# tgm-team/tgm

Measured on AMD Instinct MI355X. Metric: sampled-edges/sec (TGAT 2-hop k=20 recency sampler, tgbl-wiki synthetic), higher is better.
Workload: dtype int32/int64 indices + f32 feature rows (copied, no arithmetic)

## Files before the change

include/tgm_amd.h:

```cpp
#ifndef TGM_AMD_H
#define TGM_AMD_H

#include <stddef.h>
#include <stdint.h>

#ifdef __cplusplus
extern "C" {
#endif

#define TGMX_ABI_VERSION 7

#define TGMX_OK 0
#define TGMX_E_INVALID (-1)
#define TGMX_E_LAUNCH (-2)
#define TGMX_E_UNSUPPORTED (-3)

#define TGMX_ST_SEED_RANGE 1
#define TGMX_ST_SEED_TIME 2
#define TGMX_ST_EDGE_RANGE 4
#define TGMX_ST_SCRATCH 8
#define TGMX_ST_TS_BOUND 16

typedef void* tgmx_stream_t;
typedef void* tgmx_event_t;
// ... 40 lines not shown
                     int32_t* status, tgmx_stream_t stream,
                     tgmx_event_t ev_start, tgmx_event_t ev_stop);

size_t tgmx_ring_update_scratch_bytes(int64_t n, int32_t directed);
int tgmx_ring_update(tgmx_adj_t* ring, int32_t* write_pos, float* ring_x, int32_t D, int32_t B,
                     int32_t num_nodes, const int32_t* src, const int32_t* dst, const int64_t* ts,
                     const float* edge_x, int64_t n, int64_t eid0, int32_t directed, int32_t key_wrap32,
                     int32_t* scratch, int32_t* status, tgmx_stream_t stream);

#define TGMX_MAX_SEED_GROUPS 8
#define TGMX_MAX_HOPS 8
typedef struct tgmx_recency_step {
  tgmx_adj_t* ring;
  int32_t* write_pos;
  float* ring_x;
  const int64_t* indptr;
  int64_t ev_lo, ev_hi;
  int32_t D, B, num_nodes;
  int32_t n_groups;
  const int32_t* grp_nid[TGMX_MAX_SEED_GROUPS];
  const int64_t* grp_ts[TGMX_MAX_SEED_GROUPS];
  int64_t grp_n[TGMX_MAX_SEED_GROUPS];
  int32_t* seed_nid0;
  int64_t* seed_ts0;
  int64_t S0;
  int32_t n_hops;
  int32_t k[TGMX_MAX_HOPS];
  int32_t* out_nid[TGMX_MAX_HOPS];
  int64_t* out_ts[TGMX_MAX_HOPS];
  float* out_x[TGMX_MAX_HOPS];
  const int32_t* src;
  const int32_t* dst;
  const int64_t* ts;
  const float* edge_x;
  int64_t n, eid0;
  int32_t directed, key_wrap32;
  int32_t* scratch;
  int32_t* status;
  int32_t timed_hop;
  tgmx_event_t ev_start, ev_stop;
  int64_t ts_bound;
  int32_t neg_group, neg_low, neg_high;
  uint64_t neg_seed, neg_call;
  int32_t* neg_out;
  int64_t* neg_time_out;
  int32_t guard_seed_errors;
  int32_t sorted_ts;
  int32_t* out_valid[TGMX_MAX_HOPS];
  int32_t* out_valid_prev[TGMX_MAX_HOPS];
  int64_t neg_index0;
  int64_t* csr_cursor;
  int32_t csr_x_by_pos;
  int32_t* out_eid[TGMX_MAX_HOPS];
} tgmx_recency_step_t;

int tgmx_recency_step(const tgmx_recency_step_t* step, tgmx_stream_t stream);
int tgmx_recency_step_plan(const tgmx_recency_step_t* step);

#define TGMX_SEED_SRC 0
#define TGMX_SEED_DST 1
#define TGMX_SEED_NEG 2
typedef struct tgmx_pipeline {
  const int32_t* src;
  const int32_t* dst;
  const int64_t* ts;
  const float* edge_x;
  int64_t num_edges;
  int32_t rank, world;
  int32_t n_roles;
  int32_t seed_role[TGMX_MAX_SEED_GROUPS];
  int32_t neg_low, neg_high;
  uint64_t neg_seed;
  int32_t update;
  int32_t reserved0;
  tgmx_recency_step_t step;
} tgmx_pipeline_t;

typedef struct tgmx_pipeline_out {
  int32_t* neg;
  int64_t* neg_time;
  int32_t* seed_nid0;
  int64_t* seed_ts0;
  int32_t* out_nid[TGMX_MAX_HOPS];
  int64_t* out_ts[TGMX_MAX_HOPS];
  float* out_x[TGMX_MAX_HOPS];
  int32_t timed_hop;
  tgmx_event_t ev_start, ev_stop;
  int32_t* out_valid[TGMX_MAX_HOPS];
  int32_t* out_valid_prev[TGMX_MAX_HOPS];
  int32_t* out_eid[TGMX_MAX_HOPS];
} tgmx_pipeline_out_t;

typedef struct tgmx_pipeline_post {
  int32_t dedup;
  int32_t dedup_neg, dedup_nbr;
  int32_t num_nodes;
  void* dedup_ws;
  int32_t* uniq_out;
  int32_t edge_hop;
  int64_t edge_cap;
  int64_t* row_off;
  int64_t* edge_index;
  int64_t* edge_t;
  float* edge_x;
  int64_t* dev_sizes;
  int64_t* host_sizes;
  tgmx_event_t sizes_ready;
} tgmx_pipeline_post_t;

typedef void* tgmx_worker_t;
// ... 374 lines not shown
```

tgm_amd/_native.py:

```python
from __future__ import annotations

import ctypes
import os
from ctypes import c_char_p, c_int32, c_int64, c_size_t, c_void_p
from typing import Optional

import torch

from .exceptions import NativeLibraryError

_HERE = os.path.dirname(os.path.abspath(__file__))
LIB_PATH = os.path.join(_HERE, 'csrc', 'libtgm_amd.so')

_P = c_void_p
SIGNATURES = {
    'tgmx_version': (c_int32, []),
    'tgmx_abi_sizeof': (c_size_t, [c_int32]),
    'tgmx_last_error': (c_char_p, []),
    'tgmx_event_create': (c_int32, [ctypes.POINTER(c_void_p)]),
    'tgmx_event_destroy': (c_int32, [_P]),
    'tgmx_event_elapsed_ms': (c_int32, [_P, _P, ctypes.POINTER(ctypes.c_float)]),
    'tgmx_recency_lookup_csr': (
        c_int32,
        [_P, _P, _P, c_int32, _P, _P, c_int64, c_int32, c_int32, c_int64, c_int64, c_int32, c_int32, _P, _P, _P, _P, _P, _P, _P],
# ... 91 lines not shown
class TgatLayerGrads(ctypes.Structure):
    _fields_ = [(n, c_void_p) for n in ('W_Q', 'W_KV', 'W_O', 'b_O', 'ln_g', 'ln_b', 'fc1_w', 'fc1_b', 'fc2_w', 'fc2_b')]


class TgatGrads(ctypes.Structure):
    _fields_ = [('tw', c_void_p), ('tb', c_void_p), ('layers', TgatLayerGrads * TGAT_MAX_LAYERS)]


PACK_MAX_JOBS = 32


class PackJob(ctypes.Structure):
    _fields_ = [('src', c_void_p), ('dst', c_void_p), ('src_ld', c_int64), ('dst_ld', c_int64), ('rows', c_int32), ('cols', c_int32),
                ('dst_rows', c_int32), ('dst_cols', c_int32), ('transpose', c_int32), ('reserved_', c_int32)]


class TgatLayerLayout(ctypes.Structure):
    _fields_ = [(n, c_int64) for n in ('R', 'rres', 'oattn', 'y', 'Q', 'qf', 'zbar', 'cat', 'h1', 'probs', 'out')] + [
        (n, c_int32) for n in ('Op', 'dhp', 'Cp', 'Kc', 'Ep')
    ]


class TgatLayout(ctypes.Structure):
    _fields_ = [('total_bytes', c_int64), ('z0', c_int64), ('level_rows', c_int64 * (TGAT_MAX_LAYERS + 1)),
                ('level_off', c_int64 * (TGAT_MAX_LAYERS + 2)), ('layers', TgatLayerLayout * TGAT_MAX_LAYERS),
                ('compact', c_int64 * (TGAT_MAX_LAYERS + 1))]


MAX_SEED_GROUPS = 8
MAX_HOPS = 8


class RecencyStep(ctypes.Structure):

    _fields_ = [
        ('ring', c_void_p), ('write_pos', c_void_p), ('ring_x', c_void_p),
        ('indptr', c_void_p), ('ev_lo', c_int64), ('ev_hi', c_int64),
        ('D', c_int32), ('B', c_int32), ('num_nodes', c_int32),
        ('n_groups', c_int32),
        ('grp_nid', c_void_p * MAX_SEED_GROUPS), ('grp_ts', c_void_p * MAX_SEED_GROUPS), ('grp_n', c_int64 * MAX_SEED_GROUPS),
        ('seed_nid0', c_void_p), ('seed_ts0', c_void_p), ('S0', c_int64),
        ('n_hops', c_int32), ('k', c_int32 * MAX_HOPS),
        ('out_nid', c_void_p * MAX_HOPS), ('out_ts', c_void_p * MAX_HOPS), ('out_x', c_void_p * MAX_HOPS),
        ('src', c_void_p), ('dst', c_void_p), ('ts', c_void_p), ('edge_x', c_void_p),
        ('n', c_int64), ('eid0', c_int64), ('directed', c_int32), ('key_wrap32', c_int32),
        ('scratch', c_void_p), ('status', c_void_p),
        ('timed_hop', c_int32), ('ev_start', c_void_p), ('ev_stop', c_void_p),
        ('ts_bound', c_int64),
        ('neg_group', c_int32), ('neg_low', c_int32), ('neg_high', c_int32),
        ('neg_seed', ctypes.c_uint64), ('neg_call', ctypes.c_uint64), ('neg_out', c_void_p), ('neg_time_out', c_void_p),
        ('guard_seed_errors', c_int32), ('sorted_ts', c_int32),
        ('out_valid', c_void_p * MAX_HOPS), ('out_valid_prev', c_void_p * MAX_HOPS),
        ('neg_index0', c_int64), ('csr_cursor', c_void_p), ('csr_x_by_pos', c_int32), ('out_eid', c_void_p * MAX_HOPS),
    ]


class PipelinePost(ctypes.Structure):

    _fields_ = [
        ('dedup', c_int32), ('dedup_neg', c_int32), ('dedup_nbr', c_int32), ('num_nodes', c_int32), ('dedup_ws', c_void_p), ('uniq_out', c_void_p),
        ('edge_hop', c_int32), ('edge_cap', c_int64), ('row_off', c_void_p), ('edge_index', c_void_p), ('edge_t', c_void_p), ('edge_x', c_void_p),
        ('dev_sizes', c_void_p), ('host_sizes', c_void_p), ('sizes_ready', c_void_p),
    ]


class TgnMemoryFwd(ctypes.Structure):

    _fields_ = [
        ('nodes', c_void_p), ('R', c_int64), ('memory', c_void_p), ('last_update', c_void_p), ('M', c_int32), ('num_nodes', c_int32),
        ('st_lo_s', c_void_p), ('st_cnt_s', c_void_p), ('st_lo_d', c_void_p), ('st_cnt_d', c_void_p),
        ('log_other', c_void_p), ('log_t', c_void_p), ('log_raw', c_void_p), ('D', c_int32),
        ('tw', c_void_p), ('tb', c_void_p), ('T', c_int32), ('mean', c_int32),
        ('W_ih', c_void_p), ('b_ih', c_void_p), ('W_hh', c_void_p), ('b_hh', c_void_p),
        ('ws_aggr', c_void_p), ('ws_h', c_void_p), ('ws_gi', c_void_p), ('ws_gh', c_void_p),
        ('out_mem', c_void_p), ('out_lu', c_void_p), ('assoc', c_void_p), ('stamp', c_int64),
    ]


class TgnStep(ctypes.Structure):

    _fields_ = [
        ('mem', c_void_p), ('conv', c_void_p),
        ('src', c_void_p), ('dst', c_void_p), ('t', c_void_p), ('raw', c_void_p), ('n', c_int32),
        ('memory', c_void_p), ('last_update', c_void_p), ('reuse_status', c_void_p),
        ('log_base', c_int64), ('log_other', c_void_p), ('log_t', c_void_p), ('log_raw', c_void_p),
        ('st_lo_s', c_void_p), ('st_cnt_s', c_void_p), ('st_lo_d', c_void_p), ('st_cnt_d', c_void_p),
    ]


class TgcnFwd(ctypes.Structure):

    _fields_ = [
        ('x', c_void_p), ('N', c_int64), ('in_ch', c_int32), ('C', c_int32),
        ('src', c_void_p), ('dst', c_void_p), ('edge_w', c_void_p), ('E', c_int64), ('fill', ctypes.c_float), ('add_self_loops', c_int32),
        ('W3', c_void_p), ('b3', c_void_p),
        ('lin_w', c_void_p * 3), ('lin_b', c_void_p * 3),
        ('H', c_void_p),
        ('A', c_void_p), ('ldA', c_int64), ('norm_ws', c_void_p), ('xwt', c_void_p), ('G', c_void_p), ('cat', c_void_p), ('pre', c_void_p * 3),
        ('out', c_void_p), ('idx32', c_int32),
    ]


MIXER_MAX_LAYERS = 8


class MixerLayer(ctypes.Structure):
# ... 8 lines not shown
        ('nbr_edge_x', c_void_p), ('seed_t', c_void_p), ('nbr_t', c_void_p), ('nbr_nids', c_void_p),
        ('seeds', c_void_p * 3), ('n_seeds', c_int64 * 3),
        ('tg_nbr', c_void_p), ('tg_lo', c_void_p), ('tg_cnt', c_void_p),
        ('node_x', c_void_p), ('num_nodes', c_int64), ('F', c_int32),
        ('S', c_int64), ('K', c_int32), ('D', c_int32), ('T', c_int32), ('E', c_int32), ('num_layers', c_int32), ('eps', ctypes.c_float),
        ('tw', c_void_p), ('tb', c_void_p), ('proj_w', c_void_p), ('proj_b', c_void_p), ('out_w', c_void_p), ('out_b', c_void_p),
        ('layers', MixerLayer * MIXER_MAX_LAYERS),
        ('x0', c_void_p), ('z', c_void_p), ('z1', c_void_p), ('y', c_void_p), ('h', c_void_p), ('cat', c_void_p),
        ('ldx0', c_int64), ('ldz', c_int64), ('ldh', c_int64), ('ldcat', c_int64),
        ('out', c_void_p),
    ]


class TconvFwd(ctypes.Structure):

    _fields_ = [
        ('x', c_void_p), ('U', c_int64), ('in_ch', c_int32), ('last_update_local', c_void_p),
        ('src', c_void_p), ('tgt', c_void_p), ('t', c_void_p), ('msg', c_void_p), ('E', c_int64), ('D', c_int32), ('T', c_int32),
        ('tw', c_void_p), ('tb', c_void_p), ('W4', c_void_p), ('b4', c_void_p), ('W_edge', c_void_p), ('H', c_int32), ('C', c_int32),
        ('edge_attr', c_void_p), ('qkvs', c_void_p), ('eproj', c_void_p), ('order', c_void_p), ('seg_lo', c_void_p), ('seg_hi', c_void_p),
        ('sort_ws', c_void_p), ('sort_ws_bytes', c_size_t), ('status', c_void_p),
        ('tgt_count', c_void_p), ('cursor', c_void_p), ('order_big', c_void_p),
    ]


SEED_SRC, SEED_DST, SEED_NEG = 0, 1, 2


class Pipeline(ctypes.Structure):

    _fields_ = [
        ('src', c_void_p), ('dst', c_void_p), ('ts', c_void_p), ('edge_x', c_void_p), ('num_edges', c_int64),
        ('rank', c_int32), ('world', c_int32), ('n_roles', c_int32), ('seed_role', c_int32 * MAX_SEED_GROUPS),
        ('neg_low', c_int32), ('neg_high', c_int32), ('neg_seed', ctypes.c_uint64),
        ('update', c_int32), ('reserved0', c_int32), ('step', RecencyStep),
    ]


class PipelineOut(ctypes.Structure):

    _fields_ = [
        ('neg', c_void_p), ('neg_time', c_void_p), ('seed_nid0', c_void_p), ('seed_ts0', c_void_p),
        ('out_nid', c_void_p * MAX_HOPS), ('out_ts', c_void_p * MAX_HOPS), ('out_x', c_void_p * MAX_HOPS),
        ('timed_hop', c_int32), ('ev_start', c_void_p), ('ev_stop', c_void_p),
        ('out_valid', c_void_p * MAX_HOPS), ('out_valid_prev', c_void_p * MAX_HOPS), ('out_eid', c_void_p * MAX_HOPS),
    ]


ACCOUNTING_PARTIALS = 1024
SIGNATURES['tgmx_lookup_accounting'] = (c_int32, [_P, c_int64, _P, _P, c_int64, _P, _P])
SIGNATURES['tgmx_uniform_lookup_csr'] = (c_int32, [_P, _P, _P, c_int32, _P, c_int64, c_int32, c_int64, c_int32, c_int32, ctypes.c_uint64, ctypes.c_uint64,
                                                   _P, _P, _P, _P, _P])
SIGNATURES['tgmx_ring_update_scratch_bytes'] = (c_size_t, [c_int64, c_int32])
SIGNATURES['tgmx_tgn_gru_gate_backward'] = (c_int32, [_P, _P, _P, _P, c_int32, c_int64, _P, _P, _P])
SIGNATURES['tgmx_tgn_aggregate_backward'] = (c_int32, [c_int64, _P, _P, _P, _P, _P, _P, c_int32, c_int32, _P, _P, c_int32, c_int32, _P, _P, _P])
SIGNATURES['tgmx_tconv_edge_attr_backward'] = (c_int32, [_P, _P, _P, _P, _P, _P, c_int32, c_int32, c_int64, _P, _P])
SIGNATURES['tgmx_tconv_attend_backward'] = (c_int32, [_P, _P, _P, _P, _P, _P, _P, _P, c_int64, c_int32, c_int32, ctypes.c_float, _P, _P, _P, _P, _P, _P, _P])
SIGNATURES['tgmx_group_ids'] = (c_int32, [_P, c_int32, _P, _P, _P, _P, _P, _P])
SIGNATURES['tgmx_group_ids_workspace_bytes'] = (c_size_t, [c_int64])
SIGNATURES['tgmx_group_ids_large'] = (c_int32, [_P, c_int64, _P, _P, _P, _P, _P, _P, c_size_t, _P])
SIGNATURES['tgmx_random_negatives'] = (c_int32, [c_int32, c_int32, c_int64, ctypes.c_uint64, ctypes.c_uint64, _P, _P, c_int64, _P, _P])
SIGNATURES['tgmx_random_negatives_at'] = (c_int32, [c_int32, c_int32, c_int64, ctypes.c_uint64, ctypes.c_uint64, c_int64, _P, _P, c_int64, _P, _P])
SIGNATURES['tgmx_unique_ids_workspace_bytes'] = (c_size_t, [c_int32])
SIGNATURES['tgmx_unique_ids'] = (c_int32, [_P, _P, c_int32, c_int32, _P, _P, _P, _P, _P])
SIGNATURES['tgmx_csr_build_workspace_bytes'] = (c_size_t, [c_int64, c_int32, c_int32])
SIGNATURES['tgmx_csr_build'] = (c_int32, [_P, _P, _P, c_int64, c_int32, _P, c_int64, c_int32, _P, _P, _P, c_size_t, _P, _P])
SIGNATURES['tgmx_recency_step'] = (c_int32, [ctypes.POINTER(RecencyStep), _P])
SIGNATURES['tgmx_recency_step_plan'] = (c_int32, [ctypes.POINTER(RecencyStep)])
SIGNATURES['tgmx_pipeline_step'] = (c_int32, [ctypes.POINTER(Pipeline), c_int64, c_int64, ctypes.c_uint64, ctypes.POINTER(PipelineOut), ctypes.POINTER(PipelinePost), _P])
SIGNATURES['tgmx_event_synchronize'] = (c_int32, [_P])
SIGNATURES['tgmx_event_create_sync'] = (c_int32, [ctypes.POINTER(c_void_p)])
SIGNATURES['tgmx_event_record'] = (c_int32, [_P, _P])
SIGNATURES['tgmx_stream_wait_event'] = (c_int32, [_P, _P])
SIGNATURES['tgmx_stream_handoff'] = (c_int32, [_P, _P, _P])
SIGNATURES['tgmx_worker_create'] = (c_int32, [ctypes.POINTER(c_void_p)])
SIGNATURES['tgmx_worker_destroy'] = (c_int32, [_P])
SIGNATURES['tgmx_worker_pipeline_step'] = (c_int32, [_P, ctypes.POINTER(Pipeline), c_int64, c_int64, ctypes.c_uint64, ctypes.POINTER(PipelineOut),
                                                     ctypes.POINTER(PipelinePost), _P, _P, _P, ctypes.POINTER(ctypes.c_uint64)])
SIGNATURES['tgmx_worker_wait'] = (c_int32, [_P, ctypes.c_uint64])
SIGNATURES['tgmx_slice'] = (c_int32, [_P, c_int64, c_int32, c_int64, c_int32, c_int64, c_int64, c_int64, ctypes.POINTER(c_int64), ctypes.POINTER(c_int64)])
SIGNATURES['tgmx_discretize_workspace_bytes'] = (c_size_t, [c_int64])
SIGNATURES['tgmx_discretize_keep'] = (c_int32, [_P, _P, _P, c_int64, ctypes.c_double, _P, _P, _P, _P, c_size_t, _P])
SIGNATURES['tgmx_tgn_memory_forward'] = (c_int32, [ctypes.POINTER(TgnMemoryFwd), _P])
SIGNATURES['tgmx_tconv_forward'] = (c_int32, [ctypes.POINTER(TconvFwd), _P])
SIGNATURES['tgmx_tgn_step'] = (c_int32, [ctypes.POINTER(TgnStep), _P])
SIGNATURES['tgmx_segment_sort_workspace_bytes'] = (c_size_t, [c_int64])
SIGNATURES['tgmx_segment_sort'] = (c_int32, [_P, c_int64, c_int32, _P, _P, _P, _P, c_size_t, _P, _P])
SIGNATURES['tgmx_tgat_tile16_floats'] = (c_size_t, [c_int32, c_int32])
SIGNATURES['tgmx_tgat_tile16'] = (c_int32, [_P, c_int64, c_int32, c_int32, _P, _P])
SIGNATURES['tgmx_pack2d'] = (c_int32, [ctypes.POINTER(PackJob), c_int32, _P])

SIGNATURES['tgmx_pair_dedup_workspace_bytes'] = (c_size_t, [c_int64])
SIGNATURES['tgmx_pair_dedup'] = (c_int32, [_P, _P, c_int64, _P, _P, _P, _P, _P, c_size_t, _P])
SIGNATURES['tgmx_tgat_layout'] = (c_int32, [ctypes.POINTER(TgatModel), c_int64, ctypes.POINTER(TgatHop), c_int32, ctypes.POINTER(TgatLayout)])
SIGNATURES['tgmx_tgat_workspace_bytes'] = (c_size_t, [ctypes.POINTER(TgatModel), c_int64, ctypes.POINTER(TgatHop)])
SIGNATURES['tgmx_tgat_backward_workspace_bytes'] = (c_size_t, [ctypes.POINTER(TgatModel), ctypes.POINTER(TgatLayout), ctypes.POINTER(TgatHop)])
SIGNATURES['tgmx_tgat_backward'] = (c_int32, [ctypes.POINTER(TgatModel), ctypes.POINTER(TgatLayout), ctypes.POINTER(TgatHop), _P, _P, c_int64,
                                              ctypes.POINTER(Dropout), ctypes.POINTER(TgatGrads), _P, c_size_t, _P])
SIGNATURES['tgmx_tgat_forward'] = (
    c_int32,
    [ctypes.POINTER(TgatModel), _P, c_int64, _P, c_int64, ctypes.POINTER(TgatHop), _P, c_size_t, c_int32, _P, _P],
)

SIGNATURES['tgmx_sgemm_nt_ep'] = (c_int32, [_P, c_int64, _P, c_int64, _P, c_int64, c_int64, c_int32, c_int32, _P, c_int32, _P, c_int64, _P])
SIGNATURES['tgmx_time_gap_workspace_bytes'] = (c_size_t, [c_int64])
SIGNATURES['tgmx_time_gap_group'] = (c_int32, [_P, _P, c_int64, c_int64, _P, c_int64, _P, c_int64, _P, c_int64, _P, c_size_t, _P, _P, _P, _P])
# ... 90 lines not shown
```

tgm_amd/csrc/pipeline.hip:

```cpp
#include <algorithm>

#include "common.h"

using namespace tgmx;

__global__ __launch_bounds__(64) void sizes_to_host_kernel(const int64_t* __restrict__ dev, int64_t* __restrict__ host) {
  if (threadIdx.x < 3) __hip_atomic_store(&host[threadIdx.x], dev[threadIdx.x], __ATOMIC_RELAXED, __HIP_MEMORY_SCOPE_SYSTEM);
}

static int pipeline_post(const tgmx_pipeline_t* p, const tgmx_recency_step_t& s, int64_t edge_lo, int64_t n_edges, long long share,
                         const tgmx_pipeline_out_t* out, const tgmx_pipeline_post_t* post, tgmx_stream_t stream) {
  TGMX_REQUIRE(post->dev_sizes && post->host_sizes && post->sizes_ready, "pipeline_step: post block needs dev_sizes / host_sizes / sizes_ready");
  long long rows[TGMX_MAX_HOPS + 1];
  rows[0] = share * p->n_roles;
  for (int h = 0; h < s.n_hops; ++h) rows[h + 1] = rows[h] * s.k[h];
  bool scan_rides = false;
  if (post->dedup) {
    TGMX_REQUIRE(post->dedup_ws && post->uniq_out, "pipeline_step: null dedup buffer");
    const int32_t* parts[16];
    int64_t sizes[16];
    int np = 0;
    parts[np] = p->src + edge_lo; sizes[np++] = n_edges;
    parts[np] = p->dst + edge_lo; sizes[np++] = n_edges;
    if (post->dedup_neg && s.neg_out) { parts[np] = s.neg_out; sizes[np++] = share; }
// ... 39 lines not shown
                                  const tgmx_pipeline_out_t* out, const tgmx_pipeline_post_t* post, tgmx_stream_t stream) {
  TGMX_REQUIRE(p && out, "pipeline_step: null argument block");
  TGMX_REQUIRE(p->src && p->dst && p->ts && p->num_edges >= 0, "pipeline_step: null stream pointer");
  TGMX_REQUIRE(edge_lo >= 0 && n_edges >= 0 && edge_lo + n_edges <= p->num_edges, "pipeline_step: edges [%lld, +%lld) outside the store (%lld)",
               (long long)edge_lo, (long long)n_edges, (long long)p->num_edges);
  TGMX_REQUIRE(p->world >= 1 && p->rank >= 0 && p->rank < p->world, "pipeline_step: rank %d of %d", p->rank, p->world);
  TGMX_REQUIRE(p->n_roles >= 1 && p->n_roles <= TGMX_MAX_SEED_GROUPS, "pipeline_step: %d seed roles", p->n_roles);
  tgmx_recency_step_t s = p->step;
  const long long lo = n_edges * p->rank / p->world, hi = n_edges * (p->rank + 1) / p->world;
  const long long share = hi - lo;
  s.n_groups = p->n_roles;
  s.neg_out = nullptr;
  s.neg_group = -1;
  for (int g = 0; g < p->n_roles; ++g) {
    s.grp_ts[g] = p->ts + edge_lo + lo;
    s.grp_n[g] = share;
    switch (p->seed_role[g]) {
      case TGMX_SEED_SRC: s.grp_nid[g] = p->src + edge_lo + lo; break;
      case TGMX_SEED_DST: s.grp_nid[g] = p->dst + edge_lo + lo; break;
      case TGMX_SEED_NEG:
        TGMX_REQUIRE(s.neg_group < 0, "pipeline_step: more than one negatives role");
        TGMX_REQUIRE(share == 0 || (out->neg && out->neg_time), "pipeline_step: null negatives output");
        s.grp_nid[g] = nullptr;
        s.neg_group = g; s.neg_low = p->neg_low; s.neg_high = p->neg_high; s.neg_seed = p->neg_seed; s.neg_call = neg_call;
        s.neg_index0 = lo;
        s.neg_out = out->neg; s.neg_time_out = out->neg_time;
        break;
      default: TGMX_REQUIRE(false, "pipeline_step: seed role %d", p->seed_role[g]);
    }
  }
  s.seed_nid0 = out->seed_nid0;
  s.seed_ts0 = out->seed_ts0;
  for (int h = 0; h < s.n_hops && h < TGMX_MAX_HOPS; ++h) {
    s.out_nid[h] = out->out_nid[h];
    s.out_ts[h] = out->out_ts[h];
    s.out_x[h] = out->out_x[h];
    s.out_valid[h] = out->out_valid[h];
    s.out_valid_prev[h] = out->out_valid_prev[h];
    s.out_eid[h] = out->out_eid[h];
  }
  s.timed_hop = out->timed_hop;
  s.ev_start = out->ev_start;
  s.ev_stop = out->ev_stop;
  if (s.indptr) {
    s.ev_hi = edge_lo;
    s.n = 0;
  } else if (p->update && n_edges > 0) {
    s.src = p->src + edge_lo;
    s.dst = p->dst + edge_lo;
    s.ts = p->ts + edge_lo;
    s.edge_x = (p->edge_x && s.D > 0) ? p->edge_x + edge_lo * (long long)s.D : nullptr;
    s.n = n_edges;
    s.eid0 = edge_lo;
  } else {
    s.n = 0;
  }
  if (share == 0) {
    return TGMX_OK;
  }
  const int rc = tgmx_recency_step(&s, stream);
  if (rc || !post) return rc;
  return pipeline_post(p, s, edge_lo, n_edges, share, out, post, stream);
}

extern "C" int tgmx_slice(const int64_t* t, int64_t n, int32_t has_start_time, int64_t start_time, int32_t has_end_time,
                          int64_t end_time, int64_t start_idx, int64_t end_idx, int64_t* lb, int64_t* ub) {
  TGMX_REQUIRE((t || n == 0) && n >= 0 && lb && ub, "slice: bad arguments");
  long long l = has_start_time ? std::lower_bound(t, t + n, start_time) - t : 0;
  long long u = has_end_time ? std::upper_bound(t, t + n, end_time) - t : n;
  const long long lo_c = start_idx > 0 ? start_idx : 0, hi_c = end_idx >= 0 ? end_idx : n;
  l = std::max(lo_c, std::min(hi_c, l));
  u = std::max(lo_c, std::min(hi_c, u));
  *lb = l;
  *ub = u;
  return TGMX_OK;
}

namespace {
__global__ __launch_bounds__(256) void lookup_accounting_kernel(const int32_t* __restrict__ ids, long long slots, const int32_t* __restrict__ sp,
                                                                const int32_t* __restrict__ sc, long long rows, unsigned long long* __restrict__ counts) {
  unsigned long long v = 0, m = 0, c = 0;
  const long long step = (long long)gridDim.x * blockDim.x;
  for (long long i = (long long)blockIdx.x * blockDim.x + threadIdx.x; i < slots; i += step) v += ids[i] != -1;
  if (sp && sc)
    for (long long i = (long long)blockIdx.x * blockDim.x + threadIdx.x; i < rows; i += step) {
      const int a = sp[i], b = sc[i];
      m += (unsigned long long)(a > b ? a : b);
      c += (unsigned long long)b;
    }
  for (int o = 32; o > 0; o >>= 1) {
    v += __shfl_xor(v, o);
    m += __shfl_xor(m, o);
    c += __shfl_xor(c, o);
  }
  if ((threadIdx.x & 63) == 0) {
    unsigned long long* o = counts + ((long long)blockIdx.x * (blockDim.x >> 6) + (threadIdx.x >> 6)) * 3;
    o[0] = v; o[1] = m; o[2] = c;
  }
}
}

extern "C" int tgmx_lookup_accounting(const int32_t* ids, int64_t slots, const int32_t* span_prev, const int32_t* span_cur, int64_t rows,
                                      int64_t* counts, tgmx_stream_t stream) {
  TGMX_REQUIRE(ids && counts && slots >= 0 && rows >= 0, "lookup_accounting: bad arguments");
  hipStream_t st = (hipStream_t)stream;
  hipLaunchKernelGGL(lookup_accounting_kernel, dim3(TGMX_ACCOUNTING_PARTIALS / 4), dim3(256), 0, st, ids, (long long)slots, span_prev, span_cur, (long long)rows,
// ... 5 lines not shown
```

tgm_amd/csrc/recency.hip:

```cpp
#include <atomic>
#include <cstdlib>
#include <cstring>

#include <hip/hip_ext.h>
#include <rocprim/block/block_radix_sort.hpp>
#include <rocprim/block/block_scan.hpp>
#include <rocprim/device/device_radix_sort.hpp>
#include <rocprim/device/device_scan.hpp>
#include <rocprim/iterator/counting_iterator.hpp>
#include <rocprim/iterator/transform_iterator.hpp>

#include "common.h"

namespace tgmx {

struct __align__(16) Rec {
  int nbr;
  int eid;
  long long ts;
};
static_assert(sizeof(Rec) == sizeof(tgmx_adj_t), "record layout");

struct SeedGroups {
  const int32_t* nid[TGMX_MAX_SEED_GROUPS];
  const int64_t* ts[TGMX_MAX_SEED_GROUPS];
  long long end[TGMX_MAX_SEED_GROUPS];
  int32_t* out_nid;
  int64_t* out_ts;
  int groups;
  int gen;
  int gen_low;
  unsigned gen_range;
  unsigned long long gen_seed, gen_call, gen_index0;
  int32_t* gen_out;
  int64_t* gen_out_ts;
};

struct LookupArgs {
  SeedGroups grp;
  const int64_t* indptr;
  const Rec* recs;
  const int32_t* write_pos;
  const float* edge_x;
  const int32_t* seeds;
  const int64_t* qtimes;
  int32_t* out_nid;
  int64_t* out_ts;
  float* out_x;
  int32_t* status;
  long long S;
  long long ev_lo, ev_hi;
  int D, k, B, N, allow_pad;
  int row_vecs;
  FastDiv dv;
  FastDiv dv_seed;
  int32_t* out_eid;
  int32_t* out_eid1;
  int x_by_pos;
  long long* cursor;
  int leave_room;
  unsigned side_blocks;
  int side_stage;
  unsigned tail_blocks;
  int k1;
  int32_t* out_nid1;
  int64_t* out_ts1;
  float* out_x1;
  int32_t* out_valid;
  int32_t* out_valid1;
  int32_t* out_valid_prev;
  int32_t* out_valid_prev1;
};

template <int VEC>
struct VecOf;
template <>
struct VecOf<4> { using type = float4; };
template <>
struct VecOf<2> { using type = float2; };
template <>
struct VecOf<1> { using type = float; };

template <typename T>
__device__ __forceinline__ T zero_vec();
template <>
__device__ __forceinline__ float4 zero_vec<float4>() { return make_float4(0.f, 0.f, 0.f, 0.f); }
template <>
__device__ __forceinline__ float2 zero_vec<float2>() { return make_float2(0.f, 0.f); }
template <>
__device__ __forceinline__ float zero_vec<float>() { return 0.f; }

__device__ __forceinline__ long long wave_prefix_count(const Rec* recs, long long a, long long z,
                                                       long long bound, int lane) {
  long long lo = a, hi = z;
  while (hi - lo > kWave) {
    const long long len = hi - lo;
    const long long stride = (len + kWave - 1) / kWave;
    long long idx = lo + (long long)(lane + 1) * stride - 1;
    if (idx > hi - 1) idx = hi - 1;
    const bool less = (long long)recs[idx].eid < bound;
    const int c = __popcll(__ballot(less));
    long long nlo = lo, nhi = hi;
    if (c > 0) {
      long long p = lo + (long long)c * stride - 1;
      if (p > hi - 1) p = hi - 1;
      nlo = p + 1;
    }
    if (c < kWave) {
      long long p = lo + (long long)(c + 1) * stride - 1;
      if (p > hi - 1) p = hi - 1;
      nhi = p;
    }
    lo = nlo;
    hi = nhi < nlo ? nlo : nhi;
  }
  const long long idx = lo + lane;
  const bool less = idx < hi && (long long)recs[idx].eid < bound;
  return lo + __popcll(__ballot(less)) - a;
}

struct UpdateArgs {
  Rec* ring;
  int32_t* write_pos;
  float* ring_x;
  const float* edge_x;
  const int32_t* src;
  const int32_t* dst;
  const int64_t* ts;
  int32_t* sorted_j;
  int32_t* sorted_node;
  int32_t* target;
  int32_t* winner;
  Rec* sorted_rec;
  long long* key;
  int32_t* node;
  long long* span;
  unsigned long long* keys_in;
  unsigned int* vals_in;
  int32_t* hash_key;
  int32_t* hash_maxp;
  int32_t* run_start;
  int32_t* run_len;
  int hash_bits;
  long long ts_bound;
  int sorted_ts;
  int sort_bits;
  int32_t* barrier;
  int32_t* status;
  int guard_mask;
  long long n, m, eid0;
  int B, N, D, key_wrap32;
};

__device__ __forceinline__ long long update_key(int node, long long t, long long span, int wrap32) {
  if (wrap32) {
    const unsigned int prod = (unsigned int)node * (unsigned int)(int)span;
    return (long long)(int)prod + t;
  }
  return (long long)node * span + t;
}

__device__ __forceinline__ void update_entry(const UpdateArgs& a, long long j, int& node, int& nbr, long long& t,
                                             long long& i) {
  const bool rev = j >= a.n;
  i = rev ? j - a.n : j;
  const int s = a.src[i], d = a.dst[i];
  node = rev ? d : s;
  nbr = rev ? s : d;
  t = a.ts[i];
}

constexpr int kBlockMaxM = 4096;
constexpr int kChunk = 256;

__device__ __forceinline__ long long strided_max_ts(const int64_t* __restrict__ ts, long long n, int tid, int nthr) {
  long long mx = -0x7fffffffffffffffLL;
  for (long long base = tid; base < n; base += 8ll * nthr) {
    long long v[8];
#pragma unroll
    for (int u = 0; u < 8; ++u) {
      const long long x = base + (long long)u * nthr;
      v[u] = x < n ? ts[x] : mx;
    }
#pragma unroll
    for (int u = 0; u < 8; ++u) mx = v[u] > mx ? v[u] : mx;
  }
  return mx;
}

__device__ __forceinline__ long long strided_min_ts(const int64_t* __restrict__ ts, long long n, int tid, int nthr) {
  long long mn = 0x7fffffffffffffffLL;
  for (long long base = tid; base < n; base += 8ll * nthr) {
    long long v[8];
#pragma unroll
    for (int u = 0; u < 8; ++u) {
      const long long x = base + (long long)u * nthr;
      v[u] = x < n ? ts[x] : mn;
    }
#pragma unroll
    for (int u = 0; u < 8; ++u) mn = v[u] < mn ? v[u] : mn;
  }
  return mn;
}

constexpr int kBlockThreads = 1024;


__device__ __forceinline__ void bitonic_select(long long& key, int& pay, long long pk, int pp, int e, int jj, int k) {
  const bool low = (e & jj) == 0, asc = (e & k) == 0;
  const bool mine_after = pair_after(key, pay, pk, pp);
  if ((low == asc) == mine_after) {
    key = pk;
    pay = pp;
  }
}

__device__ __forceinline__ bool update_blocked(const UpdateArgs& a) {
  return a.guard_mask != 0 && (__hip_atomic_load(a.status, __ATOMIC_RELAXED, __HIP_MEMORY_SCOPE_AGENT) & a.guard_mask) != 0;
}

__device__ __forceinline__ void commit_write_pos(int32_t* wp, int kept, int B) {
  const int old = atomicAdd(wp, kept);
  constexpr int kFold = 1 << 30;
  if (old < kFold && old + kept >= kFold) atomicSub(wp, kFold / B * B);
}

template <int MAXM>
struct PlaceLds {
  int sn[MAXM];
  int len[MAXM];
  int h_key[2 * MAXM], h_maxp[2 * MAXM];
  long long red[kBlockThreads / kWave], red2[kBlockThreads / kWave];
  int wave_tot[kBlockThreads / kWave];
};
template <int MAXM>
struct SortLds {
  long long key[MAXM];
  int pay[MAXM];
};

template <typename T>
__device__ __forceinline__ void st_agent(T* p, T v) {
  __hip_atomic_store(p, v, __ATOMIC_RELAXED, __HIP_MEMORY_SCOPE_AGENT);
}
template <typename T>
__device__ __forceinline__ T ld_agent(const T* p) {
  return __hip_atomic_load(p, __ATOMIC_RELAXED, __HIP_MEMORY_SCOPE_AGENT);
}

template <int E, int MAXM, bool PRESORTED, bool DEFER, bool COH = false>
__device__ __forceinline__ void update_block_body(const UpdateArgs& a, PlaceLds<MAXM>& L, SortLds<PRESORTED ? 1 : MAXM>& S,
                                                  int part = 0, int parts = 1) {
  constexpr int H = 2 * MAXM;
  constexpr int HBITS = MAXM == 512 ? 10 : (MAXM == 1024 ? 11 : (MAXM == 2048 ? 12 : 13));
  static_assert((1 << HBITS) == H, "hash size");
  long long* s_key = S.key;
  int* s_pay = S.pay;
  int* s_sn = L.sn;
  int* s_len = L.len;
  int* h_key = L.h_key;
  int* h_maxp = L.h_maxp;
  long long* red = L.red;
  long long* red2 = L.red2;
  int* wave_tot = L.wave_tot;
  const int m = (int)a.m;
  const int tid = threadIdx.x, lane = tid & 63, wave = tid >> 6;
  const int nthr = blockDim.x, nwaves = nthr >> 6;
  const int P = nthr * E;
  const bool blocked = DEFER ? false : update_blocked(a);

  for (int x = tid; x < H; x += nthr) {
    h_key[x] = -1;
    h_maxp[x] = -1;
  }
  int pay[E], node[E], w[E];
  if constexpr (PRESORTED) {
#pragma unroll
// ... 80 lines not shown
    }
    if (lane == kWave - 1) wave_tot[wave] = incl;
    int before = __shfl_up(incl, 1);
    if (lane == 0) before = 0;
    __syncthreads();
    for (int wv = 0; wv < wave; ++wv) before = wave_tot[wv] > before ? wave_tot[wv] : before;
#pragma unroll
    for (int r = 0; r < E; ++r) st[r] = st[r] > before ? st[r] : before;
  }
#pragma unroll
  for (int r = 0; r < E; ++r) {
    const int p = tid * E + r;
    if (p < m && (p == m - 1 || s_sn[p + 1] != node[r])) s_len[st[r]] = p - st[r] + 1;
  }
  __syncthreads();

  int tgt[E], hs[E], cnt[E];
#pragma unroll
  for (int r = 0; r < E; ++r) {
    const int p = tid * E + r;
    tgt[r] = -1;
    hs[r] = 0;
    cnt[r] = 0;
    if (p < m && node[r] >= 0 && (parts == 1 || node[r] % parts == part)) {
      cnt[r] = s_len[st[r]];
      const int pos = p - st[r];
      const int drop = cnt[r] > a.B ? cnt[r] - a.B : 0;
      if (pos >= drop) {
        const int t = node[r] * a.B + (w[r] + pos - drop) % a.B;
        unsigned h = ((unsigned)t * 2654435761u) >> (32 - HBITS);
        for (;;) {
          const int old = atomicCAS(&h_key[h], -1, t);
          if (old == -1 || old == t) break;
          h = (h + 1) & (H - 1);
        }
        atomicMax(&h_maxp[h], p);
        tgt[r] = t;
        hs[r] = (int)h;
      }
    }
  }
  __syncthreads();

#pragma unroll
  for (int r = 0; r < E; ++r) {
    const int p = tid * E + r;
    if (p >= m) continue;
    if (parts > 1 && (node[r] >= 0 ? node[r] % parts : 0) != part) continue;
    int win = -1, kept = 0;
    if (tgt[r] >= 0) {
      if (h_maxp[hs[r]] == p) {
        Rec rec;
        if constexpr (DEFER) {
        } else if constexpr (PRESORTED) {
          rec = a.sorted_rec[p];
        } else {
          int nd, nbr;
          long long t, i;
          update_entry(a, pay[r], nd, nbr, t, i);
          rec.nbr = nbr;
          rec.eid = a.eid0 >= 0 ? (int)(a.eid0 + i) : -1;
          rec.ts = t;
        }
        if constexpr (!DEFER) {
          if (!blocked) a.ring[tgt[r]] = rec;
        }
        win = blocked ? -1 : tgt[r];
      }
      if (p == st[r] + cnt[r] - 1) {
        kept = cnt[r] > a.B ? a.B : cnt[r];
        if constexpr (!DEFER) {
          if (!blocked) commit_write_pos(&a.write_pos[node[r]], kept, a.B);
        }
      }
    }
    a.winner[p] = win;
    if constexpr (DEFER) a.target[p] = kept;
    if constexpr (!PRESORTED) a.sorted_j[p] = pay[r];
  }
}

template <int E, int MAXM, bool PRESORTED>
__global__ __launch_bounds__(kBlockThreads) void ring_update_block_kernel(const UpdateArgs a) {
  __shared__ PlaceLds<MAXM> L;
  __shared__ SortLds<PRESORTED ? 1 : MAXM> S;
  update_block_body<E, MAXM, PRESORTED, false>(a, L, S, (int)blockIdx.x, (int)gridDim.x);
}

template <int E, int MAXM>
__global__ __launch_bounds__(kBlockThreads) void ring_update_decide_kernel(const UpdateArgs a) {
  __shared__ PlaceLds<MAXM> L;
  __shared__ SortLds<1> S;
  update_block_body<E, MAXM, true, true>(a, L, S, (int)blockIdx.x, (int)gridDim.x);
}


struct ChunkSortLds {
  long long key[kChunk];
  int pay[kChunk];
  long long red[kChunk / kWave], red2[kChunk / kWave];
};

template <bool AGENT = false>
__device__ __forceinline__ void update_chunk_sort(const UpdateArgs& a, int chunk, ChunkSortLds& W) {
  long long* s_key = W.key;
  int* s_pay = W.pay;
  long long* red = W.red;
  long long* red2 = W.red2;
  const int tid = threadIdx.x, lane = tid & 63, wave = tid >> 6;
  long long mx = strided_max_ts(a.ts, a.n, tid, kChunk), mn = strided_min_ts(a.ts, a.n, tid, kChunk);
  for (int off = 32; off > 0; off >>= 1) {
    const long long o = __shfl_xor(mx, off), o2 = __shfl_xor(mn, off);
    mx = o > mx ? o : mx;
    mn = o2 < mn ? o2 : mn;
  }
  if (lane == 0) {
    red[wave] = mx;
    red2[wave] = mn;
  }
  __syncthreads();
  mx = red[0];
  mn = red2[0];
  for (int w = 1; w < kChunk / kWave; ++w) {
    mx = red[w] > mx ? red[w] : mx;
    mn = red2[w] < mn ? red2[w] : mn;
// ... 104 lines not shown
  __syncthreads();

  int pos[NE][NC];
#pragma unroll
  for (int q = 0; q < NE; ++q) {
#pragma unroll
    for (int o = 0; o < NC; ++o) {
      int cnt = 0;
      if (act[q] && o < chunks && o != c0 + q) {
        const long long* sk = W.key + o * kSamplesPerChunk;
        const int* sp = W.pay + o * kSamplesPerChunk;
        if (pair_after(key[q], pay[q], sk[kSamplesPerChunk - 1], sp[kSamplesPerChunk - 1])) {
          cnt = kSamplesPerChunk;
        } else {
#pragma unroll
          for (int st = kSamplesPerChunk / 2; st > 0; st >>= 1)
            if (pair_after(key[q], pay[q], sk[cnt + st - 1], sp[cnt + st - 1])) cnt += st;
        }
      }
      pos[q][o] = cnt > 0 ? (cnt - 1) * kSampleEvery + 1 : -1;
    }
  }
#pragma unroll
  for (int st = kSampleEvery / 2; st > 0; st >>= 1) {
    long long k2[NE][NC];
#pragma unroll
    for (int q = 0; q < NE; ++q)
#pragma unroll
      for (int o = 0; o < NC; ++o) k2[q][o] = pos[q][o] >= 0 ? ld_agent(&gk[o * kChunk + pos[q][o] + st - 1]) : 0;
#pragma unroll
    for (int q = 0; q < NE; ++q) {
#pragma unroll
      for (int o = 0; o < NC; ++o) {
        if (pos[q][o] < 0) continue;
        bool after = key[q] > k2[q][o];
        if (key[q] == k2[q][o]) after = pay[q] > ld_agent(&gp[o * kChunk + pos[q][o] + st - 1]);
        if (after) pos[q][o] += st;
      }
    }
  }
  int node[NE], nbr[NE];
  long long t[NE], i[NE];
#pragma unroll
  for (int q = 0; q < NE; ++q) {
    node[q] = nbr[q] = -1;
    t[q] = i[q] = 0;
    if (act[q]) update_entry(a, pay[q], node[q], nbr[q], t[q], i[q]);
  }
  int w[NE];
  bool valid[NE];
#pragma unroll
  for (int q = 0; q < NE; ++q) {
    valid[q] = act[q] && node[q] >= 0 && node[q] < a.N && nbr[q] >= 0 && nbr[q] < a.N;
    w[q] = valid[q] ? a.write_pos[node[q]] : 0;
  }
#pragma unroll
  for (int q = 0; q < NE; ++q) {
    if (!act[q]) continue;
    int rank = tid;
#pragma unroll
    for (int o = 0; o < NC; ++o) rank += pos[q][o] >= 0 ? pos[q][o] : 0;
    if (!valid[q]) atomicOr(a.status, TGMX_ST_EDGE_RANGE);
    Rec rec;
    rec.nbr = nbr[q];
    rec.eid = a.eid0 >= 0 ? (int)(a.eid0 + i[q]) : -1;
    rec.ts = t[q];
    if constexpr (COH) {
      st_agent(&a.sorted_j[rank], pay[q]);
      st_agent(&a.sorted_node[rank], valid[q] ? node[q] : -1);
      st_agent(&a.target[rank], w[q] % a.B);
    } else {
      a.sorted_j[rank] = pay[q];
      a.sorted_node[rank] = valid[q] ? node[q] : -1;
      a.target[rank] = w[q] % a.B;
    }
    a.sorted_rec[rank] = rec;
  }
}

constexpr int kSideSort = 1, kSideMerge = 2, kSidePlace = 3, kSideAll = 4, kSideSortMerge = 5, kSidePlaceOnly = 6, kSideSortMergePlace = 7, kSideMergePlace = 8;

__device__ __forceinline__ bool rider_barrier(int32_t* bar, int parts) {
  __syncthreads();
  bool ok = true;
  if (threadIdx.x == 0) {
    const int gen = __hip_atomic_load(&bar[1], __ATOMIC_RELAXED, __HIP_MEMORY_SCOPE_AGENT);
    const int prev = __hip_atomic_fetch_add(&bar[0], 1, __ATOMIC_RELAXED, __HIP_MEMORY_SCOPE_AGENT);
    if (prev == parts - 1) {
      __hip_atomic_store(&bar[0], 0, __ATOMIC_RELAXED, __HIP_MEMORY_SCOPE_AGENT);
      __builtin_amdgcn_s_waitcnt(0);
      __hip_atomic_fetch_add(&bar[1], 1, __ATOMIC_RELAXED, __HIP_MEMORY_SCOPE_AGENT);
    } else {
      int spins = 0;
      while (__hip_atomic_load(&bar[1], __ATOMIC_RELAXED, __HIP_MEMORY_SCOPE_AGENT) == gen) {
        __builtin_amdgcn_s_sleep(8);
        if (++spins > (1 << 19)) {
          ok = false;
          break;
        }
      }
    }
  }
  __syncthreads();
  return ok;
}
constexpr int kRidePlaceMaxM = 1024;

constexpr int kTailGroups = 32;
__device__ __forceinline__ void tail_signal(int32_t* bar, bool publish, unsigned bid, unsigned nblk) {
  __syncthreads();
  if (threadIdx.x == 0) {
    if (publish) {
      __threadfence();
      __hip_atomic_store(&bar[4], 1, __ATOMIC_RELAXED, __HIP_MEMORY_SCOPE_AGENT);
      __hip_atomic_fetch_add(&bar[2], 1, __ATOMIC_RELAXED, __HIP_MEMORY_SCOPE_AGENT);
    } else {
      const unsigned g = bid % kTailGroups;
      const unsigned size = (nblk - g + kTailGroups - 1) / kTailGroups;
      int32_t* cnt = &bar[16 + 16 * g];
      const int prev = __hip_atomic_fetch_add(cnt, 1, __ATOMIC_RELAXED, __HIP_MEMORY_SCOPE_AGENT);
      if (prev == (int)size - 1) {
        __hip_atomic_store(cnt, 0, __ATOMIC_RELAXED, __HIP_MEMORY_SCOPE_AGENT);
        __hip_atomic_fetch_add(&bar[2], (int)size, __ATOMIC_RELAXED, __HIP_MEMORY_SCOPE_AGENT);
      }
    }
  }
}

__device__ __forceinline__ bool tail_wait(const int32_t* word, unsigned need) {
  int spins = 0;
  while ((unsigned)__hip_atomic_load(word, __ATOMIC_RELAXED, __HIP_MEMORY_SCOPE_AGENT) < need) {
    __builtin_amdgcn_s_sleep(8);
    if (++spins > (1 << 22)) return false;
  }
  return true;
}

__device__ __forceinline__ void tail_commit(const UpdateArgs& a, unsigned tb, unsigned tail_blocks, unsigned need) {
  __shared__ int ok_s;
  const int lane = lane_id();
  const long long p = (long long)tb * (blockDim.x >> 6) + (threadIdx.x >> 6);
  if (threadIdx.x == 0) ok_s = tail_wait(&a.barrier[4], 1u) ? 1 : 0;
  __syncthreads();
  bool ok = ok_s != 0;
  int row = -1, kept = 0, node = 0;
  long long rec_lo = 0, rec_hi = 0;
  constexpr int kMaxCols = 8;
  float xv[kMaxCols];
  const float* x = nullptr;
  const bool wide = a.D > kMaxCols * kWave;
  if (ok && p < a.m) {
    row = ld_agent(&a.winner[p]);
    kept = ld_agent(&a.target[p]);
    if (row >= 0) {
      const long long* src = reinterpret_cast<const long long*>(&a.sorted_rec[p]);
      rec_lo = ld_agent(&src[0]);
      rec_hi = ld_agent(&src[1]);
    }
    if (kept > 0) node = ld_agent(&a.sorted_node[p]);
    if (row >= 0 && a.D > 0 && a.edge_x) {
      const long long j = ld_agent(&a.sorted_j[p]);
      x = a.edge_x + (j >= a.n ? j - a.n : j) * a.D;
      if (!wide) {
#pragma unroll
        for (int u = 0; u < kMaxCols; ++u) {
          const int c = lane + u * kWave;
          xv[u] = c < a.D ? x[c] : 0.f;
        }
      }
    }
  }
  if (threadIdx.x == 0) ok_s = (ok && tail_wait(&a.barrier[2], need)) ? 1 : 0;
  __syncthreads();
  ok = ok_s != 0;
  if (!ok) {
    if (threadIdx.x == 0) atomicOr(a.status, TGMX_ST_SCRATCH);
  } else if (p < a.m && !update_blocked(a)) {
    if (lane == 0) {
      if (row >= 0) {
        long long* dst = reinterpret_cast<long long*>(&a.ring[row]);
        dst[0] = rec_lo;
        dst[1] = rec_hi;
      }
      if (kept > 0) commit_write_pos(&a.write_pos[node], kept, a.B);
    }
    if (row >= 0 && a.D > 0) {
      float* __restrict__ o = a.ring_x + (long long)row * a.D;
      if (!x) {
        for (int c = lane; c < a.D; c += kWave) o[c] = 0.f;
      } else if (wide) {
        for (int c = lane; c < a.D; c += kWave) o[c] = x[c];
      } else {
#pragma unroll
        for (int u = 0; u < kMaxCols; ++u) {
          const int c = lane + u * kWave;
          if (c < a.D) o[c] = xv[u];
        }
      }
    }
  }
  __syncthreads();
  if (threadIdx.x == 0) {
    const int prev = __hip_atomic_fetch_add(&a.barrier[3], 1, __ATOMIC_RELAXED, __HIP_MEMORY_SCOPE_AGENT);
    if (prev == (int)tail_blocks - 1) {
      __hip_atomic_store(&a.barrier[2], 0, __ATOMIC_RELAXED, __HIP_MEMORY_SCOPE_AGENT);
      __hip_atomic_store(&a.barrier[3], 0, __ATOMIC_RELAXED, __HIP_MEMORY_SCOPE_AGENT);
      __hip_atomic_store(&a.barrier[4], 0, __ATOMIC_RELAXED, __HIP_MEMORY_SCOPE_AGENT);
    }
  }
}

template <int PCAP>
union RiderLds {
  ChunkSortLds sort;
  SampleLds smp;
  PlaceLds<PCAP> place;
};
template <>
union RiderLds<0> {
  ChunkSortLds sort;
  SampleLds smp;
};

template <int PCAP = kRidePlaceMaxM>
__device__ __forceinline__ void update_side_work(const UpdateArgs& u, int stage, int block) {
  __shared__ RiderLds<PCAP> W;
  if (stage == kSideSort) {
    update_chunk_sort(u, block, W.sort);
  } else if (stage == kSideMerge) {
    update_merge_riding<1, kBlockMaxM / kChunk>(u, block, W.smp);
  } else if (stage == kSideSortMerge) {
    update_chunk_sort<true>(u, block, W.sort);
    if (!rider_barrier(u.barrier, (int)((u.m + kChunk - 1) / kChunk)) && threadIdx.x == 0) atomicOr(u.status, TGMX_ST_SCRATCH);
    update_merge_riding<1, kBlockMaxM / kChunk>(u, block, W.smp);
  } else if constexpr (PCAP > 0) {
    constexpr int NCH = PCAP / kChunk;
    if (stage == kSideSortMergePlace) {
      const int chunks = (int)((u.m + kChunk - 1) / kChunk);
      __shared__ int last_out;
      update_chunk_sort<true>(u, block, W.sort);
      if (!rider_barrier(u.barrier, chunks) && threadIdx.x == 0) atomicOr(u.status, TGMX_ST_SCRATCH);
      update_merge_riding<1, NCH, true>(u, block, W.smp);
      __syncthreads();
      if (threadIdx.x == 0) {
        const int prev = __hip_atomic_fetch_add(&u.barrier[5], 1, __ATOMIC_RELAXED, __HIP_MEMORY_SCOPE_AGENT);
        last_out = prev == chunks - 1;
        if (last_out) __hip_atomic_store(&u.barrier[5], 0, __ATOMIC_RELAXED, __HIP_MEMORY_SCOPE_AGENT);
      }
      __syncthreads();
      if (!last_out) return;
      SortLds<1> none;
      update_block_body<NCH, PCAP, true, true, true>(u, W.place, none);
      return;
    }
    if (stage == kSideMergePlace) {
      const int chunks = (int)((u.m + kChunk - 1) / kChunk);
      __shared__ int last_mp;
      update_merge_riding<1, NCH, true>(u, block, W.smp);
      __syncthreads();
      if (threadIdx.x == 0) {
        const int prev = __hip_atomic_fetch_add(&u.barrier[5], 1, __ATOMIC_RELAXED, __HIP_MEMORY_SCOPE_AGENT);
        last_mp = prev == chunks - 1;
// ... 61 lines not shown
    const int32_t* pn = a.grp.nid[0];
    const int64_t* pt = a.grp.ts[0];
    long long base = 0;
    int sel = 0;
#pragma unroll
    for (int g = 1; g < TGMX_MAX_SEED_GROUPS; ++g) {
      if (g < a.grp.groups && s >= a.grp.end[g - 1]) {
        pn = a.grp.nid[g];
        pt = a.grp.ts[g];
        base = a.grp.end[g - 1];
        sel = g;
      }
    }
    const bool gen = sel == a.grp.gen;
    n = gen ? negative_draw(a.grp.gen_seed, a.grp.gen_call, a.grp.gen_index0 + (unsigned long long)(s - base), a.grp.gen_low, a.grp.gen_range) : pn[s - base];
    q = pt[s - base];
    if (publish && lane == 0) {
      a.grp.out_nid[s] = n;
      a.grp.out_ts[s] = q;
      if (gen) {
        a.grp.gen_out[s - base] = n;
        a.grp.gen_out_ts[s - base] = q;
      }
    }
  } else {
    n = a.seeds[s];
    q = a.qtimes[s];
  }
}

__device__ __forceinline__ void check_seed(const LookupArgs& a, int n, long long q, int allow_pad, int lane) {
  if (lane == 0) {
    int st = 0;
    if (n >= a.N || n < -1 || (n == -1 && !allow_pad)) st |= TGMX_ST_SEED_RANGE;
    if (q < 0 && !allow_pad) st |= TGMX_ST_SEED_TIME;
    if (st) atomicOr(a.status, st);
  }
}

struct Window {
  long long w0;
  int wlen, wrot;
};

template <bool RING>
__device__ __forceinline__ Window find_window(const LookupArgs& a, int n, bool live, int lane) {
  Window w;
  w.w0 = 0;
  w.wlen = 0;
  w.wrot = 0;
  if (live) {
    if (RING) {
      w.w0 = (long long)n * a.B;
      w.wrot = a.write_pos[n] % a.B;
      w.wlen = a.B;
    } else {
      const long long ra = a.indptr[n], rz = a.indptr[n + 1];
      const long long p_hi = ra + wave_prefix_count(a.recs, ra, rz, a.ev_hi, lane);
      const long long p_lo = a.ev_lo <= 0 ? ra : ra + wave_prefix_count(a.recs, ra, rz, a.ev_lo, lane);
      w.w0 = p_hi - a.B > p_lo ? p_hi - a.B : p_lo;
      w.wlen = (int)(p_hi - w.w0);
    }
  }
  return w;
}

template <bool RING>
__device__ __forceinline__ long long slot_of(const Window& w, int B, int i) {
  if (RING) {
    int sl = w.wrot + i;
    if (sl >= B) sl -= B;
    return w.w0 + sl;
  }
  return w.w0 + i;
}

struct SmallPick {
  bool has;
  int nbr, src, eid;
  long long ts;
};

template <bool RING>
__device__ __forceinline__ SmallPick small_pick(const LookupArgs& a, int n, long long q, int k, bool live, int lane) {
  const int B = a.B;
  const Window w = find_window<RING>(a, n, live, lane);
  Rec r;
  r.nbr = -1; r.eid = 0; r.ts = 0;
  if (RING) {
    if (live && lane < B) r = a.recs[(long long)n * B + lane];
    int from_slot = w.wrot + lane;
    if (from_slot >= B) from_slot -= B;
    if (lane >= B) from_slot = lane;
    r.nbr = __shfl(r.nbr, from_slot);
    r.ts = __shfl(r.ts, from_slot);
    if (a.out_eid || a.out_eid1) r.eid = __shfl(r.eid, from_slot);
  } else if (lane < w.wlen) {
    r = a.recs[slot_of<RING>(w, B, lane)];
  }
  const bool ok = lane < w.wlen && r.nbr >= 0 && r.ts < q;
  const unsigned long long m = __ballot(ok);
  const int cnt = m ? 64 - __clzll((long long)m) : 0;
  const int i = cnt - k + lane;
  const int from = i > 0 ? i : 0;
  const int g_nbr = __shfl(r.nbr, from);
  const int g_eid = __shfl(r.eid, from);
  const long long g_ts = __shfl(r.ts, from);
  SmallPick o;
  o.has = i >= 0 && g_nbr >= 0;
  o.nbr = o.has ? g_nbr : -1;
  o.ts = o.has ? g_ts : 0;
  o.src = o.has ? ((RING || a.x_by_pos) ? (int)slot_of<RING>(w, B, from) : g_eid) : -1;
  o.eid = o.has ? g_eid : -1;
  return o;
}

template <int VEC>
__device__ __forceinline__ void gather_rows(const LookupArgs& a, long long s, int k, int lane, const int* lds_eid, float* out_x, int first_slot) {
  using V = typename VecOf<VEC>::type;
  const V* __restrict__ X = reinterpret_cast<const V*>(a.edge_x);
  V* __restrict__ O = reinterpret_cast<V*>(out_x + s * (long long)k * a.D);
  const int total = k * a.row_vecs;
  constexpr int U = 8;
  for (int f0 = first_slot * a.row_vecs + lane; f0 < total; f0 += kWave * U) {
    long long idx[U];
    bool has[U];
#pragma unroll
    for (int u = 0; u < U; ++u) {
      const int f = f0 + u * kWave;
      const int fc = f < total ? f : f0;
      const int slot = (int)a.dv.div_nb((uint32_t)fc);
      const int col = fc - slot * a.row_vecs;
      const int e = lds_eid[slot];
      has[u] = e >= 0;
      idx[u] = has[u] ? (long long)e * a.row_vecs + col : 0;
    }
    V v[U];
#pragma unroll
    for (int u = 0; u < U; ++u) v[u] = X[idx[u]];
#pragma unroll
    for (int u = 0; u < U; ++u) {
      const int f = f0 + u * kWave;
      if (f < total) O[f] = has[u] ? v[u] : zero_vec<V>();
    }
  }
}

template <bool RING, int VEC, bool SMALL>
__device__ __forceinline__ void lookup_seed(const LookupArgs& a, long long s, int n, long long q, int k, int lane, int* lds_eid,
                                            int32_t* out_nid, int64_t* out_ts, float* out_x, int32_t* out_valid, int32_t* out_valid_prev,
                                            int32_t* out_eid = nullptr) {
  const bool live = n >= 0 && n < a.N;
  int v_new = 0;
  if (SMALL) {
    const SmallPick o = small_pick<RING>(a, n, q, k, live, lane);
    if (lane < k) {
      out_nid[s * k + lane] = o.nbr;
      out_ts[s * k + lane] = o.ts;
      if (out_eid) out_eid[s * k + lane] = o.eid;
      lds_eid[lane] = o.src;
    }
    const unsigned long long m = __ballot(lane < k && o.has);
    v_new = m ? k - __builtin_ctzll(m) : 0;
  } else {
    const int B = a.B;
    const Window w = find_window<RING>(a, n, live, lane);
    int cnt = 0;
    for (int top = w.wlen; top > 0 && cnt == 0; top -= kWave) {
      const int lo = top > kWave ? top - kWave : 0;
      const int i = lo + lane;
      bool ok = false;
      if (i < top) {
        const Rec r = a.recs[slot_of<RING>(w, B, i)];
        ok = r.nbr >= 0 && r.ts < q;
      }
      const unsigned long long m = __ballot(ok);
      if (m) cnt = lo + 64 - __clzll((long long)m);
    }
    for (int c = lane; c < k; c += kWave) {
      const int i = cnt - k + c;
      Rec r;
      r.nbr = -1; r.eid = 0; r.ts = 0;
      if (i >= 0) r = a.recs[slot_of<RING>(w, B, i)];
      const bool has = r.nbr >= 0;
      out_nid[s * k + c] = has ? r.nbr : -1;
      out_ts[s * k + c] = has ? r.ts : 0;
      if (out_eid) out_eid[s * k + c] = has ? r.eid : -1;
      lds_eid[c] = has ? ((RING || a.x_by_pos) ? (int)slot_of<RING>(w, B, i) : r.eid) : -1;
      if (has && k - c > v_new) v_new = k - c;
    }
    for (int o = 32; o > 0; o >>= 1) {
      const int other = __shfl_xor(v_new, o);
      v_new = other > v_new ? other : v_new;
    }
  }
  if (a.D == 0 || out_x == nullptr) return;
  int first_slot = 0;
  if (out_valid) {
    const int v_old = out_valid[s];
    first_slot = k - (v_old > v_new ? v_old : v_new);
    if (lane == 0) {
      out_valid[s] = v_new;
      if (out_valid_prev) out_valid_prev[s] = v_old;
    }
  }
  __builtin_amdgcn_wave_barrier();
  gather_rows<VEC>(a, s, k, lane, lds_eid, out_x, first_slot);
  __builtin_amdgcn_wave_barrier();
}

template <bool RING, int VEC, bool SMALL, bool RIDE>
__global__ __launch_bounds__(256) void recency_lookup_kernel(const LookupArgs a, const UpdateArgs u) {
  extern __shared__ __attribute__((aligned(16))) int lds_eid_all[];
  unsigned bid = blockIdx.x, nblk = gridDim.x;
  if constexpr (RING && RIDE) {
    if (bid < a.side_blocks) {
      update_side_work(u, a.side_stage, (int)bid);
      if (a.tail_blocks) tail_signal(u.barrier, true, 0, 0);
      return;
    }
    bid -= a.side_blocks;
    nblk -= a.side_blocks + a.tail_blocks;
    if (bid >= nblk) {
      tail_commit(u, bid - nblk, a.tail_blocks, nblk + a.side_blocks);
      return;
    }
  }
  const int lane = lane_id();
  const int wave_in_block = threadIdx.x >> 6;
  int* lds_eid = lds_eid_all + wave_in_block * a.k;
  const long long waves_total = (long long)nblk * (blockDim.x >> 6);
  for (long long s = (long long)bid * (blockDim.x >> 6) + wave_in_block; s < a.S; s += waves_total) {
    int n;
    long long q;
    fetch_seed(a, s, lane, true, n, q);
    check_seed(a, n, q, a.allow_pad, lane);
    lookup_seed<RING, VEC, SMALL>(a, s, n, q, a.k, lane, lds_eid, a.out_nid, a.out_ts, a.out_x, a.out_valid, a.out_valid_prev, a.out_eid);
  }
  if constexpr (RING && RIDE) {
    if (a.tail_blocks) tail_signal(u.barrier, false, bid, nblk);
  }
}

template <bool RING, int VEC, int PCAP = kRidePlaceMaxM>
__global__ __launch_bounds__(256) void recency_lookup_fused01_kernel(const LookupArgs a, const UpdateArgs u) {
  extern __shared__ __attribute__((aligned(16))) int lds_eid_all[];
  unsigned bid = blockIdx.x, nblk = gridDim.x;
  if constexpr (RING) {
    if (bid < a.side_blocks) {
      update_side_work<PCAP>(u, a.side_stage, (int)bid);
      if (a.tail_blocks) tail_signal(u.barrier, true, 0, 0);
      return;
    }
    bid -= a.side_blocks;
    nblk -= a.side_blocks + a.tail_blocks;
    if (bid >= nblk) {
      tail_commit(u, bid - nblk, a.tail_blocks, nblk + a.side_blocks);
      return;
    }
  }
  const int lane = lane_id();
  const int wave_in_block = threadIdx.x >> 6;
  const int k0 = a.k, k1 = a.k1;
  int* lds_eid = lds_eid_all + wave_in_block * (k0 > k1 ? k0 : k1);
  const long long waves_total = (long long)nblk * (blockDim.x >> 6);
  const long long S0 = a.S, S1 = a.S * k0;
  for (long long w = (long long)bid * (blockDim.x >> 6) + wave_in_block; w < S0 + S1; w += waves_total) {
    int n;
    long long q;
    if (w < S0) {
      fetch_seed(a, w, lane, true, n, q);
      check_seed(a, n, q, 0, lane);
      lookup_seed<RING, VEC, true>(a, w, n, q, k0, lane, lds_eid, a.out_nid, a.out_ts, a.out_x, a.out_valid, a.out_valid_prev, a.out_eid);
    } else {
      const long long idx = w - S0;
      const long long s0 = idx / k0;
      const int j = (int)(idx - s0 * k0);
      int n0;
      long long q0;
      fetch_seed(a, s0, lane, false, n0, q0);
      const SmallPick o = small_pick<RING>(a, n0, q0, k0, n0 >= 0 && n0 < a.N, lane);
      n = __shfl(o.nbr, j);
      q = __shfl(o.ts, j);
      lookup_seed<RING, VEC, true>(a, idx, n, q, k1, lane, lds_eid, a.out_nid1, a.out_ts1, a.out_x1, a.out_valid1, a.out_valid_prev1, a.out_eid1);
    }
  }
  if constexpr (RING) {
    if (a.tail_blocks) tail_signal(u.barrier, false, bid, nblk);
  }
}

struct GroupPick {
  bool has;
  int nbr, src;
  long long ts;
};

template <bool RING, int GL>
__device__ __forceinline__ GroupPick group_pick(const LookupArgs& a, int n, long long q, int k, bool live, int gl, int sub) {
  const int B = a.B;
  long long w0 = 0;
  int wrot = 0, wlen = 0;
  if constexpr (RING) {
    w0 = (long long)(live ? n : 0) * B;
    wrot = live ? a.write_pos[n] % B : 0;
    wlen = live ? B : 0;
  } else {
    const long long ra = live ? a.indptr[n] : 0, rz = live ? a.indptr[n + 1] : 0;
    const long long p_hi = ra + group_prefix_count<GL>(a.recs, ra, rz, a.ev_hi, gl, sub);
    const long long p_lo = a.ev_lo <= 0 ? ra : ra + group_prefix_count<GL>(a.recs, ra, rz, a.ev_lo, gl, sub);
    w0 = p_hi - B > p_lo ? p_hi - B : p_lo;
    wlen = (int)(p_hi - w0);
  }
  Rec r;
  r.nbr = -1; r.eid = 0; r.ts = 0;
  if (gl < wlen) r = a.recs[w0 + gl];
  if constexpr (RING) {
    int from_slot = wrot + gl;
    if (from_slot >= B) from_slot -= B;
    if (gl >= B) from_slot = gl;
    r.nbr = __shfl(r.nbr, sub * GL + from_slot);
    r.ts = __shfl(r.ts, sub * GL + from_slot);
  }
  const bool ok = gl < wlen && r.nbr >= 0 && r.ts < q;
  const unsigned long long m = (__ballot(ok) >> (sub * GL)) & ((GL == 64) ? ~0ull : ((1ull << GL) - 1));
  const int cnt = m ? 64 - __clzll((long long)m) : 0;
  const int i = cnt - k + gl;
  const int from = i > 0 ? i : 0;
  const int g_nbr = __shfl(r.nbr, sub * GL + from);
  const int g_eid = __shfl(r.eid, sub * GL + from);
  const long long g_ts = __shfl(r.ts, sub * GL + from);
  GroupPick o;
  o.has = i >= 0 && g_nbr >= 0;
  o.nbr = o.has ? g_nbr : -1;
  o.ts = o.has ? g_ts : 0;
  int sl = wrot + from;
  if (sl >= B) sl -= B;
  o.src = o.has ? ((RING || a.x_by_pos) ? (int)(w0 + sl) : g_eid) : -1;
  return o;
}

template <int VEC, int GL>
// ... 8 lines not shown
  if (a.D == 0) return;
  int first_slot = 0;
  if (out_valid) {
    const unsigned long long m = (__ballot(act && gl < k && o.has) >> (sub * GL)) & ((GL == 64) ? ~0ull : ((1ull << GL) - 1));
    const int v_new = m ? k - __builtin_ctzll(m) : 0;
    int v_old = 0;
    if (act) {
      v_old = out_valid[s];
      first_slot = k - (v_old > v_new ? v_old : v_new);
    }
    __builtin_amdgcn_wave_barrier();
    if (act && gl == 0) {
      out_valid[s] = v_new;
      if (out_valid_prev) out_valid_prev[s] = v_old;
    }
  }
  __builtin_amdgcn_wave_barrier();
  if (act) {
    const V* __restrict__ X = reinterpret_cast<const V*>(a.edge_x);
    V* __restrict__ O = reinterpret_cast<V*>(out_x + s * (long long)k * a.D);
    const int total = k * a.row_vecs;
    constexpr int U = 4;
    for (int f0 = first_slot * a.row_vecs + gl; f0 < total; f0 += GL * U) {
      V v[U];
#pragma unroll
      for (int u = 0; u < U; ++u) {
        const int f = f0 + u * GL;
        v[u] = zero_vec<V>();
        if (f < total) {
          const int slot = (int)a.dv.div((uint32_t)f);
          const int col = f - slot * a.row_vecs;
          const int e = lds_eid[slot];
          if (e >= 0) v[u] = X[(long long)e * a.row_vecs + col];
        }
      }
#pragma unroll
      for (int u = 0; u < U; ++u) {
        const int f = f0 + u * GL;
        if (f < total) O[f] = v[u];
      }
    }
  }
  __builtin_amdgcn_wave_barrier();
}

template <bool RING, int VEC, int GL, bool RIDE>
__global__ __launch_bounds__(256) void lookup_packed_kernel(const LookupArgs a, const UpdateArgs u) {
  constexpr int kGroups = kWave / GL;
  extern __shared__ __attribute__((aligned(16))) int lds_eid_all[];
  unsigned bid = blockIdx.x, nblk = gridDim.x;
  if constexpr (RING && RIDE) {
    if (bid < a.side_blocks) {
      update_side_work(u, a.side_stage, (int)bid);
      if (a.tail_blocks) tail_signal(u.barrier, true, 0, 0);
      return;
    }
    bid -= a.side_blocks;
    nblk -= a.side_blocks + a.tail_blocks;
    if (bid >= nblk) {
      tail_commit(u, bid - nblk, a.tail_blocks, nblk + a.side_blocks);
      return;
    }
  }
  const int lane = lane_id();
  const int sub = lane / GL, gl = lane - sub * GL;
  const int wave_in_block = threadIdx.x >> 6;
  const int k = a.k;
  int* lds_eid = lds_eid_all + (wave_in_block * kGroups + sub) * k;
  const long long waves_total = (long long)nblk * (blockDim.x >> 6);
  const long long n_rounds = (a.S + kGroups - 1) / kGroups;
  for (long long w = (long long)bid * (blockDim.x >> 6) + wave_in_block; w < n_rounds; w += waves_total) {
    const long long s = w * kGroups + sub;
    const bool act = s < a.S;
    int n = -1;
    long long q = 0;
    if (act) {
      if (a.grp.groups > 0) {
        fetch_seed(a, s, gl, true, n, q);
      } else {
        n = a.seeds[s];
        q = a.qtimes[s];
      }
    }
    if (act && gl == 0) {
      int st = 0;
      if (n >= a.N || n < -1 || (n == -1 && !a.allow_pad)) st |= TGMX_ST_SEED_RANGE;
      if (q < 0 && !a.allow_pad) st |= TGMX_ST_SEED_TIME;
      if (st) atomicOr(a.status, st);
    }
    const GroupPick o = group_pick<RING, GL>(a, n, q, k, n >= 0 && n < a.N, gl, sub);
    group_emit<VEC, GL>(a, act, s, k, o, lds_eid, gl, sub, a.out_nid, a.out_ts, a.out_x, a.out_valid, a.out_valid_prev);
  }
  if constexpr (RING && RIDE) {
    if (a.tail_blocks) tail_signal(u.barrier, false, bid, nblk);
  }
}


typedef unsigned int tgmx_u4 __attribute__((ext_vector_type(4)));
typedef unsigned int tgmx_u2 __attribute__((ext_vector_type(2)));
__device__ __forceinline__ void buffer_store_vec(float4 v, __amdgpu_buffer_rsrc_t r, unsigned off, unsigned soff) {
  __builtin_amdgcn_raw_buffer_store_b128(*reinterpret_cast<tgmx_u4*>(&v), r, off, soff, 0);
}
__device__ __forceinline__ void buffer_store_vec(float2 v, __amdgpu_buffer_rsrc_t r, unsigned off, unsigned soff) {
  __builtin_amdgcn_raw_buffer_store_b64(*reinterpret_cast<tgmx_u2*>(&v), r, off, soff, 0);
}
__device__ __forceinline__ void buffer_store_vec(float v, __amdgpu_buffer_rsrc_t r, unsigned off, unsigned soff) {
  __builtin_amdgcn_raw_buffer_store_b32(__float_as_uint(v), r, off, soff, 0);
}
__device__ __forceinline__ void buffer_load_vec(float4& v, __amdgpu_buffer_rsrc_t r, unsigned off) {
  const tgmx_u4 x = __builtin_amdgcn_raw_buffer_load_b128(r, off, 0, 0);
  v = *reinterpret_cast<const float4*>(&x);
}
__device__ __forceinline__ void buffer_load_vec(float2& v, __amdgpu_buffer_rsrc_t r, unsigned off) {
  const tgmx_u2 x = __builtin_amdgcn_raw_buffer_load_b64(r, off, 0, 0);
  v = *reinterpret_cast<const float2*>(&x);
}
__device__ __forceinline__ void buffer_load_vec(float& v, __amdgpu_buffer_rsrc_t r, unsigned off) {
  v = __uint_as_float(__builtin_amdgcn_raw_buffer_load_b32(r, off, 0, 0));
}
template <typename T>
__device__ __forceinline__ T* wave_uniform_ptr(T* p) {
  const unsigned long long v = (unsigned long long)p;
  const unsigned lo = __builtin_amdgcn_readfirstlane((unsigned)v), hi = __builtin_amdgcn_readfirstlane((unsigned)(v >> 32));
  return reinterpret_cast<T*>(((unsigned long long)hi << 32) | lo);
}

template <int VEC, bool SMALL_TABLE>
__device__ __forceinline__ void tile_copy(const LookupArgs& a, long long t, int rows, int k, int lane, const int* Lsrc,
                                          const unsigned short* Llist, int n_rows, long long table_rows) {
  using V = typename VecOf<VEC>::type;
  const V* __restrict__ X = reinterpret_cast<const V*>(a.edge_x);
  const int rv = a.row_vecs, total = n_rows * rv;
  float* base = wave_uniform_ptr(a.out_x + t * 64 * (long long)k * a.D);
  const __amdgpu_buffer_rsrc_t O = __builtin_amdgcn_make_buffer_rsrc(base, 0, rows * k * rv * (int)sizeof(V), 0x00020000);
  const __amdgpu_buffer_rsrc_t T = __builtin_amdgcn_make_buffer_rsrc(const_cast<float*>(a.edge_x), 0,
                                                                     SMALL_TABLE ? (int)(unsigned)(table_rows * rv * (long long)sizeof(V)) : 0, 0x00020000);
  constexpr int U = SMALL_TABLE ? 16 : 12;
  constexpr unsigned kDrop = 0xFFFFFFF0u;
  __builtin_amdgcn_s_waitcnt(0x0F70);
  for (int fb = 0; fb < total; fb += kWave * U) {
    unsigned off[U];
    V v[U];
    if constexpr (SMALL_TABLE) {
      unsigned src[U];
#pragma unroll
      for (int u = 0; u < U; ++u) {
        const int f = fb + u * kWave + lane;
// ... 29 lines not shown
#pragma unroll
      for (int u = 0; u < U; ++u) v[u] = X[idx[u]];
#pragma unroll
      for (int u = 0; u < U; ++u) v[u] = has[u] ? v[u] : zero_vec<V>();
    }
#pragma unroll
    for (int u = 0; u < U; ++u) buffer_store_vec(v[u], O, off[u], 0u);
  }
}

__device__ __forceinline__ long long lane_prefix_count(const Rec* __restrict__ recs, long long a, long long z, long long bound) {
  long long lo = a, hi = z;
  while (hi - lo > 3) {
    const long long q = (hi - lo) >> 2;
    const long long m1 = lo + q, m2 = lo + 2 * q, m3 = lo + 3 * q;
    const bool l1 = (long long)recs[m1].eid < bound, l2 = (long long)recs[m2].eid < bound, l3 = (long long)recs[m3].eid < bound;
    if (l3) lo = m3 + 1;
    else if (l2) { lo = m2 + 1; hi = m3; }
    else if (l1) { lo = m1 + 1; hi = m2; }
    else hi = m1;
  }
  while (lo < hi && (long long)recs[lo].eid < bound) ++lo;
  return lo - a;
}

__device__ __forceinline__ long long lane_prefix_end_hinted(const Rec* __restrict__ recs, long long ra, long long rz, long long bound, long long hint) {
  long long lo = ra, hi = rz;
  if (hint >= ra && hint <= rz) {
    const bool below = hint == ra || (long long)recs[hint - 1].eid < bound;
    const bool at = hint < rz && (long long)recs[hint].eid < bound;
    if (below && !at) return hint;
    if (below) {
      lo = hint + 1;
      long long step = 1;
      while (lo + step <= rz && (long long)recs[lo + step - 1].eid < bound) {
        lo += step;
        step <<= 1;
      }
      hi = lo + step - 1 < rz ? lo + step - 1 : rz;
    } else {
      hi = hint - 1;
    }
  }
  return lo + lane_prefix_count(recs, lo, hi, bound);
}

template <bool RING, int VEC, int BCAP, bool RIDE>
__global__ __launch_bounds__(256) void lookup_tile_kernel(const LookupArgs a, const UpdateArgs u) {
  extern __shared__ __attribute__((aligned(16))) int lds_eid_all[];
  unsigned bid = blockIdx.x, nblk = gridDim.x;
  if constexpr (RING && RIDE) {
    if (bid < a.side_blocks) {
      update_side_work(u, a.side_stage, (int)bid);
      if (a.tail_blocks) tail_signal(u.barrier, true, 0, 0);
      return;
    }
    bid -= a.side_blocks;
    nblk -= a.side_blocks + a.tail_blocks;
    if (bid >= nblk) {
      tail_commit(u, bid - nblk, a.tail_blocks, nblk + a.side_blocks);
      return;
    }
  }
  const int lane = lane_id();
  const int wave_in_block = threadIdx.x >> 6, wpb = blockDim.x >> 6;
  const int k = a.k, B = a.B;
  int* L = lds_eid_all + wave_in_block * (kWave * k + kWave * k / 2 + kWave);
  int* Lstage = L;
  int* Lfirst = L + kWave * k;
  const long long tiles = (a.S + kWave - 1) / kWave;
  for (long long tv = (long long)bid * wpb + wave_in_block; tv < tiles; tv += (long long)nblk * wpb) {
    const long long t = (long long)(((unsigned long long)__builtin_amdgcn_readfirstlane((unsigned)((unsigned long long)tv >> 32)) << 32) |
                                    __builtin_amdgcn_readfirstlane((unsigned)(unsigned long long)tv));
    const long long s = t * kWave + lane;
    const bool act = s < a.S;
    int n = -1, v_old = 0;
    long long q = 0;
    if (act) {
      if (a.grp.groups > 0) {
        fetch_seed(a, s, 0, true, n, q);
      } else {
        n = a.seeds[s];
        q = a.qtimes[s];
      }
      if (a.out_valid) v_old = a.out_valid[s];
      int st = 0;
      if (n >= a.N || n < -1 || (n == -1 && !a.allow_pad)) st |= TGMX_ST_SEED_RANGE;
      if (q < 0 && !a.allow_pad) st |= TGMX_ST_SEED_TIME;
      if (st) atomicOr(a.status, st);
    }
    const bool live = n >= 0 && n < a.N;
    long long w0 = 0;
    int wrot = 0, wlen = 0;
    if (live) {
      if constexpr (RING) {
        w0 = (long long)n * B;
        wlen = B;
      } else {
        const long long ra = a.indptr[n], rz = a.indptr[n + 1];
        const long long hint = a.cursor ? a.cursor[n] : -1;
        const long long p_hi = lane_prefix_end_hinted(a.recs, ra, rz, a.ev_hi, hint);
        if (a.cursor && p_hi != hint) a.cursor[n] = p_hi;
        const long long p_lo = a.ev_lo <= 0 ? ra : ra + lane_prefix_count(a.recs, ra, rz, a.ev_lo);
        w0 = p_hi - B > p_lo ? p_hi - B : p_lo;
        wlen = (int)(p_hi - w0);
      }
    }
    Rec r[BCAP];
#pragma unroll
    for (int j = 0; j < BCAP; ++j) {
      r[j].nbr = -1;
      r[j].eid = 0;
      r[j].ts = 0;
      if (j < wlen) r[j] = a.recs[w0 + j];
    }
// ... 36 lines not shown
    const int ne = rows * k;
    {
      const int4* __restrict__ L4 = reinterpret_cast<const int4*>(Lstage);
      int32_t* __restrict__ G = a.out_nid + t * kWave * k;
      int4* __restrict__ G4 = reinterpret_cast<int4*>(G);
      for (int f = lane; f < (ne >> 2); f += kWave) G4[f] = L4[f];
      for (int f = (ne & ~3) + lane; f < ne; f += kWave) G[f] = Lstage[f];
    }
    long long* Lts = reinterpret_cast<long long*>(Lstage);
#pragma unroll
    for (int half = 0; half < 2; ++half) {
      __builtin_amdgcn_wave_barrier();
      const bool mine = (lane >> 5) == half;
      const int lr = lane & 31;
      if (mine) {
        for (int c = 0; c < k; ++c) Lts[lr * k + c] = 0;
#pragma unroll
        for (int j = 0; j < BCAP; ++j)
          if (cj[j] >= 0) Lts[lr * k + cj[j]] = r[j].ts;
      }
      __builtin_amdgcn_wave_barrier();
      const int hrows = rows - 32 * half < 32 ? rows - 32 * half : 32;
      if (hrows > 0) {
        const int he = hrows * k;
        const int4* __restrict__ T4 = reinterpret_cast<const int4*>(Lts);
        int64_t* __restrict__ H = a.out_ts + (t * kWave + 32 * half) * k;
        int4* __restrict__ H4 = reinterpret_cast<int4*>(H);
        for (int f = lane; f < (he >> 1); f += kWave) H4[f] = T4[f];
        if ((he & 1) && lane == 0) H[he - 1] = Lts[he - 1];
      }
    }
    if (a.D > 0) {
      __builtin_amdgcn_wave_barrier();
      for (int c = 0; c < k; ++c) Lstage[lane * k + c] = -1;
#pragma unroll
      for (int j = 0; j < BCAP; ++j)
        if (cj[j] >= 0) Lstage[lane * k + cj[j]] = (RING || a.x_by_pos) ? (int)(w0 + j) : r[j].eid;
      const int nact = k - first_slot;
      int incl = nact;
#pragma unroll
      for (int d = 1; d < kWave; d <<= 1) {
        const int up = __shfl_up(incl, d);
        if (lane >= d) incl += up;
      }
      const int n_rows = __shfl(incl, kWave - 1);
      unsigned short* Llist = reinterpret_cast<unsigned short*>(Lfirst);
      for (int i = 0; i < nact; ++i) Llist[incl - nact + i] = (unsigned short)((lane << 8) | (first_slot + i));
      __builtin_amdgcn_wave_barrier();
      if constexpr (RING) tile_copy<VEC, true>(a, t, rows, k, lane, Lstage, Llist, n_rows, (long long)a.N * B);
      else tile_copy<VEC, false>(a, t, rows, k, lane, Lstage, Llist, n_rows, 0);
    }
    __builtin_amdgcn_wave_barrier();
  }
  if constexpr (RING && RIDE) {
    if (a.tail_blocks) tail_signal(u.barrier, false, bid, nblk);
  }
}

template <bool RING, int VEC, int BCAP, bool RIDE>
__global__ __launch_bounds__(256) __attribute__((amdgpu_waves_per_eu(1, (RING && !RIDE) ? 2 : 8))) void lookup_tile_coop_kernel(const LookupArgs a, const UpdateArgs u) {
  extern __shared__ __attribute__((aligned(16))) int lds_eid_all[];
  constexpr int SPI = kWave / BCAP;
  constexpr int NI = (kWave + SPI - 1) / SPI;
  unsigned bid = blockIdx.x, nblk = gridDim.x;
  if constexpr (RING && RIDE) {
    if (bid < a.side_blocks) {
      update_side_work(u, a.side_stage, (int)bid);
      if (a.tail_blocks) tail_signal(u.barrier, true, 0, 0);
      return;
    }
    bid -= a.side_blocks;
    nblk -= a.side_blocks + a.tail_blocks;
    if (bid >= nblk) {
      tail_commit(u, bid - nblk, a.tail_blocks, nblk + a.side_blocks);
      return;
    }
  }
  const int lane = lane_id();
  const int wave_in_block = threadIdx.x >> 6, wpb = blockDim.x >> 6;
  const int k = a.k, B = a.B;
  constexpr int kHdrInts = kWave * 4 + kWave * 2 + kWave;
  int* L = lds_eid_all + wave_in_block * (kWave * k + kWave * k / 2 + kWave + kHdrInts);
  int* Lstage = L;
  int* Lfirst = L + kWave * k;
  int4* Lhdr = reinterpret_cast<int4*>(L + kWave * k + kWave * k / 2 + kWave);
  long long* Lq = reinterpret_cast<long long*>(Lhdr + kWave);
  int* Lspan = reinterpret_cast<int*>(Lq + kWave);
  const int seg0 = lane / BCAP;
  auto fresh = [](int v) __attribute__((always_inline)) {
    asm volatile("" : "+v"(v));
    return v;
  };
  const unsigned FM = (1u << BCAP) - 1, BM = (1u << B) - 1;
  const long long tiles = (a.S + kWave - 1) / kWave;
  for (long long tv = (long long)bid * wpb + wave_in_block; tv < tiles; tv += (long long)nblk * wpb) {
    const long long t = (long long)(((unsigned long long)__builtin_amdgcn_readfirstlane((unsigned)((unsigned long long)tv >> 32)) << 32) |
                                    __builtin_amdgcn_readfirstlane((unsigned)(unsigned long long)tv));
    const long long s = t * kWave + lane;
    const bool act = s < a.S;
    int n = -1, v_old = 0;
    long long q = 0;
    if (act) {
      if (a.grp.groups > 0) {
        fetch_seed(a, s, 0, true, n, q);
      } else {
        n = a.seeds[s];
        q = a.qtimes[s];
      }
      if (a.out_valid) v_old = a.out_valid[s];
      int st = 0;
      if (n >= a.N || n < -1 || (n == -1 && !a.allow_pad)) st |= TGMX_ST_SEED_RANGE;
      if (q < 0 && !a.allow_pad) st |= TGMX_ST_SEED_TIME;
      if (st) atomicOr(a.status, st);
    }
    const bool live = n >= 0 && n < a.N;
    long long w0 = 0;
    int wlen = 0;
    if (live) {
      if constexpr (RING) {
        w0 = (long long)n * B;
        wlen = B;
      } else {
        const long long ra = a.indptr[n], rz = a.indptr[n + 1];
        const long long hint = a.cursor ? a.cursor[n] : -1;
        const long long p_hi = lane_prefix_end_hinted(a.recs, ra, rz, a.ev_hi, hint);
        if (a.cursor && p_hi != hint) a.cursor[n] = p_hi;
        const long long p_lo = a.ev_lo <= 0 ? ra : ra + lane_prefix_count(a.recs, ra, rz, a.ev_lo);
        w0 = p_hi - B > p_lo ? p_hi - B : p_lo;
        wlen = (int)(p_hi - w0);
// ... 76 lines not shown
      __builtin_amdgcn_wave_barrier();
      if ((lane >> 5) == half) {
        const int lr = lane & 31;
        for (int c = 0; c < k; ++c) Lts[lr * k + c] = 0;
      }
      __builtin_amdgcn_wave_barrier();
      seg = fresh(seg0);
#pragma unroll
      for (int i = 0; i < NI; ++i) {
        const int sl = i * SPI + seg;
        const int c1 = (int)((cs4[i >> 2] >> (8 * (i & 3))) & 255u);
        if (c1 > 0 && (sl >> 5) == half) Lts[(sl & 31) * k + c1 - 1] = r[i].ts;
      }
      __builtin_amdgcn_wave_barrier();
      const int hrows = rows - 32 * half < 32 ? rows - 32 * half : 32;
      if (hrows > 0) {
        const int he = hrows * k;
        const int4* __restrict__ T4 = reinterpret_cast<const int4*>(Lts);
        int64_t* __restrict__ H = a.out_ts + (t * kWave + 32 * half) * k;
        int4* __restrict__ H4 = reinterpret_cast<int4*>(H);
        for (int f = lane; f < (he >> 1); f += kWave) H4[f] = T4[f];
        if ((he & 1) && lane == 0) H[he - 1] = Lts[he - 1];
      }
    }
    if (a.D > 0) {
      __builtin_amdgcn_wave_barrier();
      for (int c = 0; c < k; ++c) Lstage[lane * k + c] = -1;
      __builtin_amdgcn_wave_barrier();
      seg = fresh(seg0), j = lane - seg * BCAP;
#pragma unroll
      for (int i = 0; i < NI; ++i) {
        const int sl = i * SPI + seg;
        const int c1 = (int)((cs4[i >> 2] >> (8 * (i & 3))) & 255u);
        if (c1 > 0) Lstage[sl * k + c1 - 1] = (RING || a.x_by_pos) ? (int)((unsigned)Lhdr[sl].x + (unsigned)j) : r[i].eid;
      }
      const int nact = k - first_slot;
      int incl = nact;
#pragma unroll
      for (int d = 1; d < kWave; d <<= 1) {
        const int up = __shfl_up(incl, d);
        if (lane >= d) incl += up;
      }
      const int n_rows = __shfl(incl, kWave - 1);
      unsigned short* Llist = reinterpret_cast<unsigned short*>(Lfirst);
      for (int i = 0; i < nact; ++i) Llist[incl - nact + i] = (unsigned short)((lane << 8) | (first_slot + i));
      __builtin_amdgcn_wave_barrier();
      int lane_c = lane;
      asm volatile("" : "+v"(lane_c));
      if constexpr (RING) tile_copy<VEC, true>(a, t, rows, k, lane_c, Lstage, Llist, n_rows, (long long)a.N * B);
      else tile_copy<VEC, false>(a, t, rows, k, lane_c, Lstage, Llist, n_rows, 0);
    }
    __builtin_amdgcn_wave_barrier();
  }
  if constexpr (RING && RIDE) {
    if (a.tail_blocks) tail_signal(u.barrier, false, bid, nblk);
  }
}

template <auto Kernel>
static bool lds_optin() {
  constexpr int kMaxDevices = 64;
  static std::atomic<bool> done[kMaxDevices];
  int dev = 0;
  if (hipGetDevice(&dev) != hipSuccess || dev < 0 || dev >= kMaxDevices) dev = -1;
  if (dev >= 0 && done[dev].load(std::memory_order_acquire)) return true;
  const hipError_t e = hipFuncSetAttribute(reinterpret_cast<const void*>(Kernel), hipFuncAttributeMaxDynamicSharedMemorySize, 128 * 1024);
  if (e != hipSuccess) {
    set_error("recency_lookup: cannot reserve LDS: %s", hipGetErrorString(e));
    return false;
  }
  if (dev >= 0) done[dev].store(true, std::memory_order_release);
  return true;
}

static int device_cu_count() {
  static std::atomic<int> cus[64];
  int dev = 0;
  if (hipGetDevice(&dev) != hipSuccess || dev < 0 || dev >= 64) return 256;
  int n = cus[dev].load(std::memory_order_relaxed);
  if (n == 0) {
    if (hipDeviceGetAttribute(&n, hipDeviceAttributeMultiprocessorCount, dev) != hipSuccess || n <= 0) n = 256;
    cus[dev].store(n, std::memory_order_relaxed);
  }
  return n;
}

#define TGMX_LAUNCH_TIMED(KERNEL, GRID, BLOCK, LDS, STREAM, E0, E1, ...)                          \
  do {                                                                                           \
    if ((E0) && (E1)) hipExtLaunchKernelGGL(KERNEL, GRID, BLOCK, (uint32_t)(LDS), STREAM, E0, E1, 0, __VA_ARGS__); \
    else hipLaunchKernelGGL(KERNEL, GRID, BLOCK, LDS, STREAM, __VA_ARGS__);                      \
  } while (0)

static int prepare_lookup(LookupArgs& a, const float* out_x, int kmax) {
  int vec = 1;
  if (a.D > 0) {
    const uintptr_t bits = (uintptr_t)a.edge_x | (uintptr_t)out_x | (uintptr_t)a.out_x;
    if (a.D % 4 == 0 && (bits & 15) == 0) vec = 4;
    else if (a.D % 2 == 0 && (bits & 7) == 0) vec = 2;
  }
  a.row_vecs = a.D > 0 ? a.D / vec : 1;
  a.dv = make_fastdiv((uint32_t)a.row_vecs);
  a.dv_seed = make_fastdiv((uint32_t)(kmax * a.row_vecs));
  if ((unsigned long long)kmax * a.row_vecs * (unsigned long long)a.row_vecs >= (1ull << 32)) {
    set_error("recency_lookup: k*D^2 too large for the slot divider (k=%d, D=%d)", kmax, a.D);
    return TGMX_E_UNSUPPORTED;
  }
  return vec;
}

static int packed_group_lanes(const LookupArgs& a, int k, bool ring) {
  const int gl = (a.B <= 16 && k <= 16) ? 16 : ((a.B <= 32 && k <= 32) ? 32 : 64);
  return (ring && gl < 64 && (long long)k * a.row_vecs <= 8 * gl) ? gl : 64;
}

template <bool RING>
static int launch_lookup(LookupArgs a, hipStream_t stream, hipEvent_t ev_start, hipEvent_t ev_stop,
                         const UpdateArgs* side = nullptr, int side_stage = 0, unsigned side_blocks = 0, unsigned tail_blocks = 0) {
  if (a.S == 0) return TGMX_OK;
  const UpdateArgs u = side ? *side : UpdateArgs{};
  a.side_blocks = (RING && side) ? side_blocks : 0;
  a.side_stage = side_stage;
  a.tail_blocks = a.side_blocks ? tail_blocks : 0;
  const bool small = a.B <= kWave && a.k <= kWave;
  const int vec = prepare_lookup(a, a.out_x, a.k);
  if (vec < 0) return vec;
  const int waves_per_block = 4;
  long long blocks = (a.S + waves_per_block - 1) / waves_per_block;
  if (blocks > (1 << 20)) blocks = 1 << 20;
  const dim3 grid((unsigned)blocks + a.side_blocks + a.tail_blocks), block(waves_per_block * kWave);
  const size_t lds = (size_t)waves_per_block * a.k * sizeof(int);
  const bool ride = RING && a.side_blocks > 0;
#define TGMX_LAUNCH(VEC_, SMALL_)                                                                                              \
  do {                                                                                                                         \
    if (ride) TGMX_LAUNCH_TIMED((recency_lookup_kernel<RING, VEC_, SMALL_, true>), grid, block, lds, stream, ev_start, ev_stop, a, u); \
    else TGMX_LAUNCH_TIMED((recency_lookup_kernel<RING, VEC_, SMALL_, false>), grid, block, lds, stream, ev_start, ev_stop, a, u);     \
  } while (0)
  const int gl_any = a.out_eid ? 64 : packed_group_lanes(a, a.k, true);
  static const bool packed_hop0 = !(getenv("TGMX_PACKED_HOP0") && atoi(getenv("TGMX_PACKED_HOP0")) == 0);
  const int gl = (a.grp.groups == 0 || packed_hop0) ? gl_any : 64;
  static const bool tile_on = !(getenv("TGMX_TILE") && atoi(getenv("TGMX_TILE")) == 0);
  const bool tile_ok = gl_any < 64 && tile_on && a.B <= 32 && a.k <= 32 && (((uintptr_t)a.out_nid | (uintptr_t)a.out_ts) & 15) == 0 &&
                       a.S <= (1ll << 25) && a.S >= 2ll * kWave * device_cu_count() &&
                       (!RING || (long long)a.N * a.B * (a.D > 0 ? a.D : 1) * 4 < (1ll << 32) - 64);
  if (tile_ok) {
    const int wpb = ride ? 4 : 1;
    const long long tiles = (a.S + kWave - 1) / kWave;
    long long tblocks = (tiles + wpb - 1) / wpb;
    if (a.leave_room && !ride) {
      const long long room = (long long)device_cu_count() * 12;
      if (tblocks > room) tblocks = room;
    }
    const dim3 tgrid((unsigned)tblocks + a.side_blocks + a.tail_blocks), tblock(wpb * kWave);
    const int bcap = a.B <= 10 ? 10 : (a.B <= 20 ? 20 : 32);
    static const bool coop_on = !(getenv("TGMX_TILE_COOP") && atoi(getenv("TGMX_TILE_COOP")) == 0);
    const bool coop = coop_on && bcap <= 20;
    const size_t tlds = (size_t)wpb * (kWave * a.k + kWave * a.k / 2 + kWave + (coop ? kWave * 7 : 0)) * sizeof(int);
#define TGMX_TILE_LAUNCH_K(KERNEL_, VEC_, BCAP_)                                                                                            \
  do {                                                                                                                                      \
    if (ride) {                                                                                                                             \
      if (tlds > 32 * 1024 && !lds_optin<KERNEL_<RING, VEC_, BCAP_, RING>>()) return TGMX_E_LAUNCH;                                          \
      TGMX_LAUNCH_TIMED((KERNEL_<RING, VEC_, BCAP_, RING>), tgrid, tblock, tlds, stream, ev_start, ev_stop, a, u);                           \
    } else {                                                                                                                                \
      if (tlds > 32 * 1024 && !lds_optin<KERNEL_<RING, VEC_, BCAP_, false>>()) return TGMX_E_LAUNCH;                                         \
      TGMX_LAUNCH_TIMED((KERNEL_<RING, VEC_, BCAP_, false>), tgrid, tblock, tlds, stream, ev_start, ev_stop, a, u);                          \
    }                                                                                                                                       \
  } while (0)
#define TGMX_TILE_LAUNCH(VEC_, BCAP_) TGMX_TILE_LAUNCH_K(lookup_tile_kernel, VEC_, BCAP_)
#define TGMX_TILE_VEC(VEC_)                                                           \
  do {                                                                                \
    if (bcap == 10 && coop) TGMX_TILE_LAUNCH_K(lookup_tile_coop_kernel, VEC_, 10);    \
    else if (bcap == 20 && coop) TGMX_TILE_LAUNCH_K(lookup_tile_coop_kernel, VEC_, 20); \
    else if (bcap == 10) TGMX_TILE_LAUNCH(VEC_, 10);                                  \
    else if (bcap == 20) TGMX_TILE_LAUNCH(VEC_, 20);                                  \
    else TGMX_TILE_LAUNCH(VEC_, 32);                                                  \
  } while (0)
    if (vec == 4) TGMX_TILE_VEC(4);
    else {
      if (vec == 2) {
        a.row_vecs = a.D;
        a.dv = make_fastdiv((uint32_t)a.row_vecs);
        a.dv_seed = make_fastdiv((uint32_t)(a.k * a.row_vecs));
      }
      TGMX_TILE_VEC(1);
    }
#undef TGMX_TILE_VEC
#undef TGMX_TILE_LAUNCH
#undef TGMX_TILE_LAUNCH_K
  } else if (gl < 64) {
    const int per_wave = 64 / gl;
    long long pblocks = ((a.S + per_wave - 1) / per_wave + waves_per_block - 1) / waves_per_block;
    if (pblocks > (1 << 20)) pblocks = 1 << 20;
    const dim3 pgrid((unsigned)pblocks + a.side_blocks + a.tail_blocks);
    const size_t plds = (size_t)waves_per_block * per_wave * a.k * sizeof(int);
#define TGMX_PACKED(VEC_)                                                                              \
  do {                                                                                                 \
    if (gl == 16 && ride) TGMX_LAUNCH_TIMED((lookup_packed_kernel<RING, VEC_, 16, true>), pgrid, block, plds, stream, ev_start, ev_stop, a, u); \
    else if (gl == 16) TGMX_LAUNCH_TIMED((lookup_packed_kernel<RING, VEC_, 16, false>), pgrid, block, plds, stream, ev_start, ev_stop, a, u);  \
    else if (ride) TGMX_LAUNCH_TIMED((lookup_packed_kernel<RING, VEC_, 32, true>), pgrid, block, plds, stream, ev_start, ev_stop, a, u);       \
    else TGMX_LAUNCH_TIMED((lookup_packed_kernel<RING, VEC_, 32, false>), pgrid, block, plds, stream, ev_start, ev_stop, a, u);                \
  } while (0)
    if (vec == 4) TGMX_PACKED(4);
    else if (vec == 2) TGMX_PACKED(2);
    else TGMX_PACKED(1);
#undef TGMX_PACKED
  } else if (small) {
    if (vec == 4) TGMX_LAUNCH(4, true);
    else if (vec == 2) TGMX_LAUNCH(2, true);
    else TGMX_LAUNCH(1, true);
  } else {
    if (vec == 4) TGMX_LAUNCH(4, false);
    else if (vec == 2) TGMX_LAUNCH(2, false);
    else TGMX_LAUNCH(1, false);
  }
#undef TGMX_LAUNCH
  TGMX_CHECK_LAUNCH("recency_lookup");
  return TGMX_OK;
}


template <bool RING>
static int launch_fused01(LookupArgs a, hipStream_t stream, hipEvent_t ev_start, hipEvent_t ev_stop, const UpdateArgs* side,
                          int side_stage, unsigned side_blocks, unsigned tail_blocks = 0) {
  const UpdateArgs u = side ? *side : UpdateArgs{};
  a.side_blocks = (RING && side) ? side_blocks : 0;
  a.side_stage = side_stage;
  a.tail_blocks = a.side_blocks ? tail_blocks : 0;
  const int kmax = a.k > a.k1 ? a.k : a.k1;
  const int vec = prepare_lookup(a, a.out_x1, kmax);
  if (vec < 0) return vec;
  const int waves_per_block = 4;
  const long long waves = a.S + a.S * a.k;
  long long blocks = (waves + waves_per_block - 1) / waves_per_block;
  if (blocks > (1 << 20)) blocks = 1 << 20;
  const dim3 grid((unsigned)blocks + a.side_blocks + a.tail_blocks), block(waves_per_block * kWave);
  const size_t lds = (size_t)waves_per_block * kmax * sizeof(int);
  const int pcap = !(RING && side) ? 1024 : ((side_stage != kSideAll && side_stage != kSideSortMergePlace) ? 0 : (u.m <= 512 ? 512 : 1024));
  if (vec == 4 && pcap == 512) TGMX_LAUNCH_TIMED((recency_lookup_fused01_kernel<RING, 4, RING ? 512 : 1024>), grid, block, lds, stream, ev_start, ev_stop, a, u);
  else if (vec == 4 && pcap == 0) TGMX_LAUNCH_TIMED((recency_lookup_fused01_kernel<RING, 4, RING ? 0 : 1024>), grid, block, lds, stream, ev_start, ev_stop, a, u);
  else if (vec == 4) TGMX_LAUNCH_TIMED((recency_lookup_fused01_kernel<RING, 4>), grid, block, lds, stream, ev_start, ev_stop, a, u);
  else if (vec == 2) TGMX_LAUNCH_TIMED((recency_lookup_fused01_kernel<RING, 2>), grid, block, lds, stream, ev_start, ev_stop, a, u);
  else TGMX_LAUNCH_TIMED((recency_lookup_fused01_kernel<RING, 1>), grid, block, lds, stream, ev_start, ev_stop, a, u);
  TGMX_CHECK_LAUNCH("recency_lookup_fused01");
  return TGMX_OK;
}


__global__ __launch_bounds__(256) void ring_update_span_kernel(const UpdateArgs a) {
  __shared__ long long red[256 / kWave];
  const long long per = (a.n + gridDim.x - 1) / gridDim.x;
  const long long lo = (long long)blockIdx.x * per, hi = lo + per < a.n ? lo + per : a.n;
  long long mx = -0x7fffffffffffffffLL;
  if (lo < hi) mx = strided_max_ts(a.ts + lo, hi - lo, threadIdx.x, 256);
  for (int off = 32; off > 0; off >>= 1) {
    const long long o = __shfl_xor(mx, off);
    mx = o > mx ? o : mx;
  }
  if ((threadIdx.x & 63) == 0) red[threadIdx.x >> 6] = mx;
  __syncthreads();
  if (threadIdx.x == 0) {
    for (int w = 1; w < 256 / kWave; ++w) mx = red[w] > mx ? red[w] : mx;
    if (lo < hi) atomicMax(a.span, mx + 1);
  }
}

__global__ __launch_bounds__(256) void ring_update_keys_kernel(const UpdateArgs a) {
  const long long j = (long long)blockIdx.x * blockDim.x + threadIdx.x;
  if (j >= a.m) return;
  int node, nbr;
  long long t, i;
  update_entry(a, j, node, nbr, t, i);
  const long long span = a.sorted_ts ? a.ts[a.n - 1] + 1 : *a.span;
  const long long key = update_key(node, t, span, a.key_wrap32);
  if (a.sorted_ts && i + 1 < a.n && a.ts[i + 1] < t) atomicOr(a.status, TGMX_ST_TS_BOUND);
  if (a.sort_bits < 64) {
    if (t < 0 || t > a.ts_bound) atomicOr(a.status, TGMX_ST_TS_BOUND);
    a.keys_in[j] = (unsigned long long)(a.key_wrap32 ? key + 2147483648LL : key);
  } else {
    a.keys_in[j] = (unsigned long long)key ^ 0x8000000000000000ull;
  }
  a.vals_in[j] = (unsigned)j;
}

__global__ __launch_bounds__(256) void ring_update_scatter_kernel(const UpdateArgs a) {
  const long long p = (long long)blockIdx.x * blockDim.x + threadIdx.x;
  if (p >= a.m) return;
  int node, nbr;
  long long t, i;
  update_entry(a, a.sorted_j[p], node, nbr, t, i);
  const bool valid = node >= 0 && node < a.N && nbr >= 0 && nbr < a.N;
  if (!valid) atomicOr(a.status, TGMX_ST_EDGE_RANGE);
  a.sorted_node[p] = valid ? node : -1;
}

__device__ __forceinline__ int global_hash_slot(int* keys, int hash_bits, int tgt, bool insert) {
// ... 146 lines not shown
  }
  if (kept > 0) {
    int32_t* wp = &a.write_pos[a.sorted_node[p]];
    const int old = atomicAdd(wp, kept);
    constexpr int kFold = 1 << 30;
    if (old < kFold && old + kept >= kFold) atomicSub(wp, kFold / a.B * a.B);
  }
  a.winner[p] = win;
}

__global__ __launch_bounds__(256) void ring_update_write_feat_kernel(const UpdateArgs a) {
  const long long p = (long long)blockIdx.x * (blockDim.x >> 6) + __builtin_amdgcn_readfirstlane((int)(threadIdx.x >> 6));
  if (p >= a.m) return;
  const bool first = lane_id() == 0;
  if (update_blocked(a)) {
    if (first) a.winner[p] = -1;
    return;
  }
  const int tgt = a.target[p];
  const int kept = a.winner[p];
  int win = -1;
  long long i = 0;
  if (tgt >= 0 && a.hash_maxp[global_hash_slot(a.hash_key, a.hash_bits, tgt, false)] == (int)p) {
    int nd, nbr;
    long long t;
    update_entry(a, a.sorted_j[p], nd, nbr, t, i);
    if (first) {
      Rec r;
      r.nbr = nbr;
      r.eid = a.eid0 >= 0 ? (int)(a.eid0 + i) : -1;
      r.ts = t;
      a.ring[tgt] = r;
    }
    win = tgt;
  }
  if (first) {
    if (kept > 0) commit_write_pos(&a.write_pos[a.sorted_node[p]], kept, a.B);
    a.winner[p] = win;
  }
  if (win < 0) return;
  float* __restrict__ o = a.ring_x + (long long)win * a.D;
  if (a.edge_x) {
    const float* __restrict__ x = a.edge_x + i * a.D;
    for (int c = lane_id(); c < a.D; c += kWave) o[c] = x[c];
  } else {
    for (int c = lane_id(); c < a.D; c += kWave) o[c] = 0.f;
  }
}

template <bool COMMIT>
__global__ __launch_bounds__(256) void ring_update_feat_kernel(const UpdateArgs a) {
  const long long p = (long long)blockIdx.x * (blockDim.x >> 6) + (threadIdx.x >> 6);
  if (p >= a.m) return;
  if (COMMIT && update_blocked(a)) return;
  const int row = a.winner[p];
  if constexpr (COMMIT) {
    if (lane_id() == 0) {
      const int kept = a.target[p];
      if (row >= 0) a.ring[row] = a.sorted_rec[p];
      if (kept > 0) commit_write_pos(&a.write_pos[a.sorted_node[p]], kept, a.B);
    }
  }
  if (row < 0 || a.D == 0) return;
  const long long j = a.sorted_j[p];
  const long long i = j >= a.n ? j - a.n : j;
  float* __restrict__ o = a.ring_x + (long long)row * a.D;
  if (a.edge_x) {
    const float* __restrict__ x = a.edge_x + i * a.D;
    for (int c = lane_id(); c < a.D; c += kWave) o[c] = x[c];
  } else {
    for (int c = lane_id(); c < a.D; c += kWave) o[c] = 0.f;
  }
}

__global__ __launch_bounds__(kChunk) void ring_update_chunk_sort_kernel(const UpdateArgs a) {
  __shared__ ChunkSortLds W;
  update_chunk_sort(a, blockIdx.x, W);
}

__global__ __launch_bounds__(kChunk) void ring_update_merge_kernel(const UpdateArgs a) {
  __shared__ long long k_all[kBlockMaxM];
  __shared__ int p_all[kBlockMaxM];
  const int m = (int)a.m;
  const int tid = threadIdx.x;
  for (int base = tid; base < m; base += 8 * kChunk) {
    long long kv[8];
    int pv[8];
#pragma unroll
    for (int u = 0; u < 8; ++u) {
      const int x = base + u * kChunk;
      kv[u] = x < m ? a.key[x] : 0;
      pv[u] = x < m ? a.node[x] : 0;
    }
#pragma unroll
    for (int u = 0; u < 8; ++u) {
      const int x = base + u * kChunk;
      if (x < m) {
        k_all[x] = kv[u];
        p_all[x] = pv[u];
      }
    }
  }
  __syncthreads();
  update_merge_entry<16>(a, k_all, p_all, blockIdx.x, tid);
}

static unsigned set_chunk_scratch(UpdateArgs& a, int32_t* scratch) {
  const unsigned chunks = (unsigned)((a.m + kChunk - 1) / kChunk);
  long long* s64 = reinterpret_cast<long long*>(((uintptr_t)(scratch + 4 * a.m) + 15) & ~(uintptr_t)15);
  a.key = s64;
  a.sorted_rec = reinterpret_cast<Rec*>(s64 + (long long)chunks * kChunk);
  a.node = reinterpret_cast<int32_t*>(a.sorted_rec + a.m);
  return chunks;
}

// ... 336 lines not shown
}

extern "C" size_t tgmx_ring_update_scratch_bytes(int64_t n, int32_t directed) {
  const long long m = directed ? n : 2 * n;
  constexpr size_t head = kScratchHead * sizeof(int32_t);
  if (m <= 0) return head + 256;
  if (m <= kBlockMaxM) return head + ((size_t)12 * m + 16) * sizeof(int32_t) + 256 + 12 * kChunk;
  LargeScratch w;
  if (large_scratch_layout(m, w)) return 0;
  return head + w.total;
}

extern "C" int tgmx_ring_update(tgmx_adj_t* ring, int32_t* write_pos, float* ring_x, int32_t D, int32_t B,
                                int32_t num_nodes, const int32_t* src, const int32_t* dst, const int64_t* ts,
                                const float* edge_x, int64_t n, int64_t eid0, int32_t directed, int32_t key_wrap32,
                                int32_t* scratch, int32_t* status, tgmx_stream_t stream) {
  TGMX_REQUIRE(n >= 0, "ring_update: bad sizes n=%lld", (long long)n);
  if (n == 0) return TGMX_OK;
  UpdateArgs a;
  const int rc = fill_update_args(a, ring, write_pos, ring_x, D, B, num_nodes, src, dst, ts, edge_x, n, eid0, directed,
                                  key_wrap32, scratch, status);
  if (rc) return rc;
  hipStream_t st = (hipStream_t)stream;
  if (a.m <= kBlockMaxM) launch_update_block(a, scratch + kScratchHead, st);
  else if (const int rl = launch_update_large(a, scratch + kScratchHead, st)) return rl;
  TGMX_CHECK_LAUNCH("ring_update");
  return TGMX_OK;
}

struct SideStream {
  hipStream_t stream = nullptr;
  hipEvent_t fork = nullptr, join = nullptr;
};
static SideStream* side_stream_for_current_device() {
  static SideStream side[64];
  static const bool off = getenv("TGMX_NO_SIDE_STREAM") != nullptr;
  int dev = 0;
  if (off || hipGetDevice(&dev) != hipSuccess || dev < 0 || dev >= 64) return nullptr;
  SideStream& s = side[dev];
  if (!s.stream) {
    int prio_lo = 0, prio_hi = 0;
    (void)hipDeviceGetStreamPriorityRange(&prio_lo, &prio_hi);
    static const bool no_prio = getenv("TGMX_SIDE_NO_PRIO") != nullptr;
    if (hipStreamCreateWithPriority(&s.stream, hipStreamNonBlocking, no_prio ? prio_lo : prio_hi) != hipSuccess) return nullptr;
    if (hipEventCreateWithFlags(&s.fork, hipEventDisableTiming) != hipSuccess ||
        hipEventCreateWithFlags(&s.join, hipEventDisableTiming) != hipSuccess) {
      s.stream = nullptr;
      return nullptr;
    }
  }
  return &s;
}

static bool plan_fuse01(const tgmx_recency_step_t* s, long long S0) {
  static const bool no_fuse = getenv("TGMX_NO_FUSE") != nullptr;
  static const bool no_ride = getenv("TGMX_NO_RIDE") != nullptr;
  if (no_fuse || s->n_hops < 2 || S0 <= 0 || s->B > kWave || s->k[0] <= 0 || s->k[1] <= 0) return false;
  if (s->indptr != nullptr && (long long)s->k[1] * s->D * 4 < 4096) return false;
  static const bool fuse_by_id = !(getenv("TGMX_FUSE_BY_ID") && atoi(getenv("TGMX_FUSE_BY_ID")) == 0);
  const bool by_id = s->out_eid[1] != nullptr && s->out_x[1] == nullptr;
  if (s->indptr == nullptr && !(by_id && fuse_by_id)) {
    LookupArgs a{};
    a.B = s->B; a.D = s->D; a.edge_x = s->ring_x; a.out_x = s->out_x[0];
    if (prepare_lookup(a, s->out_x[1], s->k[1]) < 0) return false;
    if (packed_group_lanes(a, s->k[1], true) < 64) return false;
  }
  const long long m = s->directed ? s->n : 2 * s->n;
  (void)no_ride;
  (void)m;
  return true;
}

extern "C" int tgmx_recency_step_plan(const tgmx_recency_step_t* s) {
  if (!s) return 0;
  long long S0 = s->S0;
  if (s->n_groups > 0) {
    S0 = 0;
    for (int g = 0; g < s->n_groups && g < TGMX_MAX_SEED_GROUPS; ++g) S0 += s->grp_n[g];
  }
  return plan_fuse01(s, S0) ? 1 : 0;
}

extern "C" int tgmx_recency_step(const tgmx_recency_step_t* s, tgmx_stream_t stream) {
  TGMX_REQUIRE(s, "recency_step: null argument block");
  TGMX_REQUIRE(s->n_groups >= 0 && s->n_groups <= TGMX_MAX_SEED_GROUPS && s->n_hops >= 0 && s->n_hops <= TGMX_MAX_HOPS,
               "recency_step: n_groups=%d n_hops=%d out of range", s->n_groups, s->n_hops);
  TGMX_REQUIRE(s->B > 0 && s->num_nodes > 0 && s->D >= 0 && s->n >= 0, "recency_step: bad sizes B=%d N=%d D=%d n=%lld", s->B,
               s->num_nodes, s->D, (long long)s->n);
  const bool csr = s->indptr != nullptr;
  TGMX_REQUIRE(s->ring && (csr || s->write_pos) && s->status, "recency_step: null state pointer");
  TGMX_REQUIRE(!csr || s->n == 0, "recency_step: the static index takes no update (n must be 0)");
  TGMX_REQUIRE(((uintptr_t)s->ring & 15) == 0, "recency_step: ring must be 16-byte aligned");
  TGMX_REQUIRE(csr || (long long)s->B * s->num_nodes < 2147483647LL, "recency_step: num_nodes*B overflows int32");
  hipStream_t st = (hipStream_t)stream;

  SeedGroups grp{};
  grp.gen = -1;
  long long S = s->S0;
  if (s->n_groups > 0) {
    S = 0;
    const int gen = s->neg_out ? s->neg_group : -1;
    TGMX_REQUIRE(gen < s->n_groups, "recency_step: neg_group=%d but %d seed groups", gen, s->n_groups);
    if (gen >= 0) {
      TGMX_REQUIRE(s->neg_low < s->neg_high && s->neg_time_out, "recency_step: generated negatives need low < high and neg_time_out");
      grp.gen = gen; grp.gen_low = s->neg_low; grp.gen_range = (unsigned)((long long)s->neg_high - s->neg_low);
      grp.gen_seed = s->neg_seed; grp.gen_call = s->neg_call; grp.gen_index0 = (unsigned long long)s->neg_index0; grp.gen_out = s->neg_out; grp.gen_out_ts = s->neg_time_out;
    }
    for (int g = 0; g < s->n_groups; ++g) {
      TGMX_REQUIRE(s->grp_n[g] >= 0 && (s->grp_n[g] == 0 || ((g == gen || s->grp_nid[g]) && s->grp_ts[g])), "recency_step: seed group %d", g);
      S += s->grp_n[g];
      grp.nid[g] = s->grp_nid[g]; grp.ts[g] = s->grp_ts[g]; grp.end[g] = S;
    }
    TGMX_REQUIRE(S == 0 || (s->seed_nid0 && s->seed_ts0), "recency_step: null hop-0 seed output");
    TGMX_REQUIRE(S == 0 || s->n_hops > 0, "recency_step: seed groups need at least one hop");
    grp.out_nid = s->seed_nid0; grp.out_ts = s->seed_ts0; grp.groups = s->n_groups;
  }

  UpdateArgs u{};
  unsigned side_chunks = 0;
  bool ride_place = false;
  if (s->n > 0) {
    const int rc = fill_update_args(u, s->ring, s->write_pos, s->ring_x, s->D, s->B, s->num_nodes, s->src, s->dst, s->ts,
                                    s->edge_x, s->n, s->eid0, s->directed, s->key_wrap32, s->scratch, s->status);
    if (rc) return rc;
    u.ts_bound = s->ts_bound;
    u.guard_mask = s->guard_seed_errors ? (TGMX_ST_SEED_RANGE | TGMX_ST_SEED_TIME) : 0;
    u.sorted_ts = s->sorted_ts;
    static const bool no_ride = getenv("TGMX_NO_RIDE") != nullptr;
    if (u.m <= kBlockMaxM && s->n_hops > 0 && S > 0 && !no_ride) side_chunks = set_chunk_scratch(u, s->scratch + kScratchHead);
    ride_place = side_chunks > 0 && u.m <= kRidePlaceMaxM && s->n_hops >= 2;
  }
  static const bool no_side_mid = getenv("TGMX_SIDE_MID") == nullptr;
  SideStream* mid = nullptr;
  if (side_chunks > 0 && !ride_place && u.m > kRidePlaceMaxM && !no_side_mid && (mid = side_stream_for_current_device()) != nullptr) {
    (void)hipEventRecord(mid->fork, st);
    (void)hipStreamWaitEvent(mid->stream, mid->fork, 0);
    launch_update_mid_front(u, side_chunks, mid->stream);
    (void)hipEventRecord(mid->join, mid->stream);
    side_chunks = 0;
  }
  static const bool use_tail = getenv("TGMX_TAIL") != nullptr;
  const unsigned tail_blocks = (ride_place && use_tail && s->n_hops == 2) ? (unsigned)((u.m + 3) / 4) : 0u;
  SideStream* side = nullptr;
  bool side_pending = false;
  if (s->n > 0 && u.m > kBlockMaxM && s->n_hops > 0 && S > 0 && (side = side_stream_for_current_device()) != nullptr) {
    (void)hipEventRecord(side->fork, st);
    (void)hipStreamWaitEvent(side->stream, side->fork, 0);
    side_pending = true;
  }
  auto enqueue_side = [&]() -> int {
    if (!side_pending) return TGMX_OK;
    side_pending = false;
    long long widest = S;
    for (int h = 0; h + 1 < s->n_hops; ++h) widest *= s->k[h];
    const bool saturating = widest >= 2ll * kWave * device_cu_count();
    if (const int rl = launch_update_large_front(u, s->scratch + kScratchHead, side->stream, saturating)) return rl;
    (void)hipEventRecord(side->join, side->stream);
    return TGMX_OK;
  };

  const int32_t* cur_n = s->seed_nid0;
  const int64_t* cur_t = s->seed_ts0;
  int h = 0;
  if (plan_fuse01(s, S)) {
    const int k0 = s->k[0], k1 = s->k[1];
    TGMX_REQUIRE(s->B >= k0 && s->B >= k1, "recency_step: k=[%d, %d] but B=%d", k0, k1, s->B);
    TGMX_REQUIRE(cur_n && cur_t && s->out_nid[0] && s->out_ts[0] && s->out_nid[1] && s->out_ts[1] &&
                     (s->D == 0 || (s->ring_x && (s->out_x[0] || s->out_eid[0]) && (s->out_x[1] || s->out_eid[1]))), "recency_step: null pointer at hop 0 / 1");
    LookupArgs a{};
    a.grp = grp;
    a.indptr = s->indptr; a.recs = reinterpret_cast<const Rec*>(s->ring); a.write_pos = s->write_pos; a.edge_x = s->ring_x;
    a.seeds = cur_n; a.qtimes = cur_t; a.out_nid = s->out_nid[0]; a.out_ts = s->out_ts[0]; a.out_x = s->out_x[0];
    a.k1 = k1; a.out_nid1 = s->out_nid[1]; a.out_ts1 = s->out_ts[1]; a.out_x1 = s->out_x[1];
    a.out_valid = s->out_valid[0]; a.out_valid1 = s->out_valid[1];
    a.out_valid_prev = s->out_valid_prev[0]; a.out_valid_prev1 = s->out_valid_prev[1];
    a.out_eid = s->out_eid[0]; a.out_eid1 = s->out_eid[1];
    a.status = s->status; a.S = S; a.D = s->D; a.k = k0; a.B = s->B; a.N = s->num_nodes; a.allow_pad = 0;
    a.ev_lo = s->ev_lo; a.ev_hi = s->ev_hi;
    a.x_by_pos = csr && s->csr_x_by_pos;
    const bool timed = s->timed_hop == 0 || s->timed_hop == 1;
    hipEvent_t e0 = timed ? (hipEvent_t)s->ev_start : nullptr, e1 = timed ? (hipEvent_t)s->ev_stop : nullptr;
    static const bool three_phase_on = !(getenv("TGMX_THREE_PHASE") && atoi(getenv("TGMX_THREE_PHASE")) == 0);
    const bool three_phase = three_phase_on && ride_place && u.m > 512 && !tail_blocks;
    const int rc = csr ? launch_fused01<false>(a, st, e0, e1, nullptr, 0, 0)
                       : launch_fused01<true>(a, st, e0, e1, side_chunks > 0 ? &u : nullptr,
                                              ride_place ? (three_phase ? kSideSortMergePlace : kSideAll) : kSideSortMerge,
                                              (ride_place && !three_phase) ? 1u : side_chunks, tail_blocks);
    if (rc) return rc;
    if (const int rs = enqueue_side()) return rs;
    cur_n = s->out_nid[1];
    cur_t = s->out_ts[1];
    S *= (long long)k0 * k1;
    h = 2;
  }
  for (; h < s->n_hops && S > 0; ++h) {
    const int k = s->k[h];
    TGMX_REQUIRE(k > 0 && s->B >= k, "recency_step: hop %d has k=%d, B=%d", h, k, s->B);
    TGMX_REQUIRE(cur_n && cur_t && s->out_nid[h] && s->out_ts[h] && (s->D == 0 || (s->ring_x && (s->out_x[h] || s->out_eid[h]))),
                 "recency_step: null pointer at hop %d", h);
    LookupArgs a{};
    if (h == 0) a.grp = grp;
    a.indptr = s->indptr; a.recs = reinterpret_cast<const Rec*>(s->ring); a.write_pos = s->write_pos; a.edge_x = s->ring_x;
    a.seeds = cur_n; a.qtimes = cur_t; a.out_nid = s->out_nid[h]; a.out_ts = s->out_ts[h]; a.out_x = s->out_x[h];
    a.out_valid = s->out_valid[h]; a.out_valid_prev = s->out_valid_prev[h];
    a.out_eid = s->out_eid[h];
    a.status = s->status; a.S = S; a.D = s->D; a.k = k; a.B = s->B; a.N = s->num_nodes; a.allow_pad = h > 0;
    a.ev_lo = s->ev_lo; a.ev_hi = s->ev_hi;
    a.cursor = csr ? reinterpret_cast<long long*>(s->csr_cursor) : nullptr;
    a.x_by_pos = csr && s->csr_x_by_pos;
    a.leave_room = side != nullptr;
    const bool timed = h == s->timed_hop;
    hipEvent_t e0 = timed ? (hipEvent_t)s->ev_start : nullptr, e1 = timed ? (hipEvent_t)s->ev_stop : nullptr;
    const bool ride = side_chunks > 0 && h < 2;
    static const bool split_merge_on = !(getenv("TGMX_SPLIT_MERGE") && atoi(getenv("TGMX_SPLIT_MERGE")) == 0);
    const bool split_merge = split_merge_on && ride_place && s->n_hops >= 2;
    static const bool merge_late_on = !(getenv("TGMX_MERGE_LATE") && atoi(getenv("TGMX_MERGE_LATE")) == 0);
    const bool merge_late = merge_late_on && split_merge && side_chunks > 1;
    const int stage = h == 0 ? ((split_merge && !merge_late) ? kSideSortMerge : kSideSort)
                             : (ride_place ? (merge_late ? kSideMergePlace : (split_merge ? kSidePlaceOnly : kSidePlace)) : kSideMerge);
    const int rc = csr ? launch_lookup<false>(a, st, e0, e1)
                       : launch_lookup<true>(a, st, e0, e1, ride ? &u : nullptr, stage,
                                             (h == 1 && ride_place && !merge_late) ? 1u : side_chunks, (h == 1 && ride_place) ? tail_blocks : 0u);
    if (rc) return rc;
    if (const int rs = enqueue_side()) return rs;
    cur_n = s->out_nid[h];
    cur_t = s->out_ts[h];
    S *= k;
  }
  if (const int rs = enqueue_side()) return rs;

  if (s->n > 0) {
    if (mid) {
      (void)hipStreamWaitEvent(st, mid->join, 0);
      hipLaunchKernelGGL(ring_update_feat_kernel<true>, dim3((unsigned)((u.m + 3) / 4)), dim3(256), 0, st, u);
    } else if (ride_place && tail_blocks) {
    } else if (ride_place) {
      hipLaunchKernelGGL(ring_update_feat_kernel<true>, dim3((unsigned)((u.m + 3) / 4)), dim3(256), 0, st, u);
    } else if (side_chunks > 0) {
      if (s->n_hops < 2) hipLaunchKernelGGL(ring_update_merge_kernel, dim3(side_chunks), dim3(kChunk), 0, st, u);
      launch_update_presorted(u, st);
    } else if (u.m <= kBlockMaxM) {
      launch_update_block(u, s->scratch + kScratchHead, st);
    } else if (side) {
      (void)hipStreamWaitEvent(st, side->join, 0);
      launch_update_large_back(u, st);
    } else if (const int rl = launch_update_large(u, s->scratch + kScratchHead, st)) {
      return rl;
    }
  }
  TGMX_CHECK_LAUNCH("recency_step");
  return TGMX_OK;
}

extern "C" int tgmx_ring_reset(tgmx_adj_t* ring, int32_t* write_pos, int32_t B, int32_t num_nodes,
                               tgmx_stream_t stream) {
  TGMX_REQUIRE(ring && write_pos && B > 0 && num_nodes > 0, "ring_reset: bad arguments");
  const long long nrec = (long long)B * num_nodes;
  long long blocks = (nrec + 255) / 256;
  if (blocks > 8192) blocks = 8192;
  hipLaunchKernelGGL(ring_reset_kernel, dim3((unsigned)blocks), dim3(256), 0, (hipStream_t)stream,
                     reinterpret_cast<Rec*>(ring), write_pos, nrec, num_nodes);
  TGMX_CHECK_LAUNCH("ring_reset");
  return TGMX_OK;
}
```

tgm_amd/hooks/recency.py:

```python
from __future__ import annotations

import logging
import warnings
from typing import Dict, List, Optional, Sequence

import torch
from torch import Tensor

from .. import _native
from ..core import DGBatch, DGraph
from ..index import TemporalCSR, build_csr
from .base import SeedableHook, StatefulHook
from .registry import hook

logger = logging.getLogger('tgm_amd.hooks.recency')

_ST_SEED_RANGE, _ST_SEED_TIME, _ST_EDGE_RANGE, _ST_SCRATCH, _ST_TS_BOUND = 1, 2, 4, 8, 16


class _NullCtx:
    def __enter__(self):
        return None

    def __exit__(self, *exc):
        return False


_NULL = _NullCtx()


def _on_device(device: torch.device):
    idx = device.index
    cur = _native._cuda_get_device
    if idx is None or idx == (cur() if cur is not None else torch.cuda.current_device()):
        return _NULL
    return torch.cuda.device(device)


@hook
class RecencyNeighborHook(StatefulHook, SeedableHook):

    _cls_requires = {'edge_src', 'edge_dst', 'edge_time'}
    _cls_produces = {'seed_nids', 'seed_times', 'nbr_nids', 'nbr_edge_time', 'nbr_edge_x', 'seed_node_nbr_mask'}

    def __init__(
        self,
        num_nodes: int,
        num_nbrs: List[int],
        seed_nodes_keys: List[str],
        seed_times_keys: List[str],
        directed: bool = False,
        id: Optional[str] = None,
        mode: str = 'ring',
        validate: str = 'sync',
        batch_size: Optional[int] = None,
        batch_starts: Optional[Sequence[int]] = None,
        key_arith: str = 'int32',
        adj_features: bool = True,
        edge_features: str = 'dense',
    ) -> None:
        super().__init__()
        if key_arith not in ('int32', 'int64'):
            raise ValueError(f"key_arith must be 'int32' or 'int64', got {key_arith!r}")
        self._key_wrap32 = 1 if key_arith == 'int32' else 0
        if edge_features not in ('dense', 'by_id'):
            raise ValueError(f"edge_features must be 'dense' or 'by_id', got {edge_features!r}")
        self._by_id = edge_features == 'by_id'
        self._adj_features = bool(adj_features)
        self._adj_features_max_bytes = 32 << 30
        if not len(num_nbrs):
            raise ValueError('num_nbrs must be non-empty')
        if not all(isinstance(x, int) and x > 0 for x in num_nbrs):
            raise ValueError('Each value in num_nbrs must be a positive integer')
        if len(seed_nodes_keys) != len(seed_times_keys):
            raise ValueError(
                f'len(seed_nodes_keys) ({len(seed_nodes_keys)}) != len(seed_times_keys) ({len(seed_times_keys)})\n'
                f'seed_nodes_keys={seed_nodes_keys}, seed_times_keys={seed_times_keys}'
            )
        if mode not in ('ring', 'csr'):
            raise ValueError(f"mode must be 'ring' or 'csr', got {mode!r}")
        if validate not in ('sync', 'deferred', 'off'):
            raise ValueError(f"validate must be 'sync', 'deferred' or 'off', got {validate!r}")
        if mode == 'csr' and batch_size is None and batch_starts is None:
            raise ValueError("mode='csr' needs the loader schedule: pass batch_size= or batch_starts=")

        self._num_nodes = int(num_nodes)
        self._num_nbrs = list(num_nbrs)
        self._max_nbrs = max(num_nbrs)
        self._directed = bool(directed)
        self._seed_nodes_keys = list(seed_nodes_keys)
        self._seed_times_keys = list(seed_times_keys)
        self._mode = mode
        self._validate = validate
        self._batch_size = batch_size
        self._batch_starts = batch_starts
        self._warned_seed_None = False
        self._warned_order = False
        self._last_batch_t = -(1 << 62)

        self._device: Optional[torch.device] = None
        self._edge_x_dim: Optional[int] = None
        self._ring: Optional[Tensor] = None
        self._ring_x: Optional[Tensor] = None
        self._write_pos: Optional[Tensor] = None
        self._scratch: Optional[Tensor] = None
        self._scratch_edges = 0
        self._status: Optional[Tensor] = None
        self._csr: Optional[TemporalCSR] = None
        self._csr_store = None
        self._csr_first = 0
        self._csr_bounds = None
        self._epoch_lo: Optional[int] = None

        self._step: Optional[_native.RecencyStep] = None
        self.profile_hop: Optional[int] = None
        self.profile_every: int = 1
        self.profile_log: List[tuple] = []
        self.profile_pool: List[_native.KernelTimer] = []
        self._calls = 0

        self._id = id
        self.seed_keys = list(seed_nodes_keys)
        self.__post_init__()

    @property
    def num_nbrs(self) -> List[int]:
        return self._num_nbrs

    @property
    def mode(self) -> str:
        return self._mode

    def reset_state(self) -> None:
        self._last_batch_t = -(1 << 62)
        self._warned_order = False
        if self._mode == 'ring':
            if self._ring is not None:
                lib = _native.load()
                with torch.cuda.device(self._device):
                    _native.check(
                        lib.tgmx_ring_reset(
                            self._ring.data_ptr(), self._write_pos.data_ptr(), self._max_nbrs, self._num_nodes, _native.stream_ptr()
                        ),
                        'tgmx_ring_reset',
                    )
        else:
            self._epoch_lo = None

    @property
    def batches_are_independent(self) -> bool:
        return self._mode == 'csr'

    def _anchor_epoch(self, first_edge: int) -> None:
        if self._mode == 'csr' and self._epoch_lo is None:
            self._epoch_lo = int(first_edge)

    def _refresh_ts_bound(self, dg: DGraph) -> None:
        store = getattr(dg, '_storage', None)
        self._bound_store = store
        bound = 0
        times = getattr(store, '_time_np', None)
        if times is not None and len(times) and int(times[0]) >= 0:
            bound = int(times[-1])
        self._store_promise = (bound, 1 if times is not None else 0)
        self._step.ts_bound, self._step.sorted_ts = self._store_promise

    def fuses_first_hops(self) -> bool:
        if self._step is None:
            return False
        return bool(_native.load().tgmx_recency_step_plan(self._step) & 1)

    def check(self) -> None:
        if self._status is None:
            return
        st = int(self._status.item())
        if st:
            self._status.zero_()
            self._raise_status(st)

    def _raise_status(self, st: int) -> None:
        if st & _ST_SEED_RANGE:
            raise ValueError(f'Seed nodes must satisfy 0 <= x < {self._num_nodes}')
        if st & _ST_SEED_TIME:
            raise ValueError('Seed times must be >= 0')
        if st & _ST_EDGE_RANGE:
            raise ValueError(f'Batch edge endpoints must satisfy 0 <= x < {self._num_nodes}')
        if st & _ST_TS_BOUND:
            raise RuntimeError('tgmx_recency_step: a batch timestamp lies outside [0, ts_bound], or the batch is not time-sorted (both promises come from the graph store)')
        if st & _ST_SCRATCH:
            raise RuntimeError('tgmx_recency_step: the update scratch was not zero-initialised (internal error)')

    def _warn_rings_under_world(self) -> None:
        try:
            import torch.distributed as dist

            world = dist.get_world_size() if (dist.is_available() and dist.is_initialized()) else 1
        except Exception:
            world = 1
        if world > 1 and not getattr(RecencyNeighborHook, '_warned_world', False):
            RecencyNeighborHook._warned_world = True
            warnings.warn(
                f"RecencyNeighborHook(mode='ring') under torch.distributed (world size {world}): every rank replays the whole global batch's "
                "ring update, which does not shrink with the number of GPUs.  For multi-GPU jobs build the static index instead -- "
                "RecencyNeighborHook(..., mode='csr', batch_size=<loader batch size>): same sampled neighbours, no per-batch state, and whole "
                'batches can be dealt to ranks with DGDataLoader(batch_shard=(rank, world)).  (INTEGRATION.md section 4)',
                UserWarning, stacklevel=3)

    def _ensure_state(self, dg: DGraph, device: torch.device) -> None:
        if self._edge_x_dim is None:
            self._edge_x_dim = dg.edge_x_dim or 0
        if self._device == device and self._status is not None:
            return
        if device.type != 'cuda':
            raise _native.NativeLibraryError(
                f'RecencyNeighborHook got a batch on {device}; tgm_amd kernels run only on a ROCm device '
                "(no CPU fallback). Create the DGraph with device='cuda'."
            )
        _native.load()
        N, B, D = self._num_nodes, self._max_nbrs, self._edge_x_dim
        old = self._device
        self._device = device
        if self._status is None or old != device:
            self._status = torch.zeros(1, dtype=torch.int32, device=device)
        if self._mode == 'ring':
            if self._ring is None:
                self._warn_rings_under_world()
                self._ring = torch.empty((N * B, 2), dtype=torch.int64, device=device)
                self._ring_x = torch.empty((N * B, max(D, 1)), dtype=torch.float32, device=device) if D else None
                self._write_pos = torch.empty(N, dtype=torch.int32, device=device)
                self.reset_state()
            elif old != device:
                self._ring = self._ring.to(device)
                self._ring_x = None if self._ring_x is None else self._ring_x.to(device)
                self._write_pos = self._write_pos.to(device)
                self._scratch = None
                self._scratch_edges = 0
        st = _native.RecencyStep()
        if self._mode == 'ring':
            st.ring, st.write_pos, st.ring_x = self._ring.data_ptr(), self._write_pos.data_ptr(), _native.ptr(self._ring_x)
        else:
            self._csr = None
        st.D, st.B, st.num_nodes = D, B, N
        for hop, k in enumerate(self._num_nbrs[: _native.MAX_HOPS]):
            st.k[hop] = k
        st.directed, st.key_wrap32 = (1 if self._directed else 0), self._key_wrap32
        st.status = self._status.data_ptr()
        st.timed_hop = -1
        self._new_empty = tuple(torch.empty(0, dtype=t, device=device).new_empty for t in (torch.int32, torch.int64, torch.float32))
        self._step = st
        self._bound_store = None
        self._refresh_ts_bound(dg)

    def _ensure_csr(self, dg: DGraph, first_edge: int) -> TemporalCSR:
        store = dg._storage
        if self._csr is None or self._csr_store is not store or self._csr.device != self._device:
            arr = store.on(self._device)
            first = self._epoch_lo if self._epoch_lo is not None else (first_edge or 0)
            self._csr_first = first
            self._csr_bounds = None if self._batch_starts is None else frozenset(int(b) for b in self._batch_starts)
            self._csr = build_csr(
                arr.src,
                arr.dst,
                arr.ts,
                self._num_nodes,
                batch_starts=self._batch_starts,
                batch_size=self._batch_size,
                first_edge=first,
                directed=self._directed,
            )
            self._csr_store = store
            st = self._step
            st.indptr, st.ring, st.ring_x = self._csr.indptr.data_ptr(), self._csr.adj.data_ptr(), _native.ptr(arr.edge_x)
            self._csr_adj_x = None
            st.csr_x_by_pos = 0
            want = arr.edge_x is not None and self._adj_features and not self._by_id
            if want:
                nbytes = self._csr.adj.shape[0] * (arr.edge_x.shape[1] * 4 + 8)
                free = torch.cuda.mem_get_info(self._device)[0]
                want = nbytes <= self._adj_features_max_bytes and nbytes <= free // 2
            if want:
                try:
                    eid = self._csr.records()[1].to(torch.int64)
                    self._csr_adj_x = arr.edge_x.index_select(0, eid)
                    del eid
                    st.ring_x, st.csr_x_by_pos = self._csr_adj_x.data_ptr(), 1
                except torch.OutOfMemoryError:
                    self._csr_adj_x = None
                    st.ring_x, st.csr_x_by_pos = _native.ptr(arr.edge_x), 0
            self._csr_cursor = torch.zeros(self._num_nodes, dtype=torch.int64, device=self._device)
            st.csr_cursor = self._csr_cursor.data_ptr()
        return self._csr

    def _check_csr_boundary(self, ev_hi: int) -> None:
        if self._csr_bounds is not None:
            ok = ev_hi in self._csr_bounds or ev_hi >= self._csr.num_edges
        else:
            ok = ev_hi >= self._csr_first and (ev_hi - self._csr_first) % self._batch_size == 0 or ev_hi >= self._csr.num_edges
        if not ok:
            raise ValueError(
                f"mode='csr': the batch starts at edge {ev_hi}, which is not a boundary of the schedule the index was built for "
                f'(first edge {self._csr_first}, ' + (f'batch_size {self._batch_size}' if self._csr_bounds is None else 'explicit batch_starts')
                + "). Build the hook with this loader's batch_size / batch_starts, or use mode='ring'."
            )

    def _ensure_scratch(self, n_edges: int, device: torch.device) -> None:
        if n_edges > self._scratch_edges:
            need = int(_native.load().tgmx_ring_update_scratch_bytes(n_edges, 1 if self._directed else 0))
            if need == 0:
                _native.check(-2, 'tgmx_ring_update_scratch_bytes')
            self._scratch = torch.zeros(need, dtype=torch.uint8, device=device)
            self._scratch_edges = n_edges
            self._step.scratch = self._scratch.data_ptr()

    def _is_store_slice(self, batch: DGBatch, tt: Tensor, device: torch.device) -> bool:
        lo, store = batch._edge_lo, self._bound_store
        if lo is None or store is None or not hasattr(store, 'on'):
            return False
        base = store.on(device).ts
        return tt.data_ptr() == base.data_ptr() + 8 * int(lo) and lo + tt.shape[0] <= base.shape[0]

    def _note_batch_time(self, dg: DGraph, batch: DGBatch) -> None:
        lo = batch._event_lo
        store = getattr(dg, '_storage', None)
        times = getattr(store, '_time_np', None)
        if lo is None or times is None or lo >= len(times):
            return
        t0 = int(times[lo])
        if t0 < self._last_batch_t and not self._warned_order:
            self._warned_order = True
            logger.warning(
                f'RecencyNeighborHook: this batch starts at t={t0}, behind the previous batch (t={self._last_batch_t}). '
                'Results may be incomplete or incorrect. This hook assumes queries are processed in chronological order: '
                '(1) the dataloader must return batches sorted by timestamp, (2) batches must not be shuffled, '
                '(3) reset the hook state between datasets / epochs / evaluation runs.'
            )
        self._last_batch_t = t0

    def __call__(self, dg: DGraph, batch: DGBatch) -> DGBatch:
        return self._call_step(dg, batch, batch.edge_src.device)

    def _publish(self, batch: DGBatch, seed_n, seed_t, out_n, out_t, out_x, seed_mask) -> DGBatch:
        from ..core.lazy import EdgeFeaturesById, SampledHops, SamplerCallTag

        tag = SamplerCallTag(out_n, out_t, out_x)
        if isinstance(out_x, EdgeFeaturesById):
            out_x.tag = tag
        else:
            out_x = SampledHops(out_x, tag)
        self.add_batch_attribute(batch, 'seed_nids', SampledHops(seed_n, tag))
        self.add_batch_attribute(batch, 'seed_times', SampledHops(seed_t, tag))
        self.add_batch_attribute(batch, 'nbr_nids', SampledHops(out_n, tag))
        self.add_batch_attribute(batch, 'nbr_edge_time', SampledHops(out_t, tag))
        self.add_batch_attribute(batch, 'nbr_edge_x', out_x)
        self.add_batch_attribute(batch, 'seed_node_nbr_mask', seed_mask)
        return batch

    def _call_step(self, dg: DGraph, batch: DGBatch, device: torch.device) -> DGBatch:
        groups, group_times, seed_mask = self._get_seed_tensors(batch, device, concat=False)
        S0 = 0
        for g in groups:
# ... 30 lines not shown
                self._ensure_csr(dg, ev_hi)
                self._check_csr_boundary(ev_hi)
                if self._epoch_lo is None:
                    self._epoch_lo = ev_hi
                st.ev_lo, st.ev_hi = self._epoch_lo, ev_hi
            ne32, ne64, nef = self._new_empty
            seeds = ne32(S0)
            seed_times = ne64(S0)
            for g, (a, t) in enumerate(zip(groups, group_times)):
                if not a.is_contiguous():
                    a = a.contiguous()
                if not t.is_contiguous():
                    t = t.contiguous()
                if t.shape[0] != a.shape[0]:
                    raise ValueError(f'seed group {g}: {a.shape[0]} nodes but {t.shape[0]} times')
                st.grp_nid[g], st.grp_ts[g], st.grp_n[g] = a.data_ptr(), t.data_ptr(), a.shape[0]
            st.n_groups = len(groups)
            st.seed_nid0, st.seed_ts0 = seeds.data_ptr(), seed_times.data_ptr()

            out_seed_n, out_seed_t, out_n, out_t, out_x = [], [], [], [], []
            cur_n, cur_t, S = seeds, seed_times, S0
            by_id = self._by_id and D > 0
            if by_id and ring_mode and batch._edge_lo is None:
                raise ValueError("edge_features='by_id' needs batches materialized from the graph store (their edges carry store ids)")
            out_eid = []
            for hop, k in enumerate(self._num_nbrs):
                nid = ne32((S, k))
                nts = ne64((S, k))
                if by_id:
                    nx = None
                    out_eid.append(ne32((S, k)))
                    st.out_eid[hop] = out_eid[-1].data_ptr()
                else:
                    nx = nef((S, k, D))
                    st.out_eid[hop] = 0
                st.out_nid[hop], st.out_ts[hop], st.out_x[hop] = nid.data_ptr(), nts.data_ptr(), _native.ptr(nx)
                out_seed_n.append(cur_n)
                out_seed_t.append(cur_t)
                out_n.append(nid)
                out_t.append(nts)
                out_x.append(nx)
                cur_n, cur_t = nid.view(-1), nts.view(-1)
                S *= k

            self._calls += 1
            timer = None
            st.timed_hop = -1
            if self.profile_hop is not None and self._calls % self.profile_every == 0 and self.profile_pool:
                timer = self.profile_pool.pop()
                st.timed_hop, st.ev_start, st.ev_stop = self.profile_hop, timer.start, timer.stop

            n_edges = batch.edge_src.shape[0] if ring_mode else 0
            keep = None
            if n_edges:
                self._ensure_scratch(n_edges, device)
                ex = batch.edge_x
                if ex is not None and D:
                    if ex.dtype != torch.float32 or not ex.is_contiguous():
                        ex = ex.to(torch.float32).contiguous()
                else:
                    ex = None
                src, dst, tt = batch.edge_src, batch.edge_dst, batch.edge_time
                if not (src.is_contiguous() and dst.is_contiguous() and tt.is_contiguous()):
                    src, dst, tt = src.contiguous(), dst.contiguous(), tt.contiguous()
                keep = (src, dst, tt, ex)
                st.src, st.dst, st.ts, st.edge_x = src.data_ptr(), dst.data_ptr(), tt.data_ptr(), _native.ptr(ex)
                st.eid0 = -1 if batch._edge_lo is None else int(batch._edge_lo)
                st.ts_bound, st.sorted_ts = self._store_promise if self._is_store_slice(batch, tt, device) else (0, 0)

            st.n, st.n_hops = n_edges, L
            st.guard_seed_errors = 1 if self._validate == 'sync' else 0
            rc = lib.tgmx_recency_step(st, stream)
            if rc:
                _native.check(rc, 'tgmx_recency_step')
            if self._validate == 'sync':
                self.check()
            del keep
            if timer is not None:
                hops = [0, 1] if self.profile_hop in (0, 1) and self.fuses_first_hops() else [self.profile_hop]
                counts = torch.empty(len(hops), dtype=torch.int64, device=device)
                for i, h in enumerate(hops):
                    torch.sum((out_n[h] != -1).view(-1), dim=0, dtype=torch.int64, out=counts[i])
                self.profile_log.append((timer, [(out_seed_n[h].shape[0], self._num_nbrs[h]) for h in hops], counts, None))
        if by_id:
            from ..core.lazy import EdgeFeaturesById

            out_x = EdgeFeaturesById(out_eid, self._feature_table(dg, device))
        return self._publish(batch, out_seed_n, out_seed_t, out_n, out_t, out_x, seed_mask)

    def _feature_table(self, dg: DGraph, device: torch.device) -> Tensor:
        return dg._storage.on(device).edge_x

    def _get_seed_tensors(self, batch: DGBatch, device: torch.device, concat: bool = True):
        seeds: List[Tensor] = []
        times: List[Tensor] = []
        mask: Dict[str, Tensor] = {}
        offset = 0
        for node_attr, time_attr in zip(self._seed_nodes_keys, self._seed_times_keys):
            missing = [a for a in (node_attr, time_attr) if not hasattr(batch, a)]
            if missing:
                raise ValueError(f'Missing seed attributes {missing} on batch')
            seed, time = getattr(batch, node_attr), getattr(batch, time_attr)
            skip = False
            for name, tensor in ((node_attr, seed), (time_attr, time)):
                if tensor is None:
                    if not self._warned_seed_None:
                        warnings.warn(
                            f'Seed attribute {name} is None on this batch, skipping this batch. '
                            'Future occurrences will also be skipped but the warning will be suppressed',
                            UserWarning,
                        )
                        self._warned_seed_None = True
                    skip = True
                    break
                if not isinstance(tensor, Tensor):
                    raise ValueError(f'{name} must be a Tensor, got {type(tensor)}')
                if tensor.ndim != 1:
                    raise ValueError(f'{name} must be 1-D, got shape {tensor.shape}')
            if skip:
                continue
            if device.type != 'cuda' and self._validate != 'off' and seed.numel():
# ... 31 lines not shown
```

tgm_amd/pipeline.py:

```python
from __future__ import annotations

import ctypes
import os
import sys
from typing import Dict, List, Optional, Sequence

import torch

from . import _native
from .core import DGBatch, DGraph
from .dist import EdgeShardHook, shard_bounds
from .hooks.dedup import DeduplicationHook
from .hooks.edge_list import SampledEdgeListHook
from .hooks.negatives import RandomNegativeEdgeSamplerHook
from .hooks.recency import RecencyNeighborHook

_ROLE_KEYS = {
    False: {'edge_src': (_native.SEED_SRC, 'edge_time'), 'edge_dst': (_native.SEED_DST, 'edge_time'), 'neg': (_native.SEED_NEG, 'neg_time')},
    True: {'shard_src': (_native.SEED_SRC, 'shard_time'), 'shard_dst': (_native.SEED_DST, 'shard_time'), 'neg': (_native.SEED_NEG, 'neg_time')},
}


_STATUS_READ_EVERY = 512
_TAGGED = frozenset(('seed_nids', 'seed_times', 'nbr_nids', 'nbr_edge_time', 'nbr_edge_x'))
_MAX_AUTO_SETS = 4
_storage_uses = torch._C._storage_Use_Count


def _snapshot(tensors: list) -> list:
    return [(sys.getrefcount(t), t._use_count()) for t in tensors]


class _Slot:

    __slots__ = ('out', 'attrs', 'nbr_nids', 'post', 'post_bufs', 'valid', 'watch', 'base')


class _OutputSet:

    __slots__ = ('buf', 'cap', 'off', 'views', 'storage', 'uses', 'version', 'pin', 'event', 'arange_n', 'lib', 'stream')

    def __del__(self) -> None:
        ev, lib = getattr(self, 'event', None), getattr(self, 'lib', None)
        if ev and lib is not None:
            try:
                lib.tgmx_event_destroy(ev)
            except Exception:
                pass


class CompiledPipeline:
    def __init__(self, dg: DGraph, shard: Optional[EdgeShardHook], neg: Optional[RandomNegativeEdgeSamplerHook],
                 nbr: RecencyNeighborHook, n_lowered: int, pool: Optional[int], dedup: Optional[DeduplicationHook] = None,
                 edges: Optional[SampledEdgeListHook] = None) -> None:
        self.n_lowered = n_lowered
        self._dedup, self._edges = dedup, edges
        self._dedup_ws = None
# ... 31 lines not shown
            if h._id is None and h.neg_ratio == 1.0 and (h._like, h._time_key) == want:
                neg = h
                i += 1
        if i >= len(hooks) or type(hooks[i]) is not RecencyNeighborHook:
            return None
        nbr = hooks[i]
        keys = _ROLE_KEYS[shard is not None]
        ok = (
            nbr._id is None
            and len(nbr._num_nbrs) <= _native.MAX_HOPS
            and 1 <= len(nbr._seed_nodes_keys) <= _native.MAX_SEED_GROUPS
            and all(k in keys and keys[k][1] == t for k, t in zip(nbr._seed_nodes_keys, nbr._seed_times_keys))
            and (neg is not None) == ('neg' in nbr._seed_nodes_keys)
            and nbr._seed_nodes_keys.count('neg') <= 1
        )
        if not ok:
            return None
        i += 1
        dedup = edges = None
        if i < len(hooks) and type(hooks[i]) is DeduplicationHook and hooks[i]._id is None:
            extra = set(hooks[i].seed_keys or [])
            if extra <= {'neg', 'nbr_nids'} and ('neg' not in extra or neg is not None) and len(nbr._num_nbrs) + 3 <= 16:
                dedup = hooks[i]
                i += 1
                if i < len(hooks) and type(hooks[i]) is SampledEdgeListHook and hooks[i]._id is None and hooks[i].hop < len(nbr._num_nbrs):
                    edges = hooks[i]
                    i += 1
        return CompiledPipeline(dg, shard, neg, nbr, i, pool, dedup, edges)

    def _bind(self) -> None:
        nbr, arr = self._nbr, self._arr
        nbr._ensure_state(self._dg, self._device)
        if getattr(nbr, '_bound_store', None) is not getattr(self._dg, '_storage', None):
            nbr._refresh_ts_bound(self._dg)
        p = _native.Pipeline()
        p.src, p.dst, p.ts, p.edge_x = arr.src.data_ptr(), arr.dst.data_ptr(), arr.ts.data_ptr(), _native.ptr(arr.edge_x)
        p.num_edges = arr.src.shape[0]
        p.rank, p.world = (self._shard.rank, self._shard.world_size) if self._shard is not None else (0, 1)
        p.n_roles = len(self._roles)
        for g, r in enumerate(self._roles):
            p.seed_role[g] = r
        if self._neg is not None:
            neg = self._neg
            if neg._rng_seed is None:
                neg._rng_seed = (neg._seed if neg._seed is not None else torch.initial_seed()) & 0xFFFFFFFFFFFFFFFF
            p.neg_low, p.neg_high, p.neg_seed = neg.low, neg.high, neg._rng_seed
        p.update = 1 if nbr._mode == 'ring' else 0
        ctypes.memmove(ctypes.byref(p.step), ctypes.byref(nbr._step), ctypes.sizeof(_native.RecencyStep))
        p.step.n_hops = len(nbr._num_nbrs)
        p.step.guard_seed_errors = 1 if nbr._validate == 'sync' else 0
        p.step.ts_bound, p.step.sorted_ts = nbr._store_promise
        self._pipe, self._step_ref = p, nbr._step
        self._scratch_ptr = nbr._step.scratch

    def _share(self, n: int) -> int:
        lo, hi = shard_bounds(n, *((self._shard.rank, self._shard.world_size) if self._shard is not None else (0, 1)))
        return hi - lo

    def _layout(self, cap: int) -> tuple:
        nbr = self._nbr
        D = nbr._edge_x_dim
        world = self._shard.world_size if self._shard is not None else 1
        share = -(-cap // world)
        S0 = share * len(self._roles)
        off: Dict[str, int] = {}
        pos = 0

        def take(name: str, nbytes: int) -> None:
            nonlocal pos
            off[name] = pos
            pos = (pos + nbytes + 255) & ~255

        take('neg', 4 * share)
        take('neg_time', 8 * share)
        take('seeds', 4 * S0)
        take('seed_t', 8 * S0)
        take('arange', 8 * S0)
        S = S0
        total_ids = 0
        for hop, k in enumerate(nbr._num_nbrs):
            take(f'nid{hop}', 4 * S * k)
            take(f'nts{hop}', 8 * S * k)
            take(f'nx{hop}', 0 if nbr._by_id else 4 * S * k * D)
            take(f'eid{hop}', 4 * S * k if nbr._by_id else 0)
            take(f'nv{hop}', 4 * S)
            take(f'nvp{hop}', 4 * S)
            total_ids += S * k
            S *= k
        if self._dedup is not None:
            N = int(self._dg._storage.num_nodes_global)
            extra = set(self._dedup.seed_keys or [])
            total = 2 * cap + (share if 'neg' in extra else 0) + (total_ids if 'nbr_nids' in extra else 0)
            take('uniq', 4 * max(min(total, N), 1))
            take('dev_sizes', 24)
            if self._edges is not None:
                h = self._edges.hop
                Sh = S0
                for k in nbr._num_nbrs[:h]:
                    Sh *= k
                ecap = max(Sh * nbr._num_nbrs[h], 1)
                take('ei', 16 * ecap)
                take('et', 8 * ecap)
                take('ex', 4 * ecap * D)
                take('ro', 8 * (Sh + 1))
        return off, pos, S0

# ... 361 lines not shown
```

Measured before the change: 8.351 billion.

## Defer ring-buffer commit to next step instead of in-kernel tail barrier

Replaces the in-kernel tail-commit phase, where tail blocks spin-waited on a grid-wide barrier before writing ring records and write positions, with a deferred commit. The current update is staged into pending header, record and slot buffers tagged with a stamp. The next step's fused kernel commits those staged entries in dedicated commit blocks while lookups read through the pending overlay. A host-side flush runs before any external access to the ring tensors. This removes the spin barrier and its serialization, at the cost of extra overlay reads on every lookup, more state and more complex consistency rules. It is on by default through an environment variable.

```diff
diff --git a/include/tgm_amd.h b/include/tgm_amd.h
--- a/include/tgm_amd.h
+++ b/include/tgm_amd.h
@@ -116,10 +116,19 @@
   int64_t* csr_cursor;
   int32_t csr_x_by_pos;
   int32_t* out_eid[TGMX_MAX_HOPS];
+  struct tgmx_defer* defer;
+  int32_t defer_ok;
 } tgmx_recency_step_t;
 
 int tgmx_recency_step(const tgmx_recency_step_t* step, tgmx_stream_t stream);
 int tgmx_recency_step_plan(const tgmx_recency_step_t* step);
+
+typedef struct tgmx_defer tgmx_defer_t;
+tgmx_defer_t* tgmx_defer_create(int32_t num_nodes, int32_t B);
+void tgmx_defer_destroy(tgmx_defer_t* d);
+int tgmx_defer_pending(const tgmx_defer_t* d);
+int64_t tgmx_defer_count(const tgmx_defer_t* d);
+int tgmx_defer_flush(tgmx_defer_t* d, tgmx_stream_t stream);
 
 #define TGMX_SEED_SRC 0
 #define TGMX_SEED_DST 1
diff --git a/tgm_amd/_native.py b/tgm_amd/_native.py
--- a/tgm_amd/_native.py
+++ b/tgm_amd/_native.py
@@ -167,6 +167,7 @@
         ('guard_seed_errors', c_int32), ('sorted_ts', c_int32),
         ('out_valid', c_void_p * MAX_HOPS), ('out_valid_prev', c_void_p * MAX_HOPS),
         ('neg_index0', c_int64), ('csr_cursor', c_void_p), ('csr_x_by_pos', c_int32), ('out_eid', c_void_p * MAX_HOPS),
+        ('defer', c_void_p), ('defer_ok', c_int32),
     ]
 
 
@@ -281,6 +282,11 @@
 SIGNATURES['tgmx_uniform_lookup_csr'] = (c_int32, [_P, _P, _P, c_int32, _P, c_int64, c_int32, c_int64, c_int32, c_int32, ctypes.c_uint64, ctypes.c_uint64,
                                                    _P, _P, _P, _P, _P])
 SIGNATURES['tgmx_ring_update_scratch_bytes'] = (c_size_t, [c_int64, c_int32])
+SIGNATURES['tgmx_defer_create'] = (c_void_p, [c_int32, c_int32])
+SIGNATURES['tgmx_defer_destroy'] = (None, [_P])
+SIGNATURES['tgmx_defer_pending'] = (c_int32, [_P])
+SIGNATURES['tgmx_defer_count'] = (c_int64, [_P])
+SIGNATURES['tgmx_defer_flush'] = (c_int32, [_P, _P])
 SIGNATURES['tgmx_tgn_gru_gate_backward'] = (c_int32, [_P, _P, _P, _P, c_int32, c_int64, _P, _P, _P])
 SIGNATURES['tgmx_tgn_aggregate_backward'] = (c_int32, [c_int64, _P, _P, _P, _P, _P, _P, c_int32, c_int32, _P, _P, c_int32, c_int32, _P, _P, _P])
 SIGNATURES['tgmx_tconv_edge_attr_backward'] = (c_int32, [_P, _P, _P, _P, _P, _P, c_int32, c_int32, c_int64, _P, _P])
diff --git a/tgm_amd/csrc/pipeline.hip b/tgm_amd/csrc/pipeline.hip
--- a/tgm_amd/csrc/pipeline.hip
+++ b/tgm_amd/csrc/pipeline.hip
@@ -115,6 +115,7 @@
     s.edge_x = (p->edge_x && s.D > 0) ? p->edge_x + edge_lo * (long long)s.D : nullptr;
     s.n = n_edges;
     s.eid0 = edge_lo;
+    s.defer_ok = 1;
   } else {
     s.n = 0;
   }
diff --git a/tgm_amd/csrc/recency.hip b/tgm_amd/csrc/recency.hip
--- a/tgm_amd/csrc/recency.hip
+++ b/tgm_amd/csrc/recency.hip
@@ -61,7 +61,13 @@
   int leave_room;
   unsigned side_blocks;
   int side_stage;
-  unsigned tail_blocks;
+  unsigned commit_blocks;
+  const unsigned long long* phdr;
+  const Rec* prec;
+  const int32_t* pslot;
+  const float* pstore;
+  unsigned pstamp;
+  int peid0;
   int k1;
   int32_t* out_nid1;
   int64_t* out_ts1;
@@ -150,6 +156,11 @@
   int guard_mask;
   long long n, m, eid0;
   int B, N, D, key_wrap32;
+  unsigned long long* dhdr;
+  Rec* drec;
+  int32_t* dslot;
+  const unsigned long long* phdr;
+  unsigned dstamp, pstamp;
 };
 
 __device__ __forceinline__ long long update_key(int node, long long t, long long span, int wrap32) {
@@ -219,10 +230,31 @@
   return a.guard_mask != 0 && (__hip_atomic_load(a.status, __ATOMIC_RELAXED, __HIP_MEMORY_SCOPE_AGENT) & a.guard_mask) != 0;
 }
 
+constexpr int kFold = 1 << 30;
 __device__ __forceinline__ void commit_write_pos(int32_t* wp, int kept, int B) {
   const int old = atomicAdd(wp, kept);
-  constexpr int kFold = 1 << 30;
   if (old < kFold && old + kept >= kFold) atomicSub(wp, kFold / B * B);
+}
+__device__ __forceinline__ int fold_add(int old, int kept, int B) {
+  return (old < kFold && old + kept >= kFold) ? old + kept - kFold / B * B : old + kept;
+}
+
+__device__ __forceinline__ int logical_wp(const int32_t* write_pos, const unsigned long long* phdr, unsigned pstamp, int n) {
+  const int wp = write_pos[n];
+  const unsigned long long h = phdr ? phdr[n] : 0ull;
+  return (phdr && (unsigned)(h >> 32) == pstamp) ? (int)(unsigned)h : wp;
+}
+
+__device__ __forceinline__ void publish_wp(const UpdateArgs& a, int n, int w0, int kept) {
+  unsigned long long* hp = &a.dhdr[n];
+  unsigned long long cur = __hip_atomic_load(hp, __ATOMIC_RELAXED, __HIP_MEMORY_SCOPE_AGENT);
+  for (;;) {
+    const int base = (unsigned)(cur >> 32) == a.dstamp ? (int)(unsigned)cur : w0;
+    const unsigned long long nv = ((unsigned long long)a.dstamp << 32) | (unsigned)fold_add(base, kept, a.B);
+    const unsigned long long prev = atomicCAS(hp, cur, nv);
+    if (prev == cur) break;
+    cur = prev;
+  }
 }
 
 template <int MAXM>
@@ -409,6 +441,13 @@
       if (h_maxp[hs[r]] == p) {
         Rec rec;
         if constexpr (DEFER) {
+          if (a.drec) {
+            const long long* src = reinterpret_cast<const long long*>(&a.sorted_rec[p]);
+            long long* dst = reinterpret_cast<long long*>(&a.drec[tgt[r]]);
+            dst[0] = COH ? ld_agent(&src[0]) : src[0];
+            dst[1] = COH ? ld_agent(&src[1]) : src[1];
+            a.dslot[tgt[r]] = (int32_t)a.dstamp;
+          }
         } else if constexpr (PRESORTED) {
           rec = a.sorted_rec[p];
         } else {
@@ -428,6 +467,8 @@
         kept = cnt[r] > a.B ? a.B : cnt[r];
         if constexpr (!DEFER) {
           if (!blocked) commit_write_pos(&a.write_pos[node[r]], kept, a.B);
+        } else {
+          if (a.dhdr) publish_wp(a, node[r], w[r], kept);
         }
       }
     }
@@ -638,7 +679,7 @@
 #pragma unroll
   for (int q = 0; q < NE; ++q) {
     valid[q] = act[q] && node[q] >= 0 && node[q] < a.N && nbr[q] >= 0 && nbr[q] < a.N;
-    w[q] = valid[q] ? a.write_pos[node[q]] : 0;
+    w[q] = valid[q] ? logical_wp(a.write_pos, a.phdr, a.pstamp, node[q]) : 0;
   }
 #pragma unroll
   for (int q = 0; q < NE; ++q) {
@@ -654,13 +695,16 @@
     if constexpr (COH) {
       st_agent(&a.sorted_j[rank], pay[q]);
       st_agent(&a.sorted_node[rank], valid[q] ? node[q] : -1);
-      st_agent(&a.target[rank], w[q] % a.B);
+      st_agent(&a.target[rank], w[q]);
+      long long* rd = reinterpret_cast<long long*>(&a.sorted_rec[rank]);
+      st_agent(&rd[0], *reinterpret_cast<const long long*>(&rec));
+      st_agent(&rd[1], rec.ts);
     } else {
       a.sorted_j[rank] = pay[q];
       a.sorted_node[rank] = valid[q] ? node[q] : -1;
-      a.target[rank] = w[q] % a.B;
-    }
-    a.sorted_rec[rank] = rec;
+      a.target[rank] = w[q];
+      a.sorted_rec[rank] = rec;
+    }
   }
 }
 
@@ -692,108 +736,32 @@
 }
 constexpr int kRidePlaceMaxM = 1024;
 
-constexpr int kTailGroups = 32;
-__device__ __forceinline__ void tail_signal(int32_t* bar, bool publish, unsigned bid, unsigned nblk) {
-  __syncthreads();
-  if (threadIdx.x == 0) {
-    if (publish) {
-      __threadfence();
-      __hip_atomic_store(&bar[4], 1, __ATOMIC_RELAXED, __HIP_MEMORY_SCOPE_AGENT);
-      __hip_atomic_fetch_add(&bar[2], 1, __ATOMIC_RELAXED, __HIP_MEMORY_SCOPE_AGENT);
-    } else {
-      const unsigned g = bid % kTailGroups;
-      const unsigned size = (nblk - g + kTailGroups - 1) / kTailGroups;
-      int32_t* cnt = &bar[16 + 16 * g];
-      const int prev = __hip_atomic_fetch_add(cnt, 1, __ATOMIC_RELAXED, __HIP_MEMORY_SCOPE_AGENT);
-      if (prev == (int)size - 1) {
-        __hip_atomic_store(cnt, 0, __ATOMIC_RELAXED, __HIP_MEMORY_SCOPE_AGENT);
-        __hip_atomic_fetch_add(&bar[2], (int)size, __ATOMIC_RELAXED, __HIP_MEMORY_SCOPE_AGENT);
-      }
-    }
-  }
-}
-
-__device__ __forceinline__ bool tail_wait(const int32_t* word, unsigned need) {
-  int spins = 0;
-  while ((unsigned)__hip_atomic_load(word, __ATOMIC_RELAXED, __HIP_MEMORY_SCOPE_AGENT) < need) {
-    __builtin_amdgcn_s_sleep(8);
-    if (++spins > (1 << 22)) return false;
-  }
-  return true;
-}
-
-__device__ __forceinline__ void tail_commit(const UpdateArgs& a, unsigned tb, unsigned tail_blocks, unsigned need) {
-  __shared__ int ok_s;
-  const int lane = lane_id();
-  const long long p = (long long)tb * (blockDim.x >> 6) + (threadIdx.x >> 6);
-  if (threadIdx.x == 0) ok_s = tail_wait(&a.barrier[4], 1u) ? 1 : 0;
-  __syncthreads();
-  bool ok = ok_s != 0;
-  int row = -1, kept = 0, node = 0;
-  long long rec_lo = 0, rec_hi = 0;
-  constexpr int kMaxCols = 8;
-  float xv[kMaxCols];
-  const float* x = nullptr;
-  const bool wide = a.D > kMaxCols * kWave;
-  if (ok && p < a.m) {
-    row = ld_agent(&a.winner[p]);
-    kept = ld_agent(&a.target[p]);
-    if (row >= 0) {
-      const long long* src = reinterpret_cast<const long long*>(&a.sorted_rec[p]);
-      rec_lo = ld_agent(&src[0]);
-      rec_hi = ld_agent(&src[1]);
-    }
-    if (kept > 0) node = ld_agent(&a.sorted_node[p]);
-    if (row >= 0 && a.D > 0 && a.edge_x) {
-      const long long j = ld_agent(&a.sorted_j[p]);
-      x = a.edge_x + (j >= a.n ? j - a.n : j) * a.D;
-      if (!wide) {
-#pragma unroll
-        for (int u = 0; u < kMaxCols; ++u) {
-          const int c = lane + u * kWave;
-          xv[u] = c < a.D ? x[c] : 0.f;
-        }
-      }
-    }
-  }
-  if (threadIdx.x == 0) ok_s = (ok && tail_wait(&a.barrier[2], need)) ? 1 : 0;
-  __syncthreads();
-  ok = ok_s != 0;
-  if (!ok) {
-    if (threadIdx.x == 0) atomicOr(a.status, TGMX_ST_SCRATCH);
-  } else if (p < a.m && !update_blocked(a)) {
-    if (lane == 0) {
-      if (row >= 0) {
-        long long* dst = reinterpret_cast<long long*>(&a.ring[row]);
-        dst[0] = rec_lo;
-        dst[1] = rec_hi;
-      }
-      if (kept > 0) commit_write_pos(&a.write_pos[node], kept, a.B);
-    }
-    if (row >= 0 && a.D > 0) {
-      float* __restrict__ o = a.ring_x + (long long)row * a.D;
-      if (!x) {
-        for (int c = lane; c < a.D; c += kWave) o[c] = 0.f;
-      } else if (wide) {
-        for (int c = lane; c < a.D; c += kWave) o[c] = x[c];
-      } else {
-#pragma unroll
-        for (int u = 0; u < kMaxCols; ++u) {
-          const int c = lane + u * kWave;
-          if (c < a.D) o[c] = xv[u];
-        }
-      }
-    }
-  }
-  __syncthreads();
-  if (threadIdx.x == 0) {
-    const int prev = __hip_atomic_fetch_add(&a.barrier[3], 1, __ATOMIC_RELAXED, __HIP_MEMORY_SCOPE_AGENT);
-    if (prev == (int)tail_blocks - 1) {
-      __hip_atomic_store(&a.barrier[2], 0, __ATOMIC_RELAXED, __HIP_MEMORY_SCOPE_AGENT);
-      __hip_atomic_store(&a.barrier[3], 0, __ATOMIC_RELAXED, __HIP_MEMORY_SCOPE_AGENT);
-      __hip_atomic_store(&a.barrier[4], 0, __ATOMIC_RELAXED, __HIP_MEMORY_SCOPE_AGENT);
-    }
-  }
+__device__ __forceinline__ void commit_position(const UpdateArgs& a, long long p) {
+  const int row = a.winner[p];
+  if (lane_id() == 0) {
+    const int kept = a.target[p];
+    if (row >= 0) a.ring[row] = a.sorted_rec[p];
+    if (kept > 0) {
+      const int n = a.sorted_node[p];
+      if (a.dhdr) a.write_pos[n] = (int)(unsigned)a.dhdr[n];
+      else commit_write_pos(&a.write_pos[n], kept, a.B);
+    }
+  }
+  if (row < 0 || a.D == 0) return;
+  const long long j = a.sorted_j[p];
+  const long long i = j >= a.n ? j - a.n : j;
+  float* __restrict__ o = a.ring_x + (long long)row * a.D;
+  if (a.edge_x) {
+    const float* __restrict__ x = a.edge_x + i * a.D;
+    for (int c = lane_id(); c < a.D; c += kWave) o[c] = x[c];
+  } else {
+    for (int c = lane_id(); c < a.D; c += kWave) o[c] = 0.f;
+  }
+}
+
+__device__ __forceinline__ void commit_block(const UpdateArgs& c, unsigned cb) {
+  const long long p = (long long)cb * (blockDim.x >> 6) + (threadIdx.x >> 6);
+  if (p < c.m) commit_position(c, p);
 }
 
 template <int PCAP>
@@ -961,7 +929,7 @@
   if (live) {
     if (RING) {
       w.w0 = (long long)n * a.B;
-      w.wrot = a.write_pos[n] % a.B;
+      w.wrot = logical_wp(a.write_pos, a.phdr, a.pstamp, n) % a.B;
       w.wlen = a.B;
     } else {
       const long long ra = a.indptr[n], rz = a.indptr[n + 1];
@@ -996,13 +964,29 @@
   const Window w = find_window<RING>(a, n, live, lane);
   Rec r;
   r.nbr = -1; r.eid = 0; r.ts = 0;
+  int src = -1;
   if (RING) {
-    if (live && lane < B) r = a.recs[(long long)n * B + lane];
+    const long long row = (long long)n * B + lane;
+    Rec pr;
+    int ps = 0;
+    if (live && lane < B) {
+      r = a.recs[row];
+      if (a.phdr) {
+        pr = a.prec[row];
+        ps = a.pslot[row];
+      }
+    }
+    src = (int)row;
+    if (a.phdr && live && lane < B && (unsigned)ps == a.pstamp) {
+      r = pr;
+      src = a.pstore ? a.N * B + (r.eid - a.peid0) : -1;
+    }
     int from_slot = w.wrot + lane;
     if (from_slot >= B) from_slot -= B;
     if (lane >= B) from_slot = lane;
     r.nbr = __shfl(r.nbr, from_slot);
     r.ts = __shfl(r.ts, from_slot);
+    src = __shfl(src, from_slot);
     if (a.out_eid || a.out_eid1) r.eid = __shfl(r.eid, from_slot);
   } else if (lane < w.wlen) {
     r = a.recs[slot_of<RING>(w, B, lane)];
@@ -1015,11 +999,12 @@
   const int g_nbr = __shfl(r.nbr, from);
   const int g_eid = __shfl(r.eid, from);
   const long long g_ts = __shfl(r.ts, from);
+  const int g_src = RING ? __shfl(src, from) : 0;
   SmallPick o;
   o.has = i >= 0 && g_nbr >= 0;
   o.nbr = o.has ? g_nbr : -1;
   o.ts = o.has ? g_ts : 0;
-  o.src = o.has ? ((RING || a.x_by_pos) ? (int)slot_of<RING>(w, B, from) : g_eid) : -1;
+  o.src = o.has ? (RING ? g_src : (a.x_by_pos ? (int)slot_of<RING>(w, B, from) : g_eid)) : -1;
   o.eid = o.has ? g_eid : -1;
   return o;
 }
@@ -1028,11 +1013,13 @@
 __device__ __forceinline__ void gather_rows(const LookupArgs& a, long long s, int k, int lane, const int* lds_eid, float* out_x, int first_slot) {
   using V = typename VecOf<VEC>::type;
   const V* __restrict__ X = reinterpret_cast<const V*>(a.edge_x);
+  const int lim = a.pstore ? a.N * a.B : 0x7fffffff;
+  const V* __restrict__ P = a.pstore ? reinterpret_cast<const V*>(a.pstore) : X;
   V* __restrict__ O = reinterpret_cast<V*>(out_x + s * (long long)k * a.D);
   const int total = k * a.row_vecs;
   constexpr int U = 8;
   for (int f0 = first_slot * a.row_vecs + lane; f0 < total; f0 += kWave * U) {
-    long long idx[U];
+    const V* ptr[U];
     bool has[U];
 #pragma unroll
     for (int u = 0; u < U; ++u) {
@@ -1042,11 +1029,12 @@
       const int col = fc - slot * a.row_vecs;
       const int e = lds_eid[slot];
       has[u] = e >= 0;
-      idx[u] = has[u] ? (long long)e * a.row_vecs + col : 0;
+      const bool st = e >= lim;
+      ptr[u] = (st ? P : X) + (has[u] ? (long long)(st ? e - lim : e) * a.row_vecs + col : 0);
     }
     V v[U];
 #pragma unroll
-    for (int u = 0; u < U; ++u) v[u] = X[idx[u]];
+    for (int u = 0; u < U; ++u) v[u] = *ptr[u];
 #pragma unroll
     for (int u = 0; u < U; ++u) {
       const int f = f0 + u * kWave;
@@ -1125,15 +1113,10 @@
   if constexpr (RING && RIDE) {
     if (bid < a.side_blocks) {
       update_side_work(u, a.side_stage, (int)bid);
-      if (a.tail_blocks) tail_signal(u.barrier, true, 0, 0);
       return;
     }
     bid -= a.side_blocks;
-    nblk -= a.side_blocks + a.tail_blocks;
-    if (bid >= nblk) {
-      tail_commit(u, bid - nblk, a.tail_blocks, nblk + a.side_blocks);
-      return;
-    }
+    nblk -= a.side_blocks;
   }
   const int lane = lane_id();
   const int wave_in_block = threadIdx.x >> 6;
@@ -1146,27 +1129,24 @@
     check_seed(a, n, q, a.allow_pad, lane);
     lookup_seed<RING, VEC, SMALL>(a, s, n, q, a.k, lane, lds_eid, a.out_nid, a.out_ts, a.out_x, a.out_valid, a.out_valid_prev, a.out_eid);
   }
-  if constexpr (RING && RIDE) {
-    if (a.tail_blocks) tail_signal(u.barrier, false, bid, nblk);
-  }
 }
 
 template <bool RING, int VEC, int PCAP = kRidePlaceMaxM>
-__global__ __launch_bounds__(256) void recency_lookup_fused01_kernel(const LookupArgs a, const UpdateArgs u) {
+__global__ __launch_bounds__(256) void recency_lookup_fused01_kernel(const LookupArgs a, const UpdateArgs u, const UpdateArgs c) {
   extern __shared__ __attribute__((aligned(16))) int lds_eid_all[];
   unsigned bid = blockIdx.x, nblk = gridDim.x;
   if constexpr (RING) {
     if (bid < a.side_blocks) {
       update_side_work<PCAP>(u, a.side_stage, (int)bid);
-      if (a.tail_blocks) tail_signal(u.barrier, true, 0, 0);
       return;
     }
     bid -= a.side_blocks;
-    nblk -= a.side_blocks + a.tail_blocks;
-    if (bid >= nblk) {
-      tail_commit(u, bid - nblk, a.tail_blocks, nblk + a.side_blocks);
+    if (bid < a.commit_blocks) {
+      commit_block(c, bid);
       return;
     }
+    bid -= a.commit_blocks;
+    nblk -= a.side_blocks + a.commit_blocks;
   }
   const int lane = lane_id();
   const int wave_in_block = threadIdx.x >> 6;
@@ -1194,9 +1174,6 @@
       lookup_seed<RING, VEC, true>(a, idx, n, q, k1, lane, lds_eid, a.out_nid1, a.out_ts1, a.out_x1, a.out_valid1, a.out_valid_prev1, a.out_eid1);
     }
   }
-  if constexpr (RING) {
-    if (a.tail_blocks) tail_signal(u.barrier, false, bid, nblk);
-  }
 }
 
 struct GroupPick {
@@ -1311,15 +1288,10 @@
   if constexpr (RING && RIDE) {
     if (bid < a.side_blocks) {
       update_side_work(u, a.side_stage, (int)bid);
-      if (a.tail_blocks) tail_signal(u.barrier, true, 0, 0);
       return;
     }
     bid -= a.side_blocks;
-    nblk -= a.side_blocks + a.tail_blocks;
-    if (bid >= nblk) {
-      tail_commit(u, bid - nblk, a.tail_blocks, nblk + a.side_blocks);
-      return;
-    }
+    nblk -= a.side_blocks;
   }
   const int lane = lane_id();
   const int sub = lane / GL, gl = lane - sub * GL;
@@ -1350,9 +1322,6 @@
     const GroupPick o = group_pick<RING, GL>(a, n, q, k, n >= 0 && n < a.N, gl, sub);
     group_emit<VEC, GL>(a, act, s, k, o, lds_eid, gl, sub, a.out_nid, a.out_ts, a.out_x, a.out_valid, a.out_valid_prev);
   }
-  if constexpr (RING && RIDE) {
-    if (a.tail_blocks) tail_signal(u.barrier, false, bid, nblk);
-  }
 }
 
 
@@ -1488,15 +1457,10 @@
   if constexpr (RING && RIDE) {
     if (bid < a.side_blocks) {
       update_side_work(u, a.side_stage, (int)bid);
-      if (a.tail_blocks) tail_signal(u.barrier, true, 0, 0);
       return;
     }
     bid -= a.side_blocks;
-    nblk -= a.side_blocks + a.tail_blocks;
-    if (bid >= nblk) {
-      tail_commit(u, bid - nblk, a.tail_blocks, nblk + a.side_blocks);
-      return;
-    }
+    nblk -= a.side_blocks;
   }
   const int lane = lane_id();
   const int wave_in_block = threadIdx.x >> 6, wpb = blockDim.x >> 6;
@@ -1639,9 +1603,6 @@
     }
     __builtin_amdgcn_wave_barrier();
   }
-  if constexpr (RING && RIDE) {
-    if (a.tail_blocks) tail_signal(u.barrier, false, bid, nblk);
-  }
 }
 
 template <bool RING, int VEC, int BCAP, bool RIDE>
@@ -1653,15 +1614,10 @@
   if constexpr (RING && RIDE) {
     if (bid < a.side_blocks) {
       update_side_work(u, a.side_stage, (int)bid);
-      if (a.tail_blocks) tail_signal(u.barrier, true, 0, 0);
       return;
     }
     bid -= a.side_blocks;
-    nblk -= a.side_blocks + a.tail_blocks;
-    if (bid >= nblk) {
-      tail_commit(u, bid - nblk, a.tail_blocks, nblk + a.side_blocks);
-      return;
-    }
+    nblk -= a.side_blocks;
   }
   const int lane = lane_id();
   const int wave_in_block = threadIdx.x >> 6, wpb = blockDim.x >> 6;
@@ -1844,9 +1800,6 @@
     }
     __builtin_amdgcn_wave_barrier();
   }
-  if constexpr (RING && RIDE) {
-    if (a.tail_blocks) tail_signal(u.barrier, false, bid, nblk);
-  }
 }
 
 template <auto Kernel>
@@ -1907,19 +1860,18 @@
 
 template <bool RING>
 static int launch_lookup(LookupArgs a, hipStream_t stream, hipEvent_t ev_start, hipEvent_t ev_stop,
-                         const UpdateArgs* side = nullptr, int side_stage = 0, unsigned side_blocks = 0, unsigned tail_blocks = 0) {
+                         const UpdateArgs* side = nullptr, int side_stage = 0, unsigned side_blocks = 0) {
   if (a.S == 0) return TGMX_OK;
   const UpdateArgs u = side ? *side : UpdateArgs{};
   a.side_blocks = (RING && side) ? side_blocks : 0;
   a.side_stage = side_stage;
-  a.tail_blocks = a.side_blocks ? tail_blocks : 0;
   const bool small = a.B <= kWave && a.k <= kWave;
   const int vec = prepare_lookup(a, a.out_x, a.k);
   if (vec < 0) return vec;
   const int waves_per_block = 4;
   long long blocks = (a.S + waves_per_block - 1) / waves_per_block;
   if (blocks > (1 << 20)) blocks = 1 << 20;
-  const dim3 grid((unsigned)blocks + a.side_blocks + a.tail_blocks), block(waves_per_block * kWave);
+  const dim3 grid((unsigned)blocks + a.side_blocks), block(waves_per_block * kWave);
   const size_t lds = (size_t)waves_per_block * a.k * sizeof(int);
   const bool ride = RING && a.side_blocks > 0;
 #define TGMX_LAUNCH(VEC_, SMALL_)                                                                                              \
@@ -1942,7 +1894,7 @@
       const long long room = (long long)device_cu_count() * 12;
       if (tblocks > room) tblocks = room;
     }
-    const dim3 tgrid((unsigned)tblocks + a.side_blocks + a.tail_blocks), tblock(wpb * kWave);
+    const dim3 tgrid((unsigned)tblocks + a.side_blocks), tblock(wpb * kWave);
     const int bcap = a.B <= 10 ? 10 : (a.B <= 20 ? 20 : 32);
     static const bool coop_on = !(getenv("TGMX_TILE_COOP") && atoi(getenv("TGMX_TILE_COOP")) == 0);
     const bool coop = coop_on && bcap <= 20;
@@ -1982,7 +1934,7 @@
     const int per_wave = 64 / gl;
     long long pblocks = ((a.S + per_wave - 1) / per_wave + waves_per_block - 1) / waves_per_block;
     if (pblocks > (1 << 20)) pblocks = 1 << 20;
-    const dim3 pgrid((unsigned)pblocks + a.side_blocks + a.tail_blocks);
+    const dim3 pgrid((unsigned)pblocks + a.side_blocks);
     const size_t plds = (size_t)waves_per_block * per_wave * a.k * sizeof(int);
 #define TGMX_PACKED(VEC_)                                                                              \
   do {                                                                                                 \
@@ -2012,11 +1964,12 @@
 
 template <bool RING>
 static int launch_fused01(LookupArgs a, hipStream_t stream, hipEvent_t ev_start, hipEvent_t ev_stop, const UpdateArgs* side,
-                          int side_stage, unsigned side_blocks, unsigned tail_blocks = 0) {
+                          int side_stage, unsigned side_blocks, const UpdateArgs* commit = nullptr) {
   const UpdateArgs u = side ? *side : UpdateArgs{};
+  const UpdateArgs c = (RING && commit) ? *commit : UpdateArgs{};
   a.side_blocks = (RING && side) ? side_blocks : 0;
   a.side_stage = side_stage;
-  a.tail_blocks = a.side_blocks ? tail_blocks : 0;
+  a.commit_blocks = (RING && commit) ? (unsigned)((c.m + 3) / 4) : 0u;
   const int kmax = a.k > a.k1 ? a.k : a.k1;
   const int vec = prepare_lookup(a, a.out_x1, kmax);
   if (vec < 0) return vec;
@@ -2024,14 +1977,14 @@
   const long long waves = a.S + a.S * a.k;
   long long blocks = (waves + waves_per_block - 1) / waves_per_block;
   if (blocks > (1 << 20)) blocks = 1 << 20;
-  const dim3 grid((unsigned)blocks + a.side_blocks + a.tail_blocks), block(waves_per_block * kWave);
+  const dim3 grid((unsigned)blocks + a.side_blocks + a.commit_blocks), block(waves_per_block * kWave);
   const size_t lds = (size_t)waves_per_block * kmax * sizeof(int);
   const int pcap = !(RING && side) ? 1024 : ((side_stage != kSideAll && side_stage != kSideSortMergePlace) ? 0 : (u.m <= 512 ? 512 : 1024));
-  if (vec == 4 && pcap == 512) TGMX_LAUNCH_TIMED((recency_lookup_fused01_kernel<RING, 4, RING ? 512 : 1024>), grid, block, lds, stream, ev_start, ev_stop, a, u);
-  else if (vec == 4 && pcap == 0) TGMX_LAUNCH_TIMED((recency_lookup_fused01_kernel<RING, 4, RING ? 0 : 1024>), grid, block, lds, stream, ev_start, ev_stop, a, u);
-  else if (vec == 4) TGMX_LAUNCH_TIMED((recency_lookup_fused01_kernel<RING, 4>), grid, block, lds, stream, ev_start, ev_stop, a, u);
-  else if (vec == 2) TGMX_LAUNCH_TIMED((recency_lookup_fused01_kernel<RING, 2>), grid, block, lds, stream, ev_start, ev_stop, a, u);
-  else TGMX_LAUNCH_TIMED((recency_lookup_fused01_kernel<RING, 1>), grid, block, lds, stream, ev_start, ev_stop, a, u);
+  if (vec == 4 && pcap == 512) TGMX_LAUNCH_TIMED((recency_lookup_fused01_kernel<RING, 4, RING ? 512 : 1024>), grid, block, lds, stream, ev_start, ev_stop, a, u, c);
+  else if (vec == 4 && pcap == 0) TGMX_LAUNCH_TIMED((recency_lookup_fused01_kernel<RING, 4, RING ? 0 : 1024>), grid, block, lds, stream, ev_start, ev_stop, a, u, c);
+  else if (vec == 4) TGMX_LAUNCH_TIMED((recency_lookup_fused01_kernel<RING, 4>), grid, block, lds, stream, ev_start, ev_stop, a, u, c);
+  else if (vec == 2) TGMX_LAUNCH_TIMED((recency_lookup_fused01_kernel<RING, 2>), grid, block, lds, stream, ev_start, ev_stop, a, u, c);
+  else TGMX_LAUNCH_TIMED((recency_lookup_fused01_kernel<RING, 1>), grid, block, lds, stream, ev_start, ev_stop, a, u, c);
   TGMX_CHECK_LAUNCH("recency_lookup_fused01");
   return TGMX_OK;
 }
@@ -2284,15 +2237,11 @@
 __global__ __launch_bounds__(256) void ring_update_feat_kernel(const UpdateArgs a) {
   const long long p = (long long)blockIdx.x * (blockDim.x >> 6) + (threadIdx.x >> 6);
   if (p >= a.m) return;
-  if (COMMIT && update_blocked(a)) return;
+  if constexpr (COMMIT) {
+    if (!update_blocked(a)) commit_position(a, p);
+    return;
+  }
   const int row = a.winner[p];
-  if constexpr (COMMIT) {
-    if (lane_id() == 0) {
-      const int kept = a.target[p];
-      if (row >= 0) a.ring[row] = a.sorted_rec[p];
-      if (kept > 0) commit_write_pos(&a.write_pos[a.sorted_node[p]], kept, a.B);
-    }
-  }
   if (row < 0 || a.D == 0) return;
   const long long j = a.sorted_j[p];
   const long long i = j >= a.n ? j - a.n : j;
@@ -2735,9 +2684,79 @@
   return &s;
 }
 
+struct tgmx_defer {
+  int N, B;
+  void* mem;
+  unsigned long long* hdr[2];
+  Rec* rec[2];
+  int32_t* slot[2];
+  int32_t* scratch[2];
+  unsigned stamp;
+  bool pending;
+  long long deferred;
+  UpdateArgs pend;
+};
+
+extern "C" tgmx_defer_t* tgmx_defer_create(int32_t num_nodes, int32_t B) {
+  if (num_nodes <= 0 || B <= 0) {
+    set_error("defer_create: bad arguments");
+    return nullptr;
+  }
+  auto* d = new tgmx_defer{};
+  d->N = num_nodes;
+  d->B = B;
+  return d;
+}
+
+extern "C" void tgmx_defer_destroy(tgmx_defer_t* d) {
+  if (d && d->mem) (void)hipFree(d->mem);
+  delete d;
+}
+
+static int defer_buffers(tgmx_defer* d, hipStream_t st) {
+  if (d->mem) return TGMX_OK;
+  auto up = [](size_t x) { return (x + 255) & ~(size_t)255; };
+  const size_t nb = (size_t)d->N * d->B;
+  const size_t half = up(tgmx_ring_update_scratch_bytes(kRidePlaceMaxM, 1));
+  const size_t o_scr = up((size_t)16 * d->N), o_slot = o_scr + 2 * half, o_rec = up(o_slot + 8 * nb), total = o_rec + 32 * nb;
+  void* mem = nullptr;
+  if (hipMalloc(&mem, total) != hipSuccess) {
+    set_error("recency_step: cannot allocate %zu bytes for the deferred commit", total);
+    return TGMX_E_LAUNCH;
+  }
+  (void)hipMemsetAsync(mem, 0, o_rec, st);
+  char* base = static_cast<char*>(mem);
+  d->mem = mem;
+  for (int q = 0; q < 2; ++q) {
+    d->hdr[q] = reinterpret_cast<unsigned long long*>(base) + (size_t)q * d->N;
+    d->scratch[q] = reinterpret_cast<int32_t*>(base + o_scr + q * half);
+    d->slot[q] = reinterpret_cast<int32_t*>(base + o_slot) + q * nb;
+    d->rec[q] = reinterpret_cast<Rec*>(base + o_rec) + q * nb;
+  }
+  return TGMX_OK;
+}
+
+extern "C" int tgmx_defer_pending(const tgmx_defer_t* d) { return d && d->pending ? 1 : 0; }
+
+extern "C" int64_t tgmx_defer_count(const tgmx_defer_t* d) { return d ? d->deferred : 0; }
+
+extern "C" int tgmx_defer_flush(tgmx_defer_t* d, tgmx_stream_t stream) {
+  TGMX_REQUIRE(d, "defer_flush: null state");
+  if (!d->pending) return TGMX_OK;
+  d->pending = false;
+  hipLaunchKernelGGL(ring_update_feat_kernel<true>, dim3((unsigned)((d->pend.m + 3) / 4)), dim3(256), 0, (hipStream_t)stream, d->pend);
+  TGMX_CHECK_LAUNCH("defer_flush");
+  return TGMX_OK;
+}
+
+static bool getenv_no_ride() {
+  static const bool no_ride = getenv("TGMX_NO_RIDE") != nullptr;
+  return no_ride;
+}
+
+
 static bool plan_fuse01(const tgmx_recency_step_t* s, long long S0) {
   static const bool no_fuse = getenv("TGMX_NO_FUSE") != nullptr;
-  static const bool no_ride = getenv("TGMX_NO_RIDE") != nullptr;
   if (no_fuse || s->n_hops < 2 || S0 <= 0 || s->B > kWave || s->k[0] <= 0 || s->k[1] <= 0) return false;
   if (s->indptr != nullptr && (long long)s->k[1] * s->D * 4 < 4096) return false;
   static const bool fuse_by_id = !(getenv("TGMX_FUSE_BY_ID") && atoi(getenv("TGMX_FUSE_BY_ID")) == 0);
@@ -2748,9 +2767,6 @@
     if (prepare_lookup(a, s->out_x[1], s->k[1]) < 0) return false;
     if (packed_group_lanes(a, s->k[1], true) < 64) return false;
   }
-  const long long m = s->directed ? s->n : 2 * s->n;
-  (void)no_ride;
-  (void)m;
   return true;
 }
 
@@ -2799,19 +2815,36 @@
     grp.out_nid = s->seed_nid0; grp.out_ts = s->seed_ts0; grp.groups = s->n_groups;
   }
 
+  tgmx_defer* dfr = csr ? nullptr : s->defer;
+  static const bool defer_on = !(getenv("TGMX_DEFER_COMMIT") && atoi(getenv("TGMX_DEFER_COMMIT")) == 0);
+  const long long m_all = s->directed ? s->n : 2 * s->n;
+  const bool defer = dfr && defer_on && s->defer_ok && s->n > 0 && m_all <= kRidePlaceMaxM && s->n_hops == 2 && S > 0 && !s->guard_seed_errors &&
+                     s->eid0 >= 0 && dfr->N == s->num_nodes && dfr->B == s->B &&
+                     (long long)s->B * s->num_nodes + s->n < 2147483647LL && plan_fuse01(s, S) && !getenv_no_ride();
+  if (dfr && dfr->pending && !defer)
+    if (const int rf = tgmx_defer_flush(dfr, stream)) return rf;
+  if (defer)
+    if (const int rb = defer_buffers(dfr, st)) return rb;
+
   UpdateArgs u{};
   unsigned side_chunks = 0;
   bool ride_place = false;
+  const unsigned stamp = defer ? dfr->stamp + 1 : 0u;
+  int32_t* scratch = defer ? dfr->scratch[stamp & 1] : s->scratch;
   if (s->n > 0) {
     const int rc = fill_update_args(u, s->ring, s->write_pos, s->ring_x, s->D, s->B, s->num_nodes, s->src, s->dst, s->ts,
-                                    s->edge_x, s->n, s->eid0, s->directed, s->key_wrap32, s->scratch, s->status);
+                                    s->edge_x, s->n, s->eid0, s->directed, s->key_wrap32, scratch, s->status);
     if (rc) return rc;
     u.ts_bound = s->ts_bound;
     u.guard_mask = s->guard_seed_errors ? (TGMX_ST_SEED_RANGE | TGMX_ST_SEED_TIME) : 0;
     u.sorted_ts = s->sorted_ts;
-    static const bool no_ride = getenv("TGMX_NO_RIDE") != nullptr;
-    if (u.m <= kBlockMaxM && s->n_hops > 0 && S > 0 && !no_ride) side_chunks = set_chunk_scratch(u, s->scratch + kScratchHead);
+    if (u.m <= kBlockMaxM && s->n_hops > 0 && S > 0 && !getenv_no_ride()) side_chunks = set_chunk_scratch(u, scratch + kScratchHead);
     ride_place = side_chunks > 0 && u.m <= kRidePlaceMaxM && s->n_hops >= 2;
+  }
+  if (defer) {
+    const int q = (int)(stamp & 1);
+    u.dhdr = dfr->hdr[q]; u.drec = dfr->rec[q]; u.dslot = dfr->slot[q]; u.dstamp = stamp;
+    if (dfr->pending) { u.phdr = dfr->hdr[q ^ 1]; u.pstamp = dfr->stamp; }
   }
   static const bool no_side_mid = getenv("TGMX_SIDE_MID") == nullptr;
   SideStream* mid = nullptr;
@@ -2822,8 +2855,6 @@
     (void)hipEventRecord(mid->join, mid->stream);
     side_chunks = 0;
   }
-  static const bool use_tail = getenv("TGMX_TAIL") != nullptr;
-  const unsigned tail_blocks = (ride_place && use_tail && s->n_hops == 2) ? (unsigned)((u.m + 3) / 4) : 0u;
   SideStream* side = nullptr;
   bool side_pending = false;
   if (s->n > 0 && u.m > kBlockMaxM && s->n_hops > 0 && S > 0 && (side = side_stream_for_current_device()) != nullptr) {
@@ -2864,11 +2895,17 @@
     const bool timed = s->timed_hop == 0 || s->timed_hop == 1;
     hipEvent_t e0 = timed ? (hipEvent_t)s->ev_start : nullptr, e1 = timed ? (hipEvent_t)s->ev_stop : nullptr;
     static const bool three_phase_on = !(getenv("TGMX_THREE_PHASE") && atoi(getenv("TGMX_THREE_PHASE")) == 0);
-    const bool three_phase = three_phase_on && ride_place && u.m > 512 && !tail_blocks;
+    const bool three_phase = three_phase_on && ride_place && u.m > 512;
+    const bool commit = defer && dfr->pending;
+    if (commit) {
+      a.phdr = u.phdr; a.pstamp = u.pstamp;
+      a.prec = dfr->rec[(stamp & 1) ^ 1]; a.pslot = dfr->slot[(stamp & 1) ^ 1];
+      a.pstore = s->D > 0 ? dfr->pend.edge_x : nullptr; a.peid0 = (int)dfr->pend.eid0;
+    }
     const int rc = csr ? launch_fused01<false>(a, st, e0, e1, nullptr, 0, 0)
                        : launch_fused01<true>(a, st, e0, e1, side_chunks > 0 ? &u : nullptr,
                                               ride_place ? (three_phase ? kSideSortMergePlace : kSideAll) : kSideSortMerge,
-                                              (ride_place && !three_phase) ? 1u : side_chunks, tail_blocks);
+                                              (ride_place && !three_phase) ? 1u : side_chunks, commit ? &dfr->pend : nullptr);
     if (rc) return rc;
     if (const int rs = enqueue_side()) return rs;
     cur_n = s->out_nid[1];
@@ -2903,7 +2940,7 @@
                              : (ride_place ? (merge_late ? kSideMergePlace : (split_merge ? kSidePlaceOnly : kSidePlace)) : kSideMerge);
     const int rc = csr ? launch_lookup<false>(a, st, e0, e1)
                        : launch_lookup<true>(a, st, e0, e1, ride ? &u : nullptr, stage,
-                                             (h == 1 && ride_place && !merge_late) ? 1u : side_chunks, (h == 1 && ride_place) ? tail_blocks : 0u);
+                                             (h == 1 && ride_place && !merge_late) ? 1u : side_chunks);
     if (rc) return rc;
     if (const int rs = enqueue_side()) return rs;
     cur_n = s->out_nid[h];
@@ -2916,7 +2953,11 @@
     if (mid) {
       (void)hipStreamWaitEvent(st, mid->join, 0);
       hipLaunchKernelGGL(ring_update_feat_kernel<true>, dim3((unsigned)((u.m + 3) / 4)), dim3(256), 0, st, u);
-    } else if (ride_place && tail_blocks) {
+    } else if (defer) {
+      dfr->pend = u;
+      dfr->pending = true;
+      dfr->stamp = stamp;
+      ++dfr->deferred;
     } else if (ride_place) {
       hipLaunchKernelGGL(ring_update_feat_kernel<true>, dim3((unsigned)((u.m + 3) / 4)), dim3(256), 0, st, u);
     } else if (side_chunks > 0) {
diff --git a/tgm_amd/hooks/recency.py b/tgm_amd/hooks/recency.py
--- a/tgm_amd/hooks/recency.py
+++ b/tgm_amd/hooks/recency.py
@@ -1,7 +1,10 @@
 from __future__ import annotations
 
+import ctypes
 import logging
+import os
 import warnings
+import weakref
 from typing import Dict, List, Optional, Sequence
 
 import torch
@@ -100,9 +103,12 @@
 
         self._device: Optional[torch.device] = None
         self._edge_x_dim: Optional[int] = None
-        self._ring: Optional[Tensor] = None
-        self._ring_x: Optional[Tensor] = None
-        self._write_pos: Optional[Tensor] = None
+        self._ring_t: Optional[Tensor] = None
+        self._ring_x_t: Optional[Tensor] = None
+        self._write_pos_t: Optional[Tensor] = None
+        self._defer_commit = os.environ.get('TGMX_DEFER_COMMIT', '1') != '0'
+        self._defer = None
+        self._pre_flush = None
         self._scratch: Optional[Tensor] = None
         self._scratch_edges = 0
         self._status: Optional[Tensor] = None
@@ -131,16 +137,77 @@
     def mode(self) -> str:
         return self._mode
 
+    @property
+    def _ring(self) -> Optional[Tensor]:
+        self.flush_commit()
+        return self._ring_t
+
+    @property
+    def _ring_x(self) -> Optional[Tensor]:
+        self.flush_commit()
+        return self._ring_x_t
+
+    @property
+    def _write_pos(self) -> Optional[Tensor]:
+        self.flush_commit()
+        return self._write_pos_t
+
+    def flush_commit(self) -> None:
+        if self._defer is None:
+            return
+        pre = self._pre_flush() if self._pre_flush is not None else None
+        if pre is not None:
+            pre()
+        lib = _native.load()
+        if not lib.tgmx_defer_pending(self._defer):
+            return
+        with torch.cuda.device(self._device):
+            _native.check(lib.tgmx_defer_flush(self._defer, _native.stream_ptr(self._device.index)), 'tgmx_defer_flush')
+
+    @property
+    def defer_commit(self) -> bool:
+        return self._defer_commit
+
+    @defer_commit.setter
+    def defer_commit(self, on: bool) -> None:
+        self._defer_commit = bool(on)
+        if self._step is None or self._mode != 'ring':
+            return
+        if not on:
+            self._drop_defer()
+        else:
+            self._make_defer()
+        st = _native.RecencyStep()
+        ctypes.memmove(ctypes.byref(st), ctypes.byref(self._step), ctypes.sizeof(_native.RecencyStep))
+        st.defer = self._defer
+        self._step = st
+
+    def _make_defer(self) -> None:
+        if self._defer is None:
+            lib = _native.load()
+            h = lib.tgmx_defer_create(self._num_nodes, self._max_nbrs)
+            if not h:
+                _native.check(-2, 'tgmx_defer_create')
+            self._defer = h
+            self._defer_fin = weakref.finalize(self, lib.tgmx_defer_destroy, h)
+
+    def _drop_defer(self) -> None:
+        if self._defer is not None:
+            self.flush_commit()
+            self._defer_fin()
+            self._defer = None
+
     def reset_state(self) -> None:
         self._last_batch_t = -(1 << 62)
         self._warned_order = False
         if self._mode == 'ring':
-            if self._ring is not None:
+            if self._ring_t is not None:
+                self.flush_commit()
                 lib = _native.load()
                 with torch.cuda.device(self._device):
                     _native.check(
                         lib.tgmx_ring_reset(
-                            self._ring.data_ptr(), self._write_pos.data_ptr(), self._max_nbrs, self._num_nodes, _native.stream_ptr()
+                            self._ring_t.data_ptr(), self._write_pos_t.data_ptr(), self._max_nbrs, self._num_nodes, _native.stream_ptr()
                         ),
                         'tgmx_ring_reset',
                     )
@@ -156,6 +223,7 @@
             self._epoch_lo = int(first_edge)
 
     def _refresh_ts_bound(self, dg: DGraph) -> None:
+        self.flush_commit()
         store = getattr(dg, '_storage', None)
         self._bound_store = store
         bound = 0
@@ -223,21 +291,28 @@
         if self._status is None or old != device:
             self._status = torch.zeros(1, dtype=torch.int32, device=device)
         if self._mode == 'ring':
-            if self._ring is None:
+            if self._ring_t is None:
                 self._warn_rings_under_world()
-                self._ring = torch.empty((N * B, 2), dtype=torch.int64, device=device)
-                self._ring_x = torch.empty((N * B, max(D, 1)), dtype=torch.float32, device=device) if D else None
-                self._write_pos = torch.empty(N, dtype=torch.int32, device=device)
+                self._ring_t = torch.empty((N * B, 2), dtype=torch.int64, device=device)
+                self._ring_x_t = torch.empty((N * B, max(D, 1)), dtype=torch.float32, device=device) if D else None
+                self._write_pos_t = torch.empty(N, dtype=torch.int32, device=device)
                 self.reset_state()
             elif old != device:
-                self._ring = self._ring.to(device)
-                self._ring_x = None if self._ring_x is None else self._ring_x.to(device)
-                self._write_pos = self._write_pos.to(device)
+                if self._defer is not None:
+                    self._device = old
+                    self._drop_defer()
+                    self._device = device
+                self._ring_t = self._ring_t.to(device)
+                self._ring_x_t = None if self._ring_x_t is None else self._ring_x_t.to(device)
+                self._write_pos_t = self._write_pos_t.to(device)
                 self._scratch = None
                 self._scratch_edges = 0
         st = _native.RecencyStep()
         if self._mode == 'ring':
-            st.ring, st.write_pos, st.ring_x = self._ring.data_ptr(), self._write_pos.data_ptr(), _native.ptr(self._ring_x)
+            st.ring, st.write_pos, st.ring_x = self._ring_t.data_ptr(), self._write_pos_t.data_ptr(), _native.ptr(self._ring_x_t)
+            if self._defer_commit:
+                self._make_defer()
+            st.defer = self._defer
         else:
             self._csr = None
         st.D, st.B, st.num_nodes = D, B, N
@@ -305,7 +380,8 @@
 
     def _ensure_scratch(self, n_edges: int, device: torch.device) -> None:
         if n_edges > self._scratch_edges:
-            need = int(_native.load().tgmx_ring_update_scratch_bytes(n_edges, 1 if self._directed else 0))
+            lib = _native.load()
+            need = int(lib.tgmx_ring_update_scratch_bytes(n_edges, 1 if self._directed else 0))
             if need == 0:
                 _native.check(-2, 'tgmx_ring_update_scratch_bytes')
             self._scratch = torch.zeros(need, dtype=torch.uint8, device=device)
@@ -442,6 +518,7 @@
 
             n_edges = batch.edge_src.shape[0] if ring_mode else 0
             keep = None
+            st.defer_ok = 0
             if n_edges:
                 self._ensure_scratch(n_edges, device)
                 ex = batch.edge_x
@@ -456,7 +533,11 @@
                 keep = (src, dst, tt, ex)
                 st.src, st.dst, st.ts, st.edge_x = src.data_ptr(), dst.data_ptr(), tt.data_ptr(), _native.ptr(ex)
                 st.eid0 = -1 if batch._edge_lo is None else int(batch._edge_lo)
-                st.ts_bound, st.sorted_ts = self._store_promise if self._is_store_slice(batch, tt, device) else (0, 0)
+                slice_ = self._is_store_slice(batch, tt, device)
+                st.ts_bound, st.sorted_ts = self._store_promise if slice_ else (0, 0)
+                if slice_ and self._defer is not None and batch._edge_lo is not None:
+                    sx = self._bound_store.on(device).edge_x if D else None
+                    st.defer_ok = 1 if (ex is None or (sx is not None and ex.data_ptr() == sx.data_ptr() + 4 * D * int(batch._edge_lo))) else 0
 
             st.n, st.n_hops = n_edges, L
             st.guard_seed_errors = 1 if self._validate == 'sync' else 0
diff --git a/tgm_amd/pipeline.py b/tgm_amd/pipeline.py
--- a/tgm_amd/pipeline.py
+++ b/tgm_amd/pipeline.py
@@ -3,6 +3,7 @@
 import ctypes
 import os
 import sys
+import weakref
 from typing import Dict, List, Optional, Sequence
 
 import torch
@@ -140,6 +141,7 @@
         p.step.ts_bound, p.step.sorted_ts = nbr._store_promise
         self._pipe, self._step_ref = p, nbr._step
         self._scratch_ptr = nbr._step.scratch
+        nbr._pre_flush = weakref.WeakMethod(self._order_behind_worker)
 
     def _share(self, n: int) -> int:
         lo, hi = shard_bounds(n, *((self._shard.rank, self._shard.world_size) if self._shard is not None else (0, 1)))
```

After: 9.124 billion (median of 6 runs). 1.09x the previous value.
